# martinruenz/co-fusion

Measured on AMD Instinct MI355X. Metric: frames/sec at 640x480 (N active models) + ICP-reduce achieved HBM GB/s vs peak, higher is better.
Workload: dtype f32

## Files before the change

co_fusion_amd/api.py:

```python
from __future__ import annotations

import ctypes as C

import numpy as np
import torch

from . import lib as _libmod

NUM_PYRS = 3


class Cam(C.Structure):
    _fields_ = [("fx", C.c_float), ("fy", C.c_float), ("cx", C.c_float), ("cy", C.c_float)]

    def level(self, l):
        d = float(1 << l)
        return Cam(self.fx / d, self.fy / d, self.cx / d, self.cy / d)


class Config(C.Structure):
    _fields_ = [("width", C.c_int), ("height", C.c_int), ("fx", C.c_float), ("fy", C.c_float), ("cx", C.c_float),
                ("cy", C.c_float), ("device", C.c_int), ("max_models", C.c_int), ("max_surfels", C.c_int)]


# ... 280 lines not shown
        self._check(self.lib.cf_odom_track_batch_async(self.h, oo, n, pp, C.byref(opts), ee))

    def _batch_args(self, odoms, poses):
        n = len(odoms)
        self._keep_poses = [_f(np.asarray(p, np.float32).reshape(16)) for p in poses]
        pp = (C.POINTER(C.c_float) * max(n, 1))(*[C.cast(k, C.POINTER(C.c_float)) for k in self._keep_poses])
        oo = (C.c_void_p * max(n, 1))(*[o.h for o in odoms])

        def ptrs(ts):
            if ts is None:
                return None
            assert len(ts) == n
            return (C.c_void_p * max(n, 1))(*[None if t is None else t.data_ptr() for t in ts])
        return n, oo, pp, ptrs

    def init_models_batch_select(self, odoms, pred_v4, pred_n4, pred_rgba, poses, frame_rgba, alt_v4=None, alt_n4=None, alt_rgba=None,
                                 fill_counts=None, ratio=0.0):
        n, oo, pp, ptrs = self._batch_args(odoms, poses)
        self._check(self.lib.cf_odom_init_models_batch_select(self.h, oo, n, ptrs(pred_v4), ptrs(pred_n4), ptrs(pred_rgba), ptrs(alt_v4),
                                                              ptrs(alt_n4), ptrs(alt_rgba), ptrs(fill_counts), C.c_float(ratio), pp,
                                                              ptrs(frame_rgba)))

    def init_models_batch_frames(self, odoms, pred_v4, pred_n4, pred_rgba, poses, frame_rgba):
        n, oo, pp, ptrs = self._batch_args(odoms, poses)
        self._check(self.lib.cf_odom_init_models_batch_frames(self.h, oo, n, ptrs(pred_v4), ptrs(pred_n4), ptrs(pred_rgba), pp, ptrs(frame_rgba)))

    def init_models_batch(self, odoms, pred_v4, pred_n4, pred_rgba, poses, frame_rgba):
        n, oo, pp, ptrs = self._batch_args(odoms, poses)
        self._check(self.lib.cf_odom_init_models_batch(self.h, oo, n, ptrs(pred_v4), ptrs(pred_n4), ptrs(pred_rgba), pp, _p(frame_rgba)))

    def set_icp_arith(self, mode):
        self._check(self.lib.cf_set_icp_arith(self.h, {"product": 0, "gram": 1, "reference": 2}.get(mode, mode)))

    def profile_enable(self, on=True):
        self._check(self.lib.cf_profile_enable(self.h, int(on)))

    def profile_read(self, reset=True):
        p = Profile()
        self._check(self.lib.cf_profile_read(self.h, C.byref(p), int(reset)))
        return p


class Odometry:

    _BUF = {0: (np.float32, 3), 1: (np.float32, 3), 2: (np.float32, 3), 3: (np.float32, 3), 4: (np.float32, 1),
            5: (np.float32, 1), 6: (np.uint8, 1), 7: (np.uint8, 1), 8: (np.uint8, 1), 9: (np.int16, 1),
            10: (np.int16, 1)}

    def __init__(self, ctx: Context):
        self.ctx = ctx
        self.h = C.c_void_p()
        ctx._check(ctx.lib.cf_odom_create(ctx.h, C.byref(self.h)))

    def close(self):
        if getattr(self, "h", None) and self.ctx.h:
            self.ctx.lib.cf_odom_destroy(self.h)
        self.h = None

    def __del__(self):
        try:
            self.close()
        except Exception:
            pass

    def init_icp_model(self, pred_v4, pred_n4, pose):
        self.ctx._check(self.ctx.lib.cf_odom_init_icp_model(self.h, _p(pred_v4), _p(pred_n4),
                                                            _f(np.asarray(pose, np.float32).reshape(16))))

    def init_rgb_model(self, rgba):
        self.ctx._check(self.ctx.lib.cf_odom_init_rgb_model(self.h, _p(rgba)))

    def set_band(self, row_begin, row_end, add_counts=1):
        self.ctx._check(self.ctx.lib.cf_odom_set_band(self.h, int(row_begin), int(row_end), int(add_counts)))

    def set_culling(self, on=True):
        self.ctx._check(self.ctx.lib.cf_odom_set_culling(self.h, int(bool(on))))

    def init_rgb(self, rgba):
        self.ctx._check(self.ctx.lib.cf_odom_init_rgb(self.h, _p(rgba)))

    def init_first_rgb(self, rgba):
        self.ctx._check(self.ctx.lib.cf_odom_init_first_rgb(self.h, _p(rgba)))

    def init_icp(self, depth_pyr, cutoff):
        arr = (C.c_void_p * 3)(*[d.data_ptr() for d in depth_pyr])
        self._keep = depth_pyr
        self.ctx._check(self.ctx.lib.cf_odom_init_icp(self.h, arr, C.c_float(cutoff)))

    def init_icp_maps(self, vertex4, normal4):
        self.ctx._check(self.ctx.lib.cf_odom_init_icp_maps(self.h, _p(vertex4), _p(normal4)))

    def track(self, trans, rot, rgb_only=False, icp_weight=10.0, pyramid=True, fast_odom=False, so3=True,
              err_surface=None):
        t = _f(np.asarray(trans, np.float32).reshape(3))
        r = _f(np.asarray(rot, np.float32).reshape(9))
        opts = TrackOpts(int(rgb_only), int(pyramid), int(fast_odom), int(so3), icp_weight)
        st = TrackStats()
        self.ctx._check(self.ctx.lib.cf_odom_get_incremental_transformation(self.h, t, r, C.byref(opts),
                                                                            _p(err_surface), C.byref(st)))
        return np.array(t, np.float32), np.array(r, np.float32).reshape(3, 3), st

    def fetch(self):
        t = (C.c_float * 3)(); r = (C.c_float * 9)()
        st = TrackStats()
        self.ctx._check(self.ctx.lib.cf_odom_fetch_result(self.h, t, r, C.byref(st)))
        return np.array(t, np.float32), np.array(r, np.float32).reshape(3, 3), st

    def level0_visited(self):
        a = C.c_uint64(); b = C.c_uint64()
        self.ctx._check(self.ctx.lib.cf_odom_level0_visited(self.h, C.byref(a), C.byref(b)))
        return a.value, b.value

    def last_launch_shape(self):
        a = (C.c_int * 3)(); b = (C.c_int * 3)(); e = C.c_int()
        self.ctx._check(self.ctx.lib.cf_odom_last_launch_shape(self.h, a, b, C.byref(e)))
        return list(a), list(b), e.value

    def share_frame_maps(self, owner):
        self.ctx._check(self.ctx.lib.cf_odom_share_frame_maps(self.h, owner.h))

    def bench_icp(self, level, iters=200):
        us = C.c_float()
        self.ctx._check(self.ctx.lib.cf_odom_bench_icp(self.h, level, iters, C.byref(us)))
        return us.value

    def buffer_address(self, which, level):
        ptr = C.c_void_p()
        self.ctx._check(self.ctx.lib.cf_odom_buffer(self.h, which, level, C.byref(ptr), None))
        return ptr.value

    def buffer(self, which, level):
        ptr = C.c_void_p(); nbytes = C.c_uint64()
        self.ctx._check(self.ctx.lib.cf_odom_buffer(self.h, which, level, C.byref(ptr), C.byref(nbytes)))
        host = np.empty(nbytes.value, np.uint8)
        self.ctx._check(self.ctx.lib.cf_memcpy_d2h(self.ctx.h, host.ctypes.data_as(C.c_void_p), ptr, nbytes))
        w, h = self.ctx.width >> level, self.ctx.height >> level
        if which == 11:
            return host.view(np.float32).reshape(h, w, 3)
        if which == 12:
            return host.view(DATATERM).reshape(h * w)
        if which == 13:
            return host.reshape(h, w)
        if which == 14:
            return host.view(np.float32).reshape((h * w + 63) // 64, 2)
        if which == 15:
            return host.reshape(self.ctx.height // 4, self.ctx.width // 4)
        if which == 16:
            return host.view(np.uint32)
        dt, planes = self._BUF[which]
        return host.view(dt).reshape(planes * h, w)


class FrameDecoder:

    def __init__(self, ctx: Context, max_w, max_h, slots=4):
        from . import klg as _klg
        self._klg = _klg
        self.ctx, self.lib = ctx, ctx.lib
        self.max_w, self.max_h, self.slots = int(max_w), int(max_h), int(slots)
        self.lib.cf_frame_decoder_create.argtypes = [C.c_void_p, C.c_int, C.c_int, C.c_int, C.POINTER(C.c_void_p)]
        self.lib.cf_frame_decoder_destroy.argtypes = [C.c_void_p]
        self.lib.cf_frame_decoder_destroy.restype = None
        self.lib.cf_frame_decoder_slot.argtypes = [C.c_void_p, C.c_int, C.POINTER(_klg.FrameSlot)]
        self.lib.cf_frame_decoder_submit.argtypes = [C.c_void_p, C.c_int, C.POINTER(_klg.FrameDesc)]
        self.lib.cf_frame_decoder_acquire.argtypes = [C.c_void_p, C.c_int, C.c_int, C.POINTER(C.c_void_p), C.POINTER(C.c_void_p)]
        self.lib.cf_frame_decoder_timing.argtypes = [C.c_void_p, C.c_int, C.POINTER(C.c_double), C.POINTER(C.c_double), C.POINTER(C.c_uint64)]
        from . import images as _im
        self._im = _im
        self.lib.cf_frame_decoder_enable_images.argtypes = [C.c_void_p]
        self.lib.cf_frame_decoder_image_slot.argtypes = [C.c_void_p, C.c_int, C.POINTER(_im.ImageSlot)]
# ... 211 lines not shown
```

co_fusion_amd/csrc/cabi.hip:

```cpp
#include <stdlib.h>
#include <string.h>

#include <string>

#include "cf_host.h"

using namespace cf;

void cf_ctx::set_error(const std::string& m)
{
    std::lock_guard<std::mutex> lk(error_mutex);
    last_error = m;
}

static int lane_ready(cf_ctx* ctx, int lane)
{
    if (!ctx->lanes[lane]) {
        HIPCHK(ctx, hipStreamCreateWithFlags(&ctx->lanes[lane], hipStreamNonBlocking));
        HIPCHK(ctx, hipEventCreateWithFlags(&ctx->lane_done[lane], hipEventDisableTiming));
    }
    return CF_OK;
}
static void leave_lane(cf_ctx* ctx)
{
    if (ctx->forked) { ctx->stream = ctx->forked_from; ctx->forked = false; }
}
static int join_lane(cf_ctx* ctx, int lane)
{
    HIPCHK(ctx, hipEventRecord(ctx->lane_done[lane], ctx->lanes[lane]));
    HIPCHK(ctx, hipStreamWaitEvent(ctx->stream, ctx->lane_done[lane], 0));
    return CF_OK;
}

extern "C" {

int cf_create(const cf_config* cfg, cf_ctx** out)
{
    if (!cfg || !out || cfg->width <= 0 || cfg->height <= 0 || (cfg->width % 16) || (cfg->height % 4)) return CF_EINVAL;
    int ndev = 0;
    if (hipGetDeviceCount(&ndev) != hipSuccess || ndev <= 0) return CF_EHIP;
    cf_ctx* ctx = new cf_ctx();
    ctx->cfg = *cfg;
    if (ctx->cfg.max_models <= 0) ctx->cfg.max_models = 1;
    *out = ctx;
    HIPCHK(ctx, hipSetDevice(cfg->device));
    HIPCHK(ctx, hipStreamCreateWithFlags(&ctx->own_stream, hipStreamNonBlocking));
    ctx->stream = ctx->own_stream;
    ctx->icp_launch = IcpLaunch{256, 0, 0};
    if (int r = dmalloc(ctx, &ctx->d_acc_a, (size_t)kGroups * 32)) return r;
    if (int r = dmalloc(ctx, &ctx->d_acc_b, (size_t)kGroups * 32)) return r;
    if (int r = dmalloc(ctx, &ctx->d_out, 64)) return r;
    if (int r = dmalloc(ctx, &ctx->d_scratch_state, 1)) return r;
    if (int r = dmalloc(ctx, &ctx->d_state_pool, (size_t)cf_ctx::kStateSlots)) return r;
    HIPCHK(ctx, hipHostMalloc(reinterpret_cast<void**>(&ctx->h_state_pool), sizeof(OdomDev) * cf_ctx::kStateSlots, hipHostMallocCoherent));
    memset(ctx->h_state_pool, 0, sizeof(OdomDev) * cf_ctx::kStateSlots);
    if (int r = dmalloc(ctx, &ctx->d_so3_sync, (size_t)ctx->cfg.max_models + 1)) return r;
    if (const char* e = getenv("CF_ICP_ARITH")) {
        if (cf_set_icp_arith(ctx, (!strcmp(e, "gram") || !strcmp(e, "1")) ? CF_ICP_ARITH_GRAM : (!strcmp(e, "reference") || !strcmp(e, "2")) ? CF_ICP_ARITH_REFERENCE
                                  : (!strcmp(e, "product") || !strcmp(e, "0")) ? CF_ICP_ARITH_PRODUCT : -1) != CF_OK) {
            ctx->set_error("CF_ICP_ARITH: product | gram | reference"); return CF_EINVAL;
        }
    }
    if (int r = dmalloc(ctx, &ctx->d_cand_scratch, (size_t)cfg->width * cfg->height)) return r;
    HIPCHK(ctx, hipHostMalloc(reinterpret_cast<void**>(&ctx->h_scratch_state), sizeof(OdomDev)));
    HIPCHK(ctx, hipHostMalloc(reinterpret_cast<void**>(&ctx->h_out), sizeof(unsigned long long) * 64));
    ctx->prof.capacity = 8192;
    ctx->prof.events = new hipEvent_t[ctx->prof.capacity];
    for (int i = 0; i < ctx->prof.capacity; i++) HIPCHK(ctx, hipEventCreate(&ctx->prof.events[i]));
    ctx->prof.used = 0; ctx->prof.enabled = 0; ctx->prof.bytes = 0; ctx->prof.launches = 0;
    HIPCHK(ctx, hipStreamSynchronize(ctx->stream));
    return CF_OK;
}

void cf_destroy(cf_ctx* ctx)
{
    if (ctx && ctx->batch_event) (void)hipEventDestroy(ctx->batch_event);
    if (ctx) for (int i = 0; i < cf_ctx::kSurfEvents; i++) if (ctx->surf_events[i]) (void)hipEventDestroy(ctx->surf_events[i]);
    if (!ctx) return;
    (void)hipStreamSynchronize(ctx->stream);
    (void)cf_rccl_destroy(ctx);
    (void)hipFree(ctx->d_acc_a); (void)hipFree(ctx->d_acc_b); (void)hipFree(ctx->d_out);
    (void)hipFree(ctx->d_scratch_state); (void)hipFree(ctx->d_so3_sync); (void)hipFree(ctx->d_cand_scratch);
    (void)hipFree(ctx->d_state_pool); (void)hipHostFree(ctx->h_state_pool);
    (void)hipHostFree(ctx->h_scratch_state); (void)hipHostFree(ctx->h_out);
    if (ctx->d_ref) (void)hipFree(ctx->d_ref);
    if (ctx->h_ref) (void)hipHostFree(ctx->h_ref);
    if (ctx->d_redetect_bits) (void)hipFree(ctx->d_redetect_bits);
    if (ctx->d_redetect_counts) (void)hipFree(ctx->d_redetect_counts);
    if (ctx->h_redetect_counts) (void)hipHostFree(ctx->h_redetect_counts);
    if (ctx->d_search) (void)hipFree(ctx->d_search);
    if (ctx->h_search) (void)hipHostFree(ctx->h_search);
    for (hipEvent_t e : ctx->redetect_ev) if (e) (void)hipEventDestroy(e);
    if (ctx->prof.events) {
        for (int i = 0; i < ctx->prof.capacity; i++) (void)hipEventDestroy(ctx->prof.events[i]);
        delete[] ctx->prof.events;
    }
    for (int i = 0; i < cf_ctx::kLanes; i++) {
        if (ctx->lanes[i]) (void)hipStreamDestroy(ctx->lanes[i]);
        if (ctx->lane_done[i]) (void)hipEventDestroy(ctx->lane_done[i]);
    }
    if (ctx->fork_point) (void)hipEventDestroy(ctx->fork_point);
    for (int i = 0; i < cf_ctx::kMarks; i++) if (ctx->marks[i]) (void)hipEventDestroy(ctx->marks[i]);
    if (ctx->own_stream) (void)hipStreamDestroy(ctx->own_stream);
    delete ctx;
}

const char* cf_last_error(const cf_ctx* ctx)
{
    if (!ctx) return "null ctx";
    static thread_local std::string copy;
    {
        std::lock_guard<std::mutex> lk(const_cast<cf_ctx*>(ctx)->error_mutex);
        copy = ctx->last_error;
    }
    return copy.c_str();
}
int cf_set_stream(cf_ctx* ctx, void* s)
{
    if (!ctx || ctx->forked) return CF_EINVAL;
    if (ctx->stream != (hipStream_t)s) HIPCHK(ctx, hipStreamSynchronize(ctx->stream));
    ctx->stream = (hipStream_t)s;
    return CF_OK;
}
int cf_use_own_stream(cf_ctx* ctx)
{
    if (!ctx || ctx->forked) return CF_EINVAL;
    if (ctx->stream != ctx->own_stream) HIPCHK(ctx, hipStreamSynchronize(ctx->stream));
    ctx->stream = ctx->own_stream;
    return CF_OK;
}

extern "C++" { thread_local cf_thread_binding cf_tls_binding; }

int cf_fork(cf_ctx* ctx, int lane)
{
    if (!ctx || lane < 0) return CF_EINVAL;
    lane %= cf_ctx::kLanes;
    if (int r = lane_ready(ctx, lane)) return r;
    if (!ctx->fork_point) HIPCHK(ctx, hipEventCreateWithFlags(&ctx->fork_point, hipEventDisableTiming));
    if (!ctx->forked) {
        ctx->forked_from = ctx->stream;
        HIPCHK(ctx, hipEventRecord(ctx->fork_point, ctx->forked_from));
        ctx->forked = true;
    }
    HIPCHK(ctx, hipStreamWaitEvent(ctx->lanes[lane], ctx->fork_point, 0));
    ctx->lanes_used |= 1u << lane;
    ctx->stream = ctx->lanes[lane];
    return CF_OK;
}
int cf_mark(cf_ctx* ctx, int slot)
{
    if (!ctx || slot < 0 || slot >= cf_ctx::kMarks) return CF_EINVAL;
    if (!ctx->marks[slot]) HIPCHK(ctx, hipEventCreateWithFlags(&ctx->marks[slot], hipEventDisableTiming));
    HIPCHK(ctx, hipEventRecord(ctx->marks[slot], ctx->stream));
    ctx->mark_set[slot] = true;
    return CF_OK;
}
int cf_event_wait_host(cf_ctx* ctx, int slot)
{
    if (!ctx || slot < 0 || slot >= cf_ctx::kMarks) return CF_EINVAL;
    if (ctx->mark_set[slot]) HIPCHK(ctx, hipEventSynchronize(ctx->marks[slot]));
    return CF_OK;
}
int cf_fork_after(cf_ctx* ctx, int lane, int slot)
{
    if (!ctx || lane < 0 || slot >= cf_ctx::kMarks || ctx->forked) return CF_EINVAL;
    lane %= cf_ctx::kLanes;
    if (int r = lane_ready(ctx, lane)) return r;
    if (slot >= 0 && ctx->mark_set[slot]) HIPCHK(ctx, hipStreamWaitEvent(ctx->lanes[lane], ctx->marks[slot], 0));
    ctx->forked_from = ctx->stream;
    ctx->forked = true;
    ctx->lanes_used |= 1u << lane;
    ctx->stream = ctx->lanes[lane];
    return CF_OK;
}
int cf_main(cf_ctx* ctx)
{
    if (!ctx) return CF_EINVAL;
    leave_lane(ctx);
    return CF_OK;
}
int cf_join(cf_ctx* ctx)
{
    if (!ctx) return CF_EINVAL;
// ... 132 lines not shown
```

co_fusion_amd/csrc/cabi_odom.hip:

```cpp
#include <math.h>
#include <string.h>

#include <string>
#include <vector>

#include "cf_host.h"

using namespace cf;

template <typename F>
static int each_level_buffer(cf_odom* od, int i, size_t n, F f)
{
    if (int r = f(od->vmap_g_prev[i], n * 3)) return r;
    if (int r = f(od->nmap_g_prev[i], n * 3)) return r;
    if (int r = f(od->vmap_curr[i], n * 3)) return r;
    if (int r = f(od->nmap_curr[i], n * 3)) return r;
    if (int r = f(od->lastDepth[i], n)) return r;
    if (int r = f(od->nextDepth[i], n)) return r;
    if (int r = f(od->lastImage[i], n)) return r;
    if (int r = f(od->nextImage[i], n)) return r;
    if (int r = f(od->lastNextImage[i], n)) return r;
    if (int r = f(od->dIdx[i], n)) return r;
    if (int r = f(od->dIdy[i], n)) return r;
    if (int r = f(od->cloud[i], n * 3)) return r;
// ... 91 lines not shown
static int populate_rgbd(cf_odom* od, const uint8_t* rgba, float* const* depths, uint8_t* const* images)
{
    cf_ctx* ctx = od->ctx; hipStream_t s = ctx->stream;
    RgbdBatch b{};
    b.c[0] = rgbd_chain(od, rgba, depths, images);
    launch_rgbd_pyramids(s, b, 1, ctx->cfg.width, ctx->cfg.height, od->maxDepthRGB);
    LAUNCHCHK(ctx);
    return CF_OK;
}
int cf_odom_init_rgb_model(cf_odom* od, const uint8_t* pred_rgba) { if (!od || !pred_rgba) return CF_EINVAL; return populate_rgbd(od, pred_rgba, od->lastDepth, od->lastImage); }
int cf_odom_init_rgb(cf_odom* od, const uint8_t* rgba) { if (!od || !rgba) return CF_EINVAL; od->next_depth_is_last = false; return populate_rgbd(od, rgba, od->nextDepth, od->nextImage); }

int cf_odom_init_models_batch(cf_ctx* ctx, cf_odom* const* ods, int n, const float* const* pred_v4, const float* const* pred_n4,
                              const uint8_t* const* pred_rgba, const float* const* poses, const uint8_t* frame_rgba)
{
    if (!ctx || n <= 0 || !frame_rgba) return CF_EINVAL;
    std::vector<const uint8_t*> frames((size_t)n, frame_rgba);
    return cf_odom_init_models_batch_frames(ctx, ods, n, pred_v4, pred_n4, pred_rgba, poses, frames.data());
}

int cf_odom_init_models_batch_frames(cf_ctx* ctx, cf_odom* const* ods, int n, const float* const* pred_v4, const float* const* pred_n4,
                                     const uint8_t* const* pred_rgba, const float* const* poses, const uint8_t* const* frame_rgba)
{
    return cf_odom_init_models_batch_select(ctx, ods, n, pred_v4, pred_n4, pred_rgba, nullptr, nullptr, nullptr, nullptr, 0.f, poses, frame_rgba);
}

int cf_odom_init_models_batch_select(cf_ctx* ctx, cf_odom* const* ods, int n, const float* const* pred_v4, const float* const* pred_n4,
                                     const uint8_t* const* pred_rgba, const float* const* alt_v4, const float* const* alt_n4,
                                     const uint8_t* const* alt_rgba, const uint32_t* const* fill_counts, float ratio,
                                     const float* const* poses, const uint8_t* const* frame_rgba)
{
    if (!ctx || !ods || n <= 0 || !pred_v4 || !pred_n4 || !pred_rgba || !poses || !frame_rgba) return CF_EINVAL;
    const bool choose = alt_v4 && alt_n4 && alt_rgba && fill_counts;
    const int W = ctx->cfg.width, H = ctx->cfg.height;
    hipStream_t s = ctx->stream;
    for (int base = 0; base < n; base += kPrepBatch) {
        const int nb = n - base < kPrepBatch ? n - base : kPrepBatch;
        ModelMapsBatch mb{};
        RgbdBatch rb{};
        for (int k = 0; k < nb; k++) {
            cf_odom* od = ods[base + k];
            if (!od || !pred_v4[base + k] || !pred_n4[base + k] || !pred_rgba[base + k] || !poses[base + k] || !frame_rgba[base + k]) return CF_EINVAL;
            mb.m[k] = model_maps_args(od, pred_v4[base + k], pred_n4[base + k], poses[base + k]);
            rb.c[k] = rgbd_chain(od, pred_rgba[base + k], od->lastDepth, od->lastImage);
            rb.c[k].v4 = pred_v4[base + k];
            if (choose && fill_counts[base + k]) {
                if (!alt_v4[base + k] || !alt_n4[base + k] || !alt_rgba[base + k]) return CF_EINVAL;
                mb.m[k].alt_v4 = alt_v4[base + k]; mb.m[k].alt_n4 = alt_n4[base + k]; mb.m[k].sel = fill_counts[base + k]; mb.m[k].sel_ratio = ratio;
                rb.c[k].alt_v4 = alt_v4[base + k]; rb.c[k].alt_rgba = alt_rgba[base + k]; rb.c[k].sel = fill_counts[base + k]; rb.c[k].sel_ratio = ratio;
            }
            od->next_depth_is_last = true;
        }
        int n_chains = nb;
        for (int k = 0; k < nb; k++) {
            cf_odom* od = ods[base + k];
            int owner = -1;
            for (int j = nb; j < n_chains; j++)
                if (rb.c[j].rgba == frame_rgba[base + k]) { owner = j; break; }
            if (owner < 0) {
                owner = n_chains++;
                rb.c[owner] = rgbd_chain(od, frame_rgba[base + k], od->nextDepth, od->nextImage);
                for (int i = 0; i < CF_NUM_PYRS; ++i) rb.c[owner].depth[i] = nullptr;
            }
            rb.fan_owner[k] = (signed char)(owner + 1);
            for (int i = 0; i < CF_NUM_PYRS; ++i) rb.fan_image[i][k] = od->nextImage[i];
        }
        launch_model_maps_and_pyramids(s, mb, nb, rb, n_chains, W, H, ods[base]->maxDepthRGB);
    }
    LAUNCHCHK(ctx);
    return CF_OK;
}

int cf_odom_init_first_rgb(cf_odom* od, const uint8_t* rgba)
{
    if (!od || !rgba) return CF_EINVAL;
    cf_ctx* ctx = od->ctx; hipStream_t s = ctx->stream;
    const int W = ctx->cfg.width, H = ctx->cfg.height;
    launch_intensity(s, rgba, W, H, od->lastNextImage[0]);
    for (int i = 0; i + 1 < CF_NUM_PYRS; i++) launch_pyrdown_u8(s, od->lastNextImage[i], W >> i, H >> i, od->lastNextImage[i + 1]);
    LAUNCHCHK(ctx);
    return CF_OK;
}

int cf_odom_init_icp(cf_odom* od, const float* const depth_pyr[CF_NUM_PYRS], float depth_cutoff)
{
    if (!od || !depth_pyr) return CF_EINVAL;
    cf_ctx* ctx = od->ctx; hipStream_t s = ctx->stream;
    const int W = ctx->cfg.width, H = ctx->cfg.height;
    FrameMapsArgs a{};
    a.cutoff = depth_cutoff;
    for (int i = 0; i < CF_NUM_PYRS; ++i) {
        const cf_cam il = cam_level(ctx_cam(ctx), i);
        a.depth[i] = depth_pyr[i]; a.vmap[i] = od->vmap_curr[i]; a.nmap[i] = od->nmap_curr[i]; a.zrange[i] = od->zrange[i];
        a.fx_inv[i] = 1.f / il.fx; a.fy_inv[i] = 1.f / il.fy; a.cx[i] = il.cx; a.cy[i] = il.cy;
        od->ext_vmap_curr[i] = nullptr; od->ext_nmap_curr[i] = nullptr; od->ext_zrange[i] = nullptr;
    }
    launch_frame_maps(s, a, W, H);
    od->zrange_valid = true;
    LAUNCHCHK(ctx);
    return CF_OK;
}

int cf_odom_init_icp_maps(cf_odom* od, const float* vertex4, const float* normal4)
{
    if (!od || !vertex4 || !normal4) return CF_EINVAL;
    cf_ctx* ctx = od->ctx; hipStream_t s = ctx->stream;
    const int W = ctx->cfg.width, H = ctx->cfg.height;
    HIPCHK(ctx, hipMemcpyAsync(od->vmaps_tmp, vertex4, sizeof(float) * 4 * (size_t)W * H, hipMemcpyDeviceToDevice, s));
    for (int i = 0; i < CF_NUM_PYRS; ++i) { od->ext_vmap_curr[i] = nullptr; od->ext_nmap_curr[i] = nullptr; od->ext_zrange[i] = nullptr; }
    launch_copy_maps(s, vertex4, normal4, W, H, od->vmap_curr[0], od->nmap_curr[0]);
    for (int i = 1; i < CF_NUM_PYRS; ++i) {
        launch_resize_map(s, od->vmap_curr[i - 1], W >> (i - 1), H >> (i - 1), od->vmap_curr[i], false);
        launch_resize_map(s, od->nmap_curr[i - 1], W >> (i - 1), H >> (i - 1), od->nmap_curr[i], true);
    }
    od->zrange_valid = false;
    LAUNCHCHK(ctx);
    return CF_OK;
}

int cf_odom_set_culling(cf_odom* od, int on)
{
    if (!od) return CF_EINVAL;
    od->use_occ = on != 0;
    return CF_OK;
}

int cf_odom_set_band(cf_odom* od, int row_begin, int row_end, int add_counts)
{
    if (!od || row_begin < 0 || row_end < row_begin || row_end > od->ctx->cfg.height || (row_begin & 3) || (row_end & 3)) return CF_EINVAL;
    od->band_begin = row_begin; od->band_end = row_end; od->band_counts = add_counts != 0;
    return CF_OK;
}
int cf_set_collective(cf_ctx* ctx, int (*fn)(void*, int, void*, uint64_t, void*), void* user)
{
    if (!ctx) return CF_EINVAL;
    ctx->collective = fn; ctx->collective_user = user;
    return CF_OK;
}

int cf_odom_bind_frame_maps(cf_odom* od, const float* const vmaps[CF_NUM_PYRS], const float* const nmaps[CF_NUM_PYRS])
{
    if (!od) return CF_EINVAL;
    for (int i = 0; i < CF_NUM_PYRS; i++) { od->ext_vmap_curr[i] = vmaps ? vmaps[i] : nullptr; od->ext_nmap_curr[i] = nmaps ? nmaps[i] : nullptr; od->ext_zrange[i] = nullptr; }
    return CF_OK;
}
int cf_odom_share_frame_maps(cf_odom* od, cf_odom* owner)
{
    if (!od || !owner || od->ctx != owner->ctx) return CF_EINVAL;
    for (int i = 0; i < CF_NUM_PYRS; i++) {
        od->ext_vmap_curr[i] = owner->cur_vmap(i); od->ext_nmap_curr[i] = owner->cur_nmap(i); od->ext_zrange[i] = owner->cur_zrange(i);
    }
    return CF_OK;
}

int cf_odom_level0_visited(cf_odom* od, uint64_t* icp_pixels, uint64_t* residual_pixels)
{
    if (!od || !icp_pixels || !residual_pixels) return CF_EINVAL;
    const cf_ctx* ctx = od->ctx;
    const OdomDev* h = od->h_state;
    const uint64_t N = (uint64_t)ctx->cfg.width * ctx->cfg.height;
    *icp_pixels = N; *residual_pixels = h->rgb ? N : 0;
    if (!h->icp) *icp_pixels = 0;
    if (h->cull && ctx->icp_arith != CF_ICP_ARITH_REFERENCE) {
        if (h->icp) { const CullRuns cr = cull_runs(h->stats.cull_box, 0, ctx->cfg.width, ctx->cfg.height); *icp_pixels = (uint64_t)cr.total * 64 < N ? (uint64_t)cr.total * 64 : N; }
        if (h->rgb && h->res_range && h->res_seen[0] >= 0) { const uint64_t px = (uint64_t)h->res_seen[0] * (uint64_t)(ctx->icp_launch.threads * 4); *residual_pixels = px < N ? px : N; }
    }
    return CF_OK;
}

int cf_odom_last_launch_shape(cf_odom* od, int icp_blocks[3], int residual_blocks[3], int* icp_blocks_err)
{
    if (!od) return CF_EINVAL;
    for (int l = 0; l < CF_NUM_PYRS; l++) {
        if (icp_blocks) icp_blocks[l] = od->launch_shape.icp[l];
        if (residual_blocks) residual_blocks[l] = od->launch_shape.res[l];
    }
    if (icp_blocks_err) *icp_blocks_err = od->launch_shape.icp_err;
    return CF_OK;
}

int cf_odom_buffer(cf_odom* od, int which, int level, void** dptr, uint64_t* bytes)
{
    if (!od || level < 0 || level >= CF_NUM_PYRS || !dptr) return CF_EINVAL;
    const size_t n = (size_t)(od->ctx->cfg.width >> level) * (od->ctx->cfg.height >> level);
    void* p = nullptr; size_t b = 0;
    if (which == 0 && !od->ext_vmap_curr[level]) od->zrange_valid = false;
    switch (which) {
        case 0: p = (void*)od->cur_vmap(level); b = n * 12; break;
        case 1: p = (void*)od->cur_nmap(level); b = n * 12; break;
        case 2: p = od->vmap_g_prev[level]; b = n * 12; break;
        case 3: p = od->nmap_g_prev[level]; b = n * 12; break;
        case 4: p = od->lastDepth[level]; b = n * 4; break;
        case 5: p = od->next_depth(level); b = n * 4; break;
        case 6: p = od->lastImage[level]; b = n; break;
        case 7: p = od->nextImage[level]; b = n; break;
        case 8: p = od->lastNextImage[level]; b = n; break;
        case 9: p = od->dIdx[level]; b = n * 2; break;
        case 10: p = od->dIdy[level]; b = n * 2; break;
        case 11: p = od->cloud[level]; b = n * 12; break;
        case 12: p = od->corres[level]; b = n * 16; break;
        case 13: p = od->cand[level]; b = n; break;
        case 14: p = od->zrange[level]; b = (n + 63) / 64 * sizeof(float2); break;
        case 15: if (level != 0) return CF_EINVAL; p = od->occ; b = (size_t)(od->ctx->cfg.width >> 2) * (od->ctx->cfg.height >> 2); break;
        case 16: if (level != 0) return CF_EINVAL; p = od->aabb; b = 6 * sizeof(unsigned); break;
        default: return CF_EINVAL;
    }
    *dptr = p; if (bytes) *bytes = b;
    return CF_OK;
}

}
```

co_fusion_amd/csrc/cabi_steps.hip:

```cpp
#include <math.h>
#include <string.h>

#include <string>
#include <vector>

#include "cf_host.h"
#include "gn_ref_host.h"

using namespace cf;

template <int N, typename Word>
static void unpack_upper(float* A, float* b, Word word)
{
    int shift = 0;
    for (int i = 0; i < N; ++i)
        for (int j = i; j < N + 1; ++j) {
            const float value = word(shift, i, j);
            shift++;
            if (j == N) { if (b) b[i] = value; }
            else if (A) A[j * N + i] = A[i * N + j] = value;
        }
}
static void se3_unpack_host(const unsigned long long* t, int F, float* A, float* b, float* residual)
{
// ... 312 lines not shown
        OdomDev* s = &h[(size_t)k];
        memset(s, 0, sizeof(*s));
        gn_state_to_dev(y.state, s);
        s->icp_acc = buf.d_acc + acc_words * k; s->rgb_acc = s->icp_acc + kAccWords;
        s->sobelScale = sobel_scale; s->maxDepthDeltaRGB = max_depth_delta;
        s->host_twin = &buf.h_twins[k];
        refresh_hot(s);
        memset(&buf.h_twins[k], 0, sizeof(OdomDev));
        gn_state_to_dev(y.twin, &buf.h_twins[k]);
        if (mode == 2) HIPCHK(ctx, hipMemsetAsync(s->rgb_acc, 0xA5, 8 * rgb_words, ctx->stream));
        unsigned long long* seed = &seeds[(size_t)k * kAccWords];
        for (int g = 0; g < kGroups; g++) { seed[(size_t)g * 32 + 29] = (unsigned long long)y.count_seed[g]; seed[(size_t)g * 32 + 30] = (unsigned long long)y.sigma_seed[g]; }
        HIPCHK(ctx, hipMemcpyAsync(s->icp_acc, seed, 8 * kAccWords, hipMemcpyHostToDevice, ctx->stream));
        OdomDev level = *s;
        level.width = cols; level.height = rows;
        level.cand[0] = y.cand; level.nextDepth[0] = y.next_depth; level.lastDepth[0] = y.last_depth; level.lastImage[0] = y.last_image;
        level.nextImage[0] = y.next_image; level.cloud[0] = y.cloud; level.dIdx[0] = y.dIdx; level.dIdy[0] = y.dIdy;
        level.corres[0] = buf.d_recs + N * k;
        level.res_range = y.ranged ? buf.d_range + 2 * k : nullptr;
        ra.m[k] = rgb_model_args(&level, buf.d_states + k, 0);
        ra.m[k].no_counts = y.no_counts ? 1 : 0;
        ra.m[k].res_blocks = y.ranged ? y.res_blocks : 0;
        ranges[(size_t)2 * k] = y.res_range[0]; ranges[(size_t)2 * k + 1] = y.res_range[1];
        HIPCHK(ctx, hipMemcpyAsync(ra.m[k].recs, y.records, 8 * N, hipMemcpyHostToDevice, ctx->stream));
        HIPCHK(ctx, hipMemcpyAsync(ra.m[k].slot_counts, y.slot_counts, sizeof(unsigned) * n_slots, hipMemcpyHostToDevice, ctx->stream));
    }
    HIPCHK(ctx, hipMemcpyAsync(buf.d_range, ranges.data(), sizeof(unsigned) * 2 * n, hipMemcpyHostToDevice, ctx->stream));
    HIPCHK(ctx, hipMemcpyAsync(buf.d_states, h.data(), sizeof(OdomDev) * n, hipMemcpyHostToDevice, ctx->stream));
    launch_rgb_records_residual(ctx->stream, ctx->icp_launch, ra, n, 0);
    LAUNCHCHK(ctx);
    for (int k = 0; k < n; k++) {
        HIPCHK(ctx, hipMemcpyAsync(systems[k].records, ra.m[k].recs, 8 * N, hipMemcpyDeviceToHost, ctx->stream));
        HIPCHK(ctx, hipMemcpyAsync(systems[k].slot_counts, ra.m[k].slot_counts, sizeof(unsigned) * n_slots, hipMemcpyDeviceToHost, ctx->stream));
        HIPCHK(ctx, hipMemcpyAsync(&acc_a[(size_t)k * kAccWords], ra.m[k].icp_acc, 8 * kAccWords, hipMemcpyDeviceToHost, ctx->stream));
    }
    launch_rgb_slot_step(ctx->stream, ra, buf.d_sync, n, mode, ctx->icp_launch.gram ? -1 : CF_FIX_ICP, next_level, last_of_level ? 1 : 0);
    LAUNCHCHK(ctx);
    if (mode == 2) HIPCHK(ctx, hipMemcpyAsync(h.data(), buf.d_states, sizeof(OdomDev) * n, hipMemcpyDeviceToHost, ctx->stream));
    else for (int k = 0; k < n; k++)
        HIPCHK(ctx, hipMemcpyAsync(&acc_b[(size_t)k * kAccWords], ra.m[k].rgb_acc, 8 * kAccWords, hipMemcpyDeviceToHost, ctx->stream));
    HIPCHK(ctx, hipStreamSynchronize(ctx->stream));
    for (int k = 0; k < n; k++) {
        cf_rgb_system& y = systems[k];
        unsigned long long c = 0, g2 = 0;
        for (int g = 0; g < kGroups; g++) { c += acc_a[(size_t)k * kAccWords + (size_t)g * 32 + 29]; g2 += acc_a[(size_t)k * kAccWords + (size_t)g * 32 + 30]; }
        y.count_total = (int64_t)c; y.sigma_total = (int64_t)g2;
        for (int w = 0; w < 32; w++) {
            unsigned long long t = 0;
            for (int g = 0; g < kGroups && mode != 2; g++) t += acc_b[(size_t)k * kAccWords + (size_t)g * 32 + w];
            y.rgb_sums[w] = (int64_t)t;
        }
        if (mode == 2) {
            gn_state_from_dev(&h[(size_t)k], &y.state);
            gn_state_from_dev(&buf.h_twins[k], &y.twin);
            memcpy(y.hot, &h[(size_t)k].hot, sizeof(GnHot));
        } else memcpy(y.hot, &h[(size_t)k].hot, sizeof(GnHot));
    }
    return CF_OK;
}

int cf_so3_prealign_step(cf_ctx* ctx, int n, cf_so3_system* systems, int do_so3, int first_level)
{
    if (!ctx || !systems || n < 1 || n > kMaxBatch || n > ctx->cfg.max_models || first_level < 0 || first_level > 2) return CF_EINVAL;
    static_assert(sizeof(systems->sync) == sizeof(So3Sync) && sizeof(systems->hot) == sizeof(GnHot), "cf_so3_system mirrors the sync and the hot block");
    for (int k = 0; k < n; k++) {
        const cf_gn_state& g = systems[k].state_in;
        if (g.width <= 0 || g.height <= 0 || (g.width % 16) || (g.height % 4)) return CF_EINVAL;
        if (do_so3 && (!systems[k].last_next_image || !systems[k].next_image)) return CF_EINVAL;
    }
    std::vector<OdomDev> back((size_t)n);
    GnStepBuffers buf;
    buf.stream = ctx->stream;
    HIPCHK(ctx, hipMalloc(reinterpret_cast<void**>(&buf.d_states), sizeof(OdomDev) * n));
    HIPCHK(ctx, hipHostMalloc(reinterpret_cast<void**>(&buf.h_twins), sizeof(OdomDev) * n, hipHostMallocCoherent));
    HIPCHK(ctx, hipMemsetAsync(buf.d_states, 0xA5, sizeof(OdomDev) * n, ctx->stream));
    TrackerStates states{};
    for (int k = 0; k < n; k++) {
        OdomDev* s = &buf.h_twins[k];
        memset(s, 0, sizeof(*s));
        gn_state_to_dev(systems[k].state_in, s);
        s->lastNextImage[2] = systems[k].last_next_image; s->nextImage[2] = systems[k].next_image;
        states.dev[k] = buf.d_states + k; states.host[k] = s;
    }
    launch_so3_prealign(ctx->stream, states, ctx->d_so3_sync, n, do_so3 != 0, first_level, nullptr);
    LAUNCHCHK(ctx);
    HIPCHK(ctx, hipMemcpyAsync(back.data(), buf.d_states, sizeof(OdomDev) * n, hipMemcpyDeviceToHost, ctx->stream));
    for (int k = 0; k < n; k++)
        HIPCHK(ctx, hipMemcpyAsync(systems[k].sync, ctx->d_so3_sync + k, sizeof(So3Sync), hipMemcpyDeviceToHost, ctx->stream));
    HIPCHK(ctx, hipStreamSynchronize(ctx->stream));
    for (int k = 0; k < n; k++) {
        gn_state_from_dev(&back[(size_t)k], &systems[k].state_out);
        memcpy(systems[k].hot, &back[(size_t)k].hot, sizeof(GnHot));
    }
    return CF_OK;
}

}
```

co_fusion_amd/csrc/cabi_track.hip:

```cpp
#include <math.h>
#include <stdio.h>
#include <stdlib.h>
#include <string.h>

#include <string>
#include <utility>

#include "cf_host.h"

using namespace cf;

#ifdef CF_ABLATE
static bool diag_no_box() { static const bool v = getenv("CF_NO_SCREEN_BOX") != nullptr; return v; }
static bool diag_no_zcull() { static const bool v = getenv("CF_NO_ZCULL") != nullptr; return v; }
static bool diag_no_occ() { static const bool v = getenv("CF_NO_OCC") != nullptr; return v; }
static const char* diag_icp_ablate() { return getenv("CF_ICP_ABLATE"); }
static const char* diag_trace_out(const char* name) { const char* e = getenv("CF_ICP_TRACE_OUT"); return e ? e : name; }
struct DiagCall {
    const char* name; int call = -2, seen = 0;
    bool hit() { if (call == -2) call = getenv(name) ? atoi(getenv(name)) : -1; return call >= 0 && seen++ == call; }
};
static int clear_accumulators(cf_ctx* ctx, cf_odom* const* ods, int n)
{
    for (int m = 0; m < n; m++) {
// ... 129 lines not shown
    }
    od->pending_so3_swap = opts->so3 != 0;
    od->launch_shape = LaunchShape{};
    LAUNCHCHK(ctx);
    return CF_OK;
}

static void fill_rgb_args(cf_ctx* ctx, cf_odom* const* ods, int n, RgbArgs out[3])
{
    for (int l = 0; l < 3; l++) {
        RgbArgs& a = out[l];
        memset(&a, 0, sizeof(a));
        a.cols = ctx->cfg.width >> l; a.rows = ctx->cfg.height >> l;
        a.il = cam_level(ctx_cam(ctx), l);
        a.sobelScale = ods[0]->sobelScale; a.maxDepthDelta = ods[0]->maxDepthDeltaRGB;
        for (int m = 0; m < n; m++) {
            a.m[m] = rgb_model_args(ods[m]->h_state, ods[m]->d_state, l);
            a.m[m].no_counts = (ods[m]->band_end > 0 && !ods[m]->band_counts) ? 1 : 0;
            a.m[m].res_blocks = a.m[m].res_range ? residual_blocks_for(ods[m]->res_hint[l]) : 0;
        }
    }
}

static void fill_icp_args(cf_ctx* ctx, cf_odom* const* ods, int n, IcpArgs out[3])
{
    for (int l = 0; l < CF_NUM_PYRS; l++) {
        IcpArgs& a = out[l];
        memset(&a, 0, sizeof(a));
        a.cols = ctx->cfg.width >> l; a.rows = ctx->cfg.height >> l;
        a.intr = cam_level(ctx_cam(ctx), l);
        a.distThres = ods[0]->distThres; a.angleThres = ods[0]->angleThres;
        a.angleSqLt = ods[0]->angleSqLt; a.distSqLe = ods[0]->distSqLe;
        a.occ_w = ctx->cfg.width >> 2; a.occ_shift = 2 - l;
        for (int m = 0; m < n; m++) {
            cf_odom* od = ods[m];
            a.m[m] = IcpModelArgs{od->cur_vmap(l), od->cur_nmap(l), od->vmap_g_prev[l], od->nmap_g_prev[l], od->d_state, od->icp_acc,
                                  od->h_state->err_surface, (od->use_occ && od->occ_valid && !diag_no_occ()) ? od->occ : nullptr,
                                  od->band_end > 0 ? (od->band_begin >> l) : 0, od->band_end > 0 ? (od->band_end >> l) : 0,
                                  od->h_state->cull,
                                  diag_no_zcull() ? nullptr : od->cur_zrange(l),
                                  od->h_state->cull ? box_blocks_for(od->box_hint, l, a.cols, a.rows, ctx->icp_launch.threads) : 0};
        }
    }
}

static int prepare_trackers(cf_ctx* ctx, cf_odom* const* ods, int n, const float* const* poses_in, const cf_track_opts* opts,
                            float* const* err_surfaces, RgbPrepBatch& prep, bool launch_prep, bool reference)
{
    for (int base = 0; base < n; base += kPrepBatch) {
        const int nb = n - base < kPrepBatch ? n - base : kPrepBatch;
        if (base) prep = RgbPrepBatch{};
        for (int m = base; m < base + nb; m++) {
            if (int r = odom_prepare(ods[m], poses_in[m], opts, err_surfaces ? err_surfaces[m] : nullptr, &prep.m[m - base])) return r;
            if (reference) {
                ods[m]->h_state->cull = 0; ods[m]->h_state->res_range = nullptr; prep.m[m - base].res_range = nullptr;
                ods[m]->box_hint[0] = kNoBoxHint;
                HIPCHK(ctx, hipMemsetAsync(ods[m]->aabb, 0, 8 * sizeof(unsigned), ctx->stream));
            }
        }
        if (launch_prep) launch_rgb_prep(ctx->stream, prep, nb, ctx->cfg.width, ctx->cfg.height);
    }
    return CF_OK;
}

extern "C" {

int cf_odom_track_batch_async(cf_ctx* ctx, cf_odom* const* ods, int n, const float* const* poses_in,
                              const cf_track_opts* opts, float* const* err_surfaces)
{
    if (!ctx || !ods || n <= 0 || n > ctx->cfg.max_models || n > kMaxBatch || !poses_in || !opts) return CF_EINVAL;
    const TrackTerms terms = track_terms(opts);
    {
        bool drain = false;
        for (int m = 0; m < n; m++) drain = drain || (ods[m] && ods[m]->result_pending);
        if (drain) {
            HIPCHK(ctx, hipStreamSynchronize(ctx->stream));
            for (int m = 0; m < n; m++) if (ods[m]) ods[m]->result_pending = false;
        }
    }
    RgbPrepBatch prep{};
    if (ctx->icp_arith == CF_ICP_ARITH_REFERENCE) {
        for (int m = 0; m < n; m++)
            if (ods[m]->band_end > 0) { ctx->set_error("the reference-order arithmetic (cf_set_icp_arith 2) does not split a tracker's reductions over GPUs"); return CF_ESTATE; }
        if (int r = prepare_trackers(ctx, ods, n, poses_in, opts, err_surfaces, prep, terms.rgb, true)) return r;
        LAUNCHCHK(ctx);
        for (int m = 0; m < n; m++)
            if (int r = ref_track(ctx, ods[m], poses_in[m], opts, err_surfaces ? err_surfaces[m] : nullptr)) return r;
        for (int m = 0; m < n; m++) ods[m]->result_pending = true;
        return CF_OK;
    }
    for (int m = 0; m < n; m++)
        if (ods[m]->gn_epoch_seen != ctx->gn_mode_epoch) {
            HIPCHK(ctx, hipMemsetAsync(ods[m]->rgb_acc, 0, sizeof(unsigned long long) * ods[m]->rgb_acc_words, ctx->stream));
            ods[m]->gn_epoch_seen = ctx->gn_mode_epoch;
        }
    const bool prep_fused = terms.rgb && opts->so3 != 0 && n <= kPrepBatch;
    if (int r = prepare_trackers(ctx, ods, n, poses_in, opts, err_surfaces, prep, terms.rgb && !prep_fused, false)) return r;
    if (prep_fused) rgb_prep_levels(prep, n, ctx->cfg.width, ctx->cfg.height);
    TrackerStates states{};
    for (int m = 0; m < n; m++) { states.dev[m] = ods[m]->d_state; states.host[m] = ods[m]->h_state; }
    IcpArgs icp_args[3];
    fill_icp_args(ctx, ods, n, icp_args);
    RgbArgs rgb_args[3];
    fill_rgb_args(ctx, ods, n, rgb_args);
    OdomDev* h_states[kMaxBatch];
    for (int m = 0; m < n; m++) h_states[m] = ods[m]->h_state;
    GnHook hook{};
    hook.fn = ctx->collective; hook.user = ctx->collective_user;
    bool any_split = false;
    for (int m = 0; m < n; m++) { hook.split[m] = ods[m]->band_end > 0 ? 1 : 0; any_split = any_split || hook.split[m]; }
    if (any_split && !ctx->collective) { ctx->set_error("a tracker has a row band (cf_odom_set_band) but no collective is registered (cf_set_collective)"); return CF_ESTATE; }
    if (any_split && ctx->gn_mode == 0) { ctx->set_error("split reductions need the record-slot data path (cf_set_gn_mode 1)"); return CF_ESTATE; }
    cf::ProfSink* prof = nullptr;
    if (ctx->prof.enabled > 0 && (ctx->prof_calls++ % (unsigned)ctx->prof.enabled) == 0) prof = &ctx->prof;
    TrackDiag diag;
    if (int r = diag.begin(ctx)) return r;
    LaunchShape* shapes[kMaxBatch];
    for (int m = 0; m < n; m++) shapes[m] = &ods[m]->launch_shape;
    IcpLaunch launch_cfg = ctx->icp_launch; launch_cfg.shape = shapes;
    if (!launch_gn_track(ctx->stream, launch_cfg, states, ctx->d_so3_sync, any_split ? &hook : nullptr, icp_args, rgb_args, n,
                         ctx->cfg.width, ctx->cfg.height, opts->so3 != 0, opts->pyramid != 0, opts->fast_odom != 0, terms.rgb, terms.icp, ctx->gn_mode, prof,
                         h_states, prep_fused ? &prep : nullptr)) {
        ctx->set_error("tracking: the registered collective failed inside the Gauss-Newton loop");
        return CF_ESTATE;
    }
    LAUNCHCHK(ctx);
    if (int r = diag.end(ctx, ods, n, icp_args[0], rgb_args[0])) return r;
    for (int m = 0; m < n; m++) ods[m]->result_pending = true;
    return CF_OK;
}

int cf_wait_stream(cf_ctx* ctx)
{
    HIPCHK(ctx, hipStreamSynchronize(ctx->stream));
    return CF_OK;
}

int cf_odom_fetch_result(cf_odom* od, float trans[3], float rot[9], cf_track_stats* stats)
{
    if (!od) return CF_EINVAL;
    cf_ctx* ctx = od->ctx;
    if (int r = cf_wait_stream(ctx)) return r;
    od->result_pending = false;
    if (trans) memcpy(trans, od->h_state->tcurr, 12);
    if (rot) memcpy(rot, od->h_state->Rcurr, 36);
    if (stats) *stats = od->h_state->stats;
    bool fault = od->h_state->stats.fault != 0;
    if (ctx->icp_arith != CF_ICP_ARITH_REFERENCE && od->expected_solves >= 0 && od->h_state->solves != od->expected_solves) {
        (void)hipMemsetAsync(ctx->d_so3_sync, 0, sizeof(So3Sync) * ((size_t)ctx->cfg.max_models + 1), ctx->stream);
        fault = true;
    }
    od->expected_solves = -1;
    if (od->pending_so3_swap) {
        for (int i = 0; i < CF_NUM_PYRS; i++) std::swap(od->lastNextImage[i], od->nextImage[i]);
        od->pending_so3_swap = false;
    }
    if (fault) {
        ctx->set_error("tracking: a bounded device-side wait expired (workgroups of one launch were not co-resident)");
        return CF_ESTATE;
    }
    return CF_OK;
}

int cf_odom_get_covariance(const cf_track_stats* stats, double cov[36])
{
    if (!stats || !cov) return CF_EINVAL;
    constexpr int N = 6;
    double lu[N * N];
    int perm[N];
    memcpy(lu, stats->lastA, sizeof(lu));
    for (int i = 0; i < N; i++) perm[i] = i;
    for (int k = 0; k < N; k++) {
        int piv = k;
        double big = fabs(lu[k * N + k]);
        for (int r = k + 1; r < N; r++) { const double a = fabs(lu[r * N + k]); if (a > big) { big = a; piv = r; } }
        if (piv != k) {
            for (int c = 0; c < N; c++) std::swap(lu[k * N + c], lu[piv * N + c]);
            std::swap(perm[k], perm[piv]);
        }
        if (big != 0.0)
            for (int r = k + 1; r < N; r++) lu[r * N + k] /= lu[k * N + k];
        for (int r = k + 1; r < N; r++)
            for (int c = k + 1; c < N; c++) lu[r * N + c] -= lu[r * N + k] * lu[k * N + c];
    }
    for (int j = 0; j < N; j++) {
        double x[N];
        for (int i = 0; i < N; i++) x[i] = (perm[i] == j) ? 1.0 : 0.0;
        for (int i = 0; i < N; i++)
            for (int c = 0; c < i; c++) x[i] -= lu[i * N + c] * x[c];
        for (int i = N - 1; i >= 0; i--) {
            for (int c = i + 1; c < N; c++) x[i] -= lu[i * N + c] * x[c];
            x[i] /= lu[i * N + i];
        }
        for (int i = 0; i < N; i++) cov[i * N + j] = x[i];
    }
    return CF_OK;
}

int cf_set_gn_mode(cf_ctx* ctx, int mode)
{
    if (!ctx || mode < 0 || mode > 2) return CF_EINVAL;
    if (mode == 2) {
        if (ctx->xcd_round_robin < 0) { HIPCHK(ctx, hipStreamSynchronize(ctx->stream)); ctx->xcd_round_robin = probe_xcd_round_robin(ctx->stream) ? 1 : 0; }
        if (!ctx->xcd_round_robin) { ctx->set_error("cf_set_gn_mode 2: workgroups of a launch are not dealt round-robin over 8 XCDs on this device; the mode needs that"); return CF_ESTATE; }
    }
// ... 43 lines not shown
```

co_fusion_amd/csrc/cf_host.h:

```cpp
#pragma once

#include <string.h>

#include <mutex>
#include <string>

#include "cf_kernels.h"

struct cf_ctx;
struct cf_thread_binding { const cf_ctx* ctx = nullptr; hipStream_t stream = nullptr; };
extern thread_local cf_thread_binding cf_tls_binding;

struct cf_ctx {
    cf_config cfg{};
    hipStream_t stream = nullptr;
    hipStream_t cur() const { return cf_tls_binding.ctx == this ? cf_tls_binding.stream : stream; }
    hipStream_t own_stream = nullptr;
    std::string last_error;
    std::mutex error_mutex;
    cf::IcpLaunch icp_launch{256, 0};
    int icp_arith = 0;
    float* d_ref = nullptr;
    float* h_ref = nullptr;
    unsigned long long* d_acc_a = nullptr;
    unsigned long long* d_acc_b = nullptr;
    unsigned long long* d_out = nullptr;
    unsigned long long* h_out = nullptr;
    cf::OdomDev* d_scratch_state = nullptr;
    cf::OdomDev* h_scratch_state = nullptr;
    uint8_t* d_cand_scratch = nullptr;
    cf::So3Sync* d_so3_sync = nullptr;
    unsigned gn_mode_epoch = 0;
    int xcd_round_robin = -1;
    int gn_mode = 1;
    static constexpr int kStateSlots = 256;
    cf::OdomDev* d_state_pool = nullptr;
    cf::OdomDev* h_state_pool = nullptr;
    bool slot_used[kStateSlots]{};
    hipEvent_t batch_event = nullptr;
    bool extent_cull = true;
    static constexpr int kLanes = 8;
    hipStream_t lanes[kLanes]{};
    hipEvent_t lane_done[kLanes]{};
    hipEvent_t fork_point = nullptr;
    static constexpr int kMarks = 64;
    hipEvent_t marks[kMarks]{};
    bool mark_set[kMarks]{};
    hipStream_t forked_from = nullptr;
    bool forked = false;
    unsigned lanes_used = 0;
    int (*collective)(void* user, int op, void* dev_buf, uint64_t words, void* stream) = nullptr;
    void* collective_user = nullptr;
    void* rccl = nullptr;
    unsigned prof_calls = 0;
    cf::ProfSink prof{};
    double prof_ms_accum = 0;
    static constexpr int kSurfEvents = 64;
    hipEvent_t surf_events[kSurfEvents]{};
    int surf_used = 0; unsigned surf_calls_seen = 0;
    double surf_ms_accum = 0; uint64_t surf_calls = 0, surf_bytes = 0;
    unsigned* d_redetect_bits = nullptr; unsigned redetect_words = 0;
    unsigned* d_redetect_counts = nullptr; unsigned* h_redetect_counts = nullptr;
    bool redetect_timing = false; hipEvent_t redetect_ev[2]{}; float redetect_last_ms = 0.f;
    static constexpr size_t kSearchWords = (size_t)cf::kRedetectBatch * cf::kMomentWords + 32;
    static constexpr size_t kSearchBytes = kSearchWords * 8 + (size_t)cf::kRedetectBatch * cf::kRedetectBins * 4;
    unsigned long long* d_search = nullptr; unsigned long long* h_search = nullptr;
    void set_error(const std::string& m);
};
inline cf_cam ctx_cam(const cf_ctx* ctx) { return cf_cam{ctx->cfg.fx, ctx->cfg.fy, ctx->cfg.cx, ctx->cfg.cy}; }
extern "C" int cf_wait_stream(cf_ctx* ctx);
#define HIPCHK(ctx, call)                                                                      \
    do {                                                                                       \
        hipError_t e_ = (call);                                                                \
        if (e_ != hipSuccess) {                                                                \
            (ctx)->set_error(std::string(#call) + ": " + hipGetErrorString(e_));               \
            return CF_EHIP;                                                                    \
        }                                                                                      \
    } while (0)
#define LAUNCHCHK(ctx) HIPCHK(ctx, hipGetLastError())
template <typename T>
inline int dmalloc(cf_ctx* ctx, T** p, size_t count)
{
    HIPCHK(ctx, hipMalloc(reinterpret_cast<void**>(p), count * sizeof(T)));
    HIPCHK(ctx, hipMemsetAsync(*p, 0, count * sizeof(T), ctx->cur()));
    return CF_OK;
}
inline int clear_acc(cf_ctx* ctx, unsigned long long* acc)
{
    HIPCHK(ctx, hipMemsetAsync(acc, 0, sizeof(unsigned long long) * cf::kGroups * 32, ctx->stream));
    return CF_OK;
}
struct cf_odom;
namespace cf {
int ref_track(cf_ctx* ctx, cf_odom* od, const float pose[16], const cf_track_opts* opts, float* err_surface);
int ref_icp_step(cf_ctx* ctx, const float Rcurr[9], const float tcurr[3], const float* vc, const float* nc, const float Rprev_inv[9], const float tprev[3],
                 cf_cam intr, const float* vp, const float* np, float dist_thres, float angle_thres, int cols, int rows, float* err, float out29[29]);
int ref_rgb_step(cf_ctx* ctx, const cf_dataterm* corres, float sigma, const float* cloud3, float fx, float fy, const int16_t* dIdx, const int16_t* dIdy,
                 float sobel_scale, int cols, int rows, float out29[29]);
int ref_so3_step(cf_ctx* ctx, const uint8_t* last_image, const uint8_t* next_image, const float basis[9], const float kinv[9], const float krlr[9],
                 int cols, int rows, float out11[11]);
inline void pose_split(const float pose[16], float R[9], float t[3])
{
    for (int i = 0; i < 3; i++) { R[3 * i] = pose[4 * i]; R[3 * i + 1] = pose[4 * i + 1]; R[3 * i + 2] = pose[4 * i + 2]; t[i] = pose[4 * i + 3]; }
}
struct TrackTerms { bool icp, rgb; };
inline TrackTerms track_terms(const cf_track_opts* o) { return TrackTerms{!o->rgb_only && o->icp_weight > 0, o->rgb_only || o->icp_weight < 100}; }
}

struct cf_odom {
    cf_ctx* ctx = nullptr;
    float* vmaps_tmp = nullptr;
    float* nmaps_tmp = nullptr;
    float* vmap_g_prev[3]{};
    float* nmap_g_prev[3]{};
    float* vmap_curr[3]{};
    float* nmap_curr[3]{};
    const float* ext_vmap_curr[3]{};
    const float* ext_nmap_curr[3]{};
    float2* zrange[3]{};
    bool zrange_valid = false;
    const float2* ext_zrange[3]{};
    const float* cur_vmap(int l) const { return ext_vmap_curr[l] ? ext_vmap_curr[l] : vmap_curr[l]; }
    const float* cur_nmap(int l) const { return ext_nmap_curr[l] ? ext_nmap_curr[l] : nmap_curr[l]; }
    const float2* cur_zrange(int l) const { return ext_vmap_curr[l] ? ext_zrange[l] : (zrange_valid ? zrange[l] : nullptr); }
    float* lastDepth[3]{};
    float* nextDepth[3]{};
    bool next_depth_is_last = false;
    float* next_depth(int i) const { return next_depth_is_last ? lastDepth[i] : nextDepth[i]; }
    uint8_t* lastImage[3]{};
    uint8_t* nextImage[3]{};
    uint8_t* lastNextImage[3]{};
    int16_t* dIdx[3]{};
    int16_t* dIdy[3]{};
    float* cloud[3]{};
    cf_dataterm* corres[3]{};
    uint8_t* cand[3]{};
    unsigned char* occ = nullptr;
    bool occ_valid = false;
    bool use_occ = false;
    unsigned* aabb = nullptr;
    float map_pose[12]{};
    int box_hint[4] = {0x7fffffff, 0, 0, 0};
    unsigned* res_range = nullptr;
    int res_hint[3] = {-1, -1, -1};
    bool box_valid = false;
    int band_begin = 0, band_end = 0;
    bool band_counts = true;
    unsigned long long* icp_acc = nullptr;
    unsigned long long* rgb_acc = nullptr;
    cf::OdomDev* d_state = nullptr;
    cf::OdomDev* h_state = nullptr;
    int slot = -1;
    float distThres = 0, angleThres = 0, sobelScale = 0, maxDepthDeltaRGB = 0, maxDepthRGB = 0;
    float angleSqLt = 0, distSqLe = 0;
    float minGrad[3]{};
    bool pending_so3_swap = false;
    size_t rgb_acc_words = 0;
    unsigned gn_epoch_seen = 0;
    bool result_pending = false;
    int expected_solves = -1;
    cf::LaunchShape launch_shape{};
};
```

co_fusion_amd/csrc/cf_kernels.h:

```cpp
#pragma once

#include <hip/hip_runtime.h>
#include <hip/hip_ext.h>
#include <stdint.h>

#include "../../include/cofusion_hip.h"

namespace cf {

__host__ __device__ __forceinline__ cf_cam cam_level(cf_cam c, int level)
{
    const int div = 1 << level;
    return cf_cam{c.fx / div, c.fy / div, c.cx / div, c.cy / div};
}

constexpr int kGroups = 64;

struct alignas(64) GnHot {
    int icp, level_done; float cull_z[2];
    float Rcurr[9], tcurr[3];
    float Rprev_inv[9], tprev[3];
    int cull_box[4];
    int rgb, rgbOnly, level_done2, pad;
    float krkInv[9], kt[3];
// ... 147 lines not shown
    if ((cols & 63) == 0) { const int nrx = (bx1 >> 6) - (bx0 >> 6) + 1; return CullRuns{bx0 >> 6, by0, nrx, nrx * (by1 - by0 + 1)}; }
    const int q0 = (by0 * cols) >> 6, q1 = ((by1 + 1) * cols - 1) >> 6;
    return CullRuns{0, q0, 0, q1 - q0 + 1};
}
inline int box_blocks_for(const int box_hint[4], int L, int cols, int rows, int threads)
{
    if (box_hint[0] == kNoBoxHint) return 0;
    const CullRuns cr = cull_runs(box_hint, L, cols, rows);
    const int wpb = threads / 64;
    const int runs = cr.total + cr.total / 4 + 2 * (cr.nrx > 0 ? cr.nrx : (cols + 63) / 64);
    int want = (((runs + 2 * wpb - 1) / (2 * wpb) + 7) / 8) * 8;
    return want < 8 ? 8 : want;
}
inline int residual_blocks_for(int seen) { return seen < 0 ? 0 : seen + seen / 4 + 2; }
struct GnArgs {
    OdomDev* od[kMaxBatch];
    unsigned long long* icp_acc[kMaxBatch];
    unsigned long long* rgb_acc[kMaxBatch];
    OdomDev* od_host[kMaxBatch];
    int slot_px;
    int icp_gram;
};
struct RgbModelArgs {
    OdomDev* st;
    const uint8_t* cand; const float* nextDepth; const float* lastDepth;
    const uint8_t* lastImage; const uint8_t* nextImage;
    cf_dataterm* corres; const float* cloud; const int16_t* dIdx; const int16_t* dIdy;
    unsigned long long* icp_acc; unsigned long long* rgb_acc;
    int no_counts;
    uint2* recs;
    unsigned* slot_counts;
    const unsigned* res_range;
    int res_blocks;
};
struct RgbArgs {
    RgbModelArgs m[kMaxBatch];
    int cols, rows;
    cf_cam il;
    float sobelScale, maxDepthDelta;
    int compact;
    int slot_px;
    IDiv cdiv;
};
inline RgbModelArgs rgb_model_args(const OdomDev* h , OdomDev* d_state, int level)
{
    return RgbModelArgs{d_state, h->cand[level], h->nextDepth[level], h->lastDepth[level], h->lastImage[level], h->nextImage[level],
                        h->corres[level], h->cloud[level], h->dIdx[level], h->dIdy[level], h->icp_acc, h->rgb_acc, 0,
                        reinterpret_cast<uint2*>(h->corres[level]),
                        reinterpret_cast<unsigned*>(reinterpret_cast<uint2*>(h->corres[level]) + (size_t)(h->width >> level) * (h->height >> level)),
                        h->res_range ? h->res_range + 2 * level : nullptr, 0};
}
constexpr int kMaxSlots = 2 * kMaxBatch;
struct IcpArgs {
    IcpModelArgs m[kMaxBatch];
    int cols, rows;
    cf_cam intr;
    float distThres, angleThres;
    float angleSqLt, distSqLe;
    int occ_w, occ_shift;
    int flags;
    int row_begin, row_end;
    IDiv cdiv;
    int slot_end[kMaxSlots];
    unsigned char slot_desc[kMaxSlots];
    int slots_used;
};
constexpr unsigned char kResidualSlot = 0x80;
void launch_icp_level(hipStream_t s, IcpLaunch cfg, const IcpArgs& args, int n, int level, hipEvent_t ev0 = nullptr, hipEvent_t ev1 = nullptr);
void launch_rgb_residual(hipStream_t s, const RgbArgs& ra, int n);
void launch_rgb_step(hipStream_t s, const RgbArgs& ra, int n);
constexpr uint64_t kRgbResidualBytes = 27;
constexpr uint64_t kRgbResidualBytesCompact = 11;
void launch_acc_total(hipStream_t s, const unsigned long long* acc, unsigned long long* out);
void launch_rgb_cand(hipStream_t s, const int16_t* dIdx, const int16_t* dIdy, const float* next_depth,
                     const uint8_t* next_image, float min_scale, int cols, int rows, uint8_t* cand);
void launch_so3_step(hipStream_t s, const uint8_t* last_image, const uint8_t* next_image, const float basis[9],
                     const float kinv[9], const float krlr[9], int cols, int rows, unsigned long long* out16);
void launch_gn_solve(hipStream_t s, const GnArgs& gn, int n, int next_level, int last_of_level);

struct ProfSink {
    hipEvent_t* events; int capacity; int used; uint64_t bytes; uint64_t launches; int enabled;
};

constexpr int kSo3Blocks = 16;
constexpr int kStepSubs = 16;
struct So3Sync { unsigned long long acc[10][16]; unsigned arrive, depart;
                 unsigned step_top, pad;
                 unsigned step_sub[kStepSubs][32]; };
struct GnHook { int (*fn)(void* user, int op, void* dev_buf, uint64_t words, void* stream); void* user; int split[kMaxBatch]; };
struct TrackerStates { OdomDev* dev[kMaxBatch]; const OdomDev* host[kMaxBatch]; };
bool launch_gn_track(hipStream_t s, IcpLaunch cfg, const TrackerStates& states, So3Sync* so3_syncs ,
                     const GnHook* hook, const IcpArgs icp_args[3], const RgbArgs rgb_args[3], int n, int width, int height, bool so3,
                     bool pyramid, bool fast_odom, bool rgb, bool icp, int mode, ProfSink* prof,
                     OdomDev* const* h_states = nullptr ,
                     const RgbPrepBatch* prep = nullptr );
void launch_rgb_slot_step(hipStream_t s, const RgbArgs& ra, So3Sync* so3_syncs , int n, int mode, int icp_fix, int next_level, int last_of_level);
void launch_rgb_records_residual(hipStream_t s, IcpLaunch cfg, const RgbArgs& ra, int n, int level);
inline size_t rgb_acc_rows(size_t n0)
{
    const size_t slots0 = (n0 + 255) / 256, quads0 = (slots0 + 1) / 2;
    return quads0 > (size_t)kGroups ? quads0 : (size_t)kGroups;
}
void launch_so3_prealign(hipStream_t s, const TrackerStates& states, So3Sync* so3_syncs , int n, bool so3, int first_level,
                         const RgbPrepBatch* prep );
void rgb_prep_levels(RgbPrepBatch& b, int n, int W, int H);
float replay_icp_level0(hipStream_t s, IcpLaunch cfg, const IcpArgs& a0, const RgbArgs& r0, int n, int slots, int ablate, int reps, hipEvent_t e0, hipEvent_t e1);
#ifdef CF_ABLATE
void trace_so3_dump(hipStream_t s);
void trace_solve_begin();
void trace_solve_end(hipStream_t s, const char* path);
void trace_step_solve(hipStream_t s, IcpLaunch cfg, const IcpArgs& a0, const RgbArgs& r0, So3Sync* syncs, int n, const char* path);
void trace_icp_level0(hipStream_t s, IcpLaunch cfg, const IcpArgs& a0, const RgbArgs& r0, int n, int slots, const char* path);
#endif
bool probe_xcd_round_robin(hipStream_t s);
float sqrt_gate_lt(float T);
float sqrt_gate_le(float T);

constexpr int kSurfBatch = 16;
struct IndexPassArgs {
    const float* surfels; const unsigned* count; unsigned id_begin, id_end; float t_inv[16]; float maxDepth; int time, timeDelta;
    unsigned long long* keys; unsigned* index; float* vertConf; float* colorTime; float* normRad;
    const float* t_inv_dev;
    float* clean_rec;
    const float* clean_depth;
    unsigned* ext;
    int ext_slot;
};
__host__ __device__ inline void inv44f(const float a[16], float o[16])
{
    const float c00 = a[5] * a[10] - a[6] * a[9];
    const float c01 = a[6] * a[8] - a[4] * a[10];
    const float c02 = a[4] * a[9] - a[5] * a[8];
    const float det = a[0] * c00 + a[1] * c01 + a[2] * c02;
    const float id = 1.0f / det;
    float Li[9];
    Li[0] = c00 * id; Li[1] = (a[2] * a[9] - a[1] * a[10]) * id; Li[2] = (a[1] * a[6] - a[2] * a[5]) * id;
    Li[3] = c01 * id; Li[4] = (a[0] * a[10] - a[2] * a[8]) * id; Li[5] = (a[2] * a[4] - a[0] * a[6]) * id;
    Li[6] = c02 * id; Li[7] = (a[1] * a[8] - a[0] * a[9]) * id; Li[8] = (a[0] * a[5] - a[1] * a[4]) * id;
    for (int i = 0; i < 3; i++) {
        o[i * 4 + 0] = Li[i * 3 + 0]; o[i * 4 + 1] = Li[i * 3 + 1]; o[i * 4 + 2] = Li[i * 3 + 2];
        o[i * 4 + 3] = -(Li[i * 3 + 0] * a[3] + Li[i * 3 + 1] * a[7] + Li[i * 3 + 2] * a[11]);
    }
    o[12] = 0; o[13] = 0; o[14] = 0; o[15] = 1;
}
struct SplatFillArgs {
    const float* depth_filt; const uint8_t* rgba;
    float inv_fx, inv_fy; int pass_geom, pass_rgb;
    float* fill_vertex; float* fill_normal; uint8_t* fill_image;
    unsigned long long* acc;
    unsigned* out2; unsigned* out2_host;
    int sample_blocks;
};
int fill_ratio_sample_blocks(int cols, int rows);
struct SplatPassArgs {
    const float* surfels; const unsigned* count; unsigned count_bound; float t_inv[16]; float maxDepth, confThreshold; int time, maxTime, timeDelta;
    const float* rays; unsigned long long* keys; uint8_t* image; float* vertexConf; float* normalRad; uint16_t* time16;
    SplatFillArgs fill;
};
struct UpdatePassArgs { const float* in; const unsigned* count; unsigned count_bound; unsigned* owner; const float* records; int time; float* out; };
struct SurfelFuseArgs {
    const unsigned* index; const float* vertConf; const float* normRad;
    const uint8_t* rgba; const float* depth_raw; const float* depth_filt; const uint8_t* mask;
    const float* tcx; const float* tcy;
    float pose[16]; cf_cam cam; float inv_fx, inv_fy;
    int cols, rows, time; float weighting; int maskID; float maxDepth;
    float* records; unsigned* new_flags; unsigned* owner;
    int flags_clean = 0;
};
struct CleanPassArgs {
    const unsigned* index; const float* vertConf; const float* colorTime;
    const float* depth_filt; const uint8_t* mask;
    const float* rec;
    float t_inv[16]; cf_cam cam; int cols, rows, time; float confThreshold, outlierCoeff; int timeDelta, maskID;
    const float* surfels; const unsigned* count; const float* fresh; const unsigned* n_fresh; unsigned total_bound; float* staged; unsigned* flags;
};
struct ScanPassArgs {
    const float* rec; const unsigned* flags; long long n; unsigned* block_sums; unsigned* total; unsigned add_to_total; float* out; unsigned* total_host;
    int zero_flags = 0;
};
void launch_index_keys_batch(hipStream_t s, const IndexPassArgs* items, int n, cf_cam cam, int cols, int rows);
bool launch_update_compaction_index_keys(hipStream_t s, const UpdatePassArgs* up, const ScanPassArgs* sc, const IndexPassArgs* ix, int n, cf_cam cam, int cols,
                                         int rows);
void launch_index_resolve_batch(hipStream_t s, const IndexPassArgs* items, int n, cf_cam cam, int cols, int rows);
enum { kSplatFull = 0, kSplatCount = 1, kSplatDepth = 2 };
void launch_combined_predict_batch(hipStream_t s, const SplatPassArgs* items, int n, cf_cam cam, int cols, int rows, int mode = kSplatFull);
void launch_associate_batch(hipStream_t s, const SurfelFuseArgs* items, int n);
void launch_update_batch(hipStream_t s, const UpdatePassArgs* items, int n);
void launch_clean_batch(hipStream_t s, const CleanPassArgs* items, int n);
// ... 33 lines not shown
```

co_fusion_amd/csrc/track_prep.hip:

```cpp
#include "cf_device.h"
#include "cf_kernels.h"
#include "track_prep_dev.h"

namespace cf {

static constexpr int kBlock = 256;
static inline int grid_for(int n) { return (n + kBlock - 1) / kBlock; }

__global__ void __launch_bounds__(kBlock) vmap_kernel(const float* __restrict__ depth, int cols, int rows, float fx_inv,
                                                      float fy_inv, float cx, float cy, float cutoff,
                                                      float* __restrict__ vmap)
{
    const int i = blockIdx.x * kBlock + threadIdx.x;
    if (i >= cols * rows) return;
    const int v = i / cols, u = i - v * cols;
    const float z = depth[i];
    if (z != 0 && z < cutoff) {
        vmap[i] = z * (u - cx) * fx_inv;
        vmap[i + rows * cols] = z * (v - cy) * fy_inv;
        vmap[i + 2 * rows * cols] = z;
    } else {
        vmap[i] = qnan();
    }
}
// ... 268 lines not shown
    if (fy >= kT2H || gx >= W2 || gy >= H2) return;
    if constexpr (kDepth) store(2, gy * W2 + gx, pyrdown_f32_at(TileTaps<float>{t1, kF1W, oy1, ox1}, W1, H1, gx, gy));
    else store(2, gy * W2 + gx, pyrdown_u8_at(TileTaps<uint8_t>{t1, kF1W, oy1, ox1}, W1, H1, gx, gy));
}
__global__ void __launch_bounds__(kBlock) rgbd_base_kernel(const RgbdBatch b, int N, float cutoff) { rgbd_base_body(b, N, cutoff, (int)blockIdx.x, (int)blockIdx.y); }
__global__ void __launch_bounds__(kBlock) rgbd_pyrdown_kernel(const RgbdBatch b, int level, int scols, int srows)
{
    const RgbdChain& c = b.c[blockIdx.y];
    const int n = (scols / 2) * (srows / 2), nb = (n + kBlock - 1) / kBlock;
    if ((int)blockIdx.x < nb) {
        const int i = blockIdx.x * kBlock + threadIdx.x;
        if (i < n && c.depth[level]) pyrdown_f32_px(c.depth[level], scols, srows, c.depth[level + 1], i);
    } else {
        const int i = (blockIdx.x - nb) * kBlock + threadIdx.x;
        if (i < n) rgbd_store_image(b, (int)blockIdx.y, level + 1, i, pyrdown_u8_val(c.image[level], scols, srows, i));
    }
}

__global__ void __launch_bounds__(kBlock) rgb_expand_kernel(const uint8_t* __restrict__ rgb, int N, uchar4* __restrict__ rgba)
{
    const int i = blockIdx.x * kBlock + threadIdx.x;
    if (i >= N) return;
    rgba[i] = make_uchar4(rgb[3 * i], rgb[3 * i + 1], rgb[3 * i + 2], 255);
}

__global__ void __launch_bounds__(kBlock) intensity_kernel(const uchar4* __restrict__ rgba, int N, uint8_t* __restrict__ dst)
{
    const int i = blockIdx.x * kBlock + threadIdx.x;
    if (i >= N) return;
    const uchar4 s = rgba[i];
    const int value = (int)((float)s.x * 0.114f + (float)s.y * 0.299f + (float)s.z * 0.587f);
    dst[i] = (uint8_t)value;
}

__constant__ float kSobelX[9] = {0.52201f, 0.00000f, -0.52201f, 0.79451f, -0.00000f, -0.79451f, 0.52201f, 0.00000f, -0.52201f};
__constant__ float kSobelY[9] = {0.52201f, 0.79451f, 0.52201f, 0.00000f, 0.00000f, 0.00000f, -0.52201f, -0.79451f, -0.52201f};

__global__ void __launch_bounds__(kBlock) sobel_kernel(const uint8_t* __restrict__ src, int cols, int rows,
                                                       int16_t* __restrict__ dx, int16_t* __restrict__ dy)
{
    const int i = blockIdx.x * kBlock + threadIdx.x;
    if (i >= cols * rows) return;
    const int y = i / cols, x = i - y * cols;
    float dxv = 0, dyv = 0;
    constexpr float sx[9] = {0.52201f, 0.00000f, -0.52201f, 0.79451f, -0.00000f, -0.79451f, 0.52201f, 0.00000f, -0.52201f};
    constexpr float sy[9] = {0.52201f, 0.79451f, 0.52201f, 0.00000f, 0.00000f, 0.00000f, -0.52201f, -0.79451f, -0.52201f};
    if (x >= 1 && y >= 1 && x <= cols - 2 && y <= rows - 2) {
        const uint8_t* __restrict__ p0 = src + (y - 1) * cols + (x - 1);
#pragma unroll
        for (int r = 0; r < 3; r++)
#pragma unroll
            for (int c = 0; c < 3; c++) {
                const float s = (float)p0[r * cols + c];
                dxv += s * sx[8 - (r * 3 + c)];
                dyv += s * sy[8 - (r * 3 + c)];
            }
    } else {
        int k = 8;
        for (int j = max(y - 1, 0); j <= min(y + 1, rows - 1); j++)
            for (int c = max(x - 1, 0); c <= min(x + 1, cols - 1); c++) {
                const float s = (float)src[j * cols + c];
                dxv += s * kSobelX[k];
                dyv += s * kSobelY[k];
                --k;
            }
    }
    dx[i] = (int16_t)(int)dxv;
    dy[i] = (int16_t)(int)dyv;
}

__global__ void __launch_bounds__(kBlock) cloud_kernel(const float* __restrict__ depth, int cols, int rows, float invFx,
                                                       float invFy, float cx, float cy, float* __restrict__ cloud3)
{
    const int i = blockIdx.x * kBlock + threadIdx.x;
    if (i >= cols * rows) return;
    const int y = i / cols, x = i - y * cols;
    const float z = depth[i];
    cloud3[i * 3 + 0] = (x - cx) * z * invFx;
    cloud3[i * 3 + 1] = (y - cy) * z * invFy;
    cloud3[i * 3 + 2] = z;
}


__global__ void __launch_bounds__(kBlock) frame_maps_kernel(const FrameMapsArgs a)
{
    int lb;
    const int lv = level_of(a.L, blockIdx.x, lb);
    const int cols = a.L.cols[lv], rows = a.L.rows[lv], N = cols * rows;
    const int i = lb * kBlock + threadIdx.x;
    const float* __restrict__ depth = a.depth[lv];
    const float cutoff = a.cutoff;
    if (a.zrange[lv]) {
        const float inf = __int_as_float(0x7f800000);
        const float zz = i < N ? depth[i] : 0.f;
        const bool ok = zz != 0 && zz < cutoff;
        float lo = ok ? zz : inf, hi = ok ? zz : -inf;
#pragma unroll
        for (int o = 32; o > 0; o >>= 1) { lo = fminf(lo, __shfl_xor(lo, o, 64)); hi = fmaxf(hi, __shfl_xor(hi, o, 64)); }
        if ((threadIdx.x & 63) == 0 && i < N) a.zrange[lv][i >> 6] = make_float2(lo, hi);
    }
    if (i >= N) return;
    float* __restrict__ vmap = a.vmap[lv];
    float* __restrict__ nmap = a.nmap[lv];
    const float fx_inv = a.fx_inv[lv], fy_inv = a.fy_inv[lv], cx = a.cx[lv], cy = a.cy[lv];
    const int v = i / cols, u = i - v * cols;
    const bool edge = (u == cols - 1 || v == rows - 1);
    const float z = depth[i];
    const float z01 = edge ? 0.f : depth[i + 1], z10 = edge ? 0.f : depth[i + cols];
    float x00 = qnan();
    if (z != 0 && z < cutoff) {
        x00 = z * (u - cx) * fx_inv;
        vmap[i] = x00;
        vmap[i + N] = z * (v - cy) * fy_inv;
        vmap[i + 2 * N] = z;
    } else {
        vmap[i] = qnan();
    }
    if (edge) { nmap[i] = qnan(); return; }
    const float x01 = (z01 != 0 && z01 < cutoff) ? z01 * ((u + 1) - cx) * fx_inv : qnan();
    const float x10 = (z10 != 0 && z10 < cutoff) ? z10 * (u - cx) * fx_inv : qnan();
    if (!is_nan(x00) && !is_nan(x01) && !is_nan(x10)) {
        const f3 v00 = {x00, z * (v - cy) * fy_inv, z};
        const f3 v01 = {x01, z01 * (v - cy) * fy_inv, z01};
        const f3 v10 = {x10, z10 * ((v + 1) - cy) * fy_inv, z10};
        const f3 r = normalized(cross(v01 - v00, v10 - v00));
        nmap[i] = r.x; nmap[i + N] = r.y; nmap[i + 2 * N] = r.z;
    } else {
        nmap[i] = qnan();
    }
}

__global__ void __launch_bounds__(kBlock) rgb_prep_kernel(const RgbPrepBatch b) { rgb_prep_body(b.m[blockIdx.y], (int)blockIdx.x); }

struct MapVal { f3 p; bool have; };

__device__ __forceinline__ void emit_map(float* __restrict__ map, int idx, int N, const MapVal& m, const m33& R, const f3& t, bool add_t)
{
    if (!m.have) { map[idx] = qnan(); return; }
    if (!is_nan(m.p.x)) {
        f3 d = mul(R, m.p);
        if (add_t) d = d + t;
        map[idx] = d.x; map[idx + N] = d.y; map[idx + 2 * N] = d.z;
    } else {
        map[idx] = qnan(); map[idx + N] = m.p.y; map[idx + 2 * N] = m.p.z;
    }
}

__device__ __forceinline__ MapVal resize4(const MapVal& a00, const MapVal& a01, const MapVal& a10, const MapVal& a11, bool normalize)
{
    MapVal o; o.have = false; o.p = f3{qnan(), qnan(), qnan()};
    const float x00 = a00.have ? a00.p.x : qnan(), x01 = a01.have ? a01.p.x : qnan();
    const float x10 = a10.have ? a10.p.x : qnan(), x11 = a11.have ? a11.p.x : qnan();
    if (is_nan(x00) || is_nan(x01) || is_nan(x10) || is_nan(x11)) return o;
    f3 n;
    n.x = (a00.p.x + a01.p.x + a10.p.x + a11.p.x) / 4;
    n.y = (a00.p.y + a01.p.y + a10.p.y + a11.p.y) / 4;
    n.z = (a00.p.z + a01.p.z + a10.p.z + a11.p.z) / 4;
    if (normalize) n = normalized(n);
    o.have = true; o.p = n;
    return o;
}

__device__ __forceinline__ MapVal lane_mapval(const MapVal& m, int src_lane)
{
    MapVal o;
    o.p.x = __shfl(m.p.x, src_lane, 64); o.p.y = __shfl(m.p.y, src_lane, 64); o.p.z = __shfl(m.p.z, src_lane, 64);
    o.have = __shfl((int)m.have, src_lane, 64) != 0;
    return o;
}
__device__ __forceinline__ void model_maps_tiled_body(const ModelMapsBatch& b, int bx, int by)
{
    const ModelMapsArgs& a = b.m[by];
    const int cols = a.cols, rows = a.rows, N0 = cols * rows, c1 = cols >> 1, c2 = cols >> 2, N1 = N0 >> 2, N2 = N0 >> 4;
    const int lane = threadIdx.x & 63, lx = lane & 15, ly = lane >> 4;
    const int tiles_x = cols >> 4;
    const int tile = bx * 4 + (threadIdx.x >> 6);
    if (tile >= tiles_x * (rows >> 2)) return;
    const int ty = tile / tiles_x, tx = tile - ty * tiles_x;
    const int x = tx * 16 + lx, y = ty * 4 + ly, i0 = y * cols + x;
    const bool alt = a.sel && (float)a.sel[0] / (float)a.sel[1] < a.sel_ratio;
    const float4* __restrict__ v4 = reinterpret_cast<const float4*>(alt ? a.alt_v4 : a.pred_v4);
    const float4* __restrict__ n4 = reinterpret_cast<const float4*>(alt ? a.alt_n4 : a.pred_n4);
    float4* __restrict__ snap = reinterpret_cast<float4*>(a.snapshot);
    m33 R; for (int k = 0; k < 9; k++) R.m[k] = a.R[k];
    const f3 tr = {a.t[0], a.t[1], a.t[2]};
    const float4 vs = v4[i0], ns = n4[i0];
    snap[i0] = vs;
    MapVal v0, n0;
    v0.have = true; n0.have = true;
    const bool valid = !(vs.z == 0);
    if (valid) { v0.p = f3{vs.x, vs.y, vs.z}; n0.p = f3{ns.x, ns.y, ns.z}; }
    else { v0.p = f3{qnan(), qnan(), qnan()}; n0.p = v0.p; }
    emit_map(a.vmap[0], i0, N0, v0, R, tr, true);
    emit_map(a.nmap[0], i0, N0, n0, R, tr, false);
    const MapVal v01 = lane_mapval(v0, lane + 1), v10 = lane_mapval(v0, lane + 16), v11 = lane_mapval(v0, lane + 17);
    const MapVal n01 = lane_mapval(n0, lane + 1), n10 = lane_mapval(n0, lane + 16), n11 = lane_mapval(n0, lane + 17);
    MapVal v1, n1;
    v1.have = false; n1.have = false; v1.p = f3{qnan(), qnan(), qnan()}; n1.p = v1.p;
    if (((lx | ly) & 1) == 0) {
        v1 = resize4(v0, v01, v10, v11, false);
        n1 = resize4(n0, n01, n10, n11, true);
        const int i1 = (y >> 1) * c1 + (x >> 1);
        emit_map(a.vmap[1], i1, N1, v1, R, tr, true);
        emit_map(a.nmap[1], i1, N1, n1, R, tr, false);
    }
    const MapVal w01 = lane_mapval(v1, lane + 2), w10 = lane_mapval(v1, lane + 32), w11 = lane_mapval(v1, lane + 34);
    const MapVal m01 = lane_mapval(n1, lane + 2), m10 = lane_mapval(n1, lane + 32), m11 = lane_mapval(n1, lane + 34);
    const unsigned long long valid_bits = __ballot(valid);
    if ((lx & 3) == 0 && ly == 0) {
        const MapVal v2 = resize4(v1, w01, w10, w11, false);
        const MapVal n2 = resize4(n1, m01, m10, m11, true);
        const int i2 = (y >> 2) * c2 + (x >> 2);
        emit_map(a.vmap[2], i2, N2, v2, R, tr, true);
        emit_map(a.nmap[2], i2, N2, n2, R, tr, false);
        if (a.occ) a.occ[i2] = ((valid_bits >> lx) & 0x000F000F000F000Full) != 0 ? 1 : 0;
    }
    if (a.aabb && valid_bits != 0) {
        const float inf = __int_as_float(0x7f800000);
        float lo[3] = {inf, inf, inf}, hi[3] = {-inf, -inf, -inf};
        if (valid && !is_nan(v0.p.x) && !is_nan(vs.z)) { lo[0] = hi[0] = (float)x; lo[1] = hi[1] = (float)y; lo[2] = hi[2] = vs.z; }
#pragma unroll
        for (int o = 32; o > 0; o >>= 1)
#pragma unroll
            for (int k = 0; k < 3; k++) { lo[k] = fminf(lo[k], __shfl_xor(lo[k], o, 64)); hi[k] = fmaxf(hi[k], __shfl_xor(hi[k], o, 64)); }
        if (lane < 6 && lo[0] <= hi[0] && lo[1] <= hi[1] && lo[2] <= hi[2]) {
            const float val = lane == 0 ? lo[0] : lane == 1 ? lo[1] : lane == 2 ? lo[2] : lane == 3 ? hi[0] : lane == 4 ? hi[1] : hi[2];
            const unsigned key = lane < 3 ? ~fkey(val) : fkey(val);
            if (key > __hip_atomic_load(&a.aabb[lane], __ATOMIC_RELAXED, __HIP_MEMORY_SCOPE_AGENT)) atomicMax(&a.aabb[lane], key);
        }
    }
}
__global__ void __launch_bounds__(256) model_maps_tiled_kernel(const ModelMapsBatch b) { model_maps_tiled_body(b, (int)blockIdx.x, (int)blockIdx.y); }
__global__ void __launch_bounds__(256) prep_fused_kernel(const ModelMapsBatch mb, int mm_bx, int mm_total, const RgbdBatch rb, int W, int H, float cutoff, int tiles)
{
    __shared__ float tile_lds[kTileLds];
    const int n_pyr = (int)gridDim.x - mm_total, b = blockIdx.x;
    if (b >= n_pyr) { const int m = b - n_pyr, by = m / mm_bx; model_maps_tiled_body(mb, m - by * mm_bx, by); }
    else {
        const int by = b / (2 * tiles), t = b - by * 2 * tiles;
        if (t < tiles) rgbd_tile_body<true>(rb, W, H, cutoff, t, by, tile_lds);
        else rgbd_tile_body<false>(rb, W, H, cutoff, t - tiles, by, tile_lds);
    }
}

static Level3 levels3(int W, int H)
{
    Level3 L; int acc = 0;
    for (int i = 0; i < 3; i++) { L.cols[i] = W >> i; L.rows[i] = H >> i; acc += grid_for(L.cols[i] * L.rows[i]); L.blk_end[i] = acc; }
    return L;
}
void launch_frame_maps(hipStream_t s, FrameMapsArgs a, int W, int H)
{
    a.L = levels3(W, H);
    frame_maps_kernel<<<a.L.blk_end[2], kBlock, 0, s>>>(a);
}
void rgb_prep_levels(RgbPrepBatch& b, int n, int W, int H)
{
    const Level3 L = levels3(W, H);
    for (int m = 0; m < n; m++) b.m[m].L = L;
}
void launch_rgb_prep(hipStream_t s, RgbPrepBatch b, int n, int W, int H)
{
    const Level3 L = levels3(W, H);
    for (int m = 0; m < n; m++) b.m[m].L = L;
    rgb_prep_kernel<<<dim3(L.blk_end[2], n), kBlock, 0, s>>>(b);
}
void launch_model_maps(hipStream_t s, const ModelMapsBatch& b, int n)
{
    const int tiles = (b.m[0].cols >> 4) * (b.m[0].rows >> 2);
    model_maps_tiled_kernel<<<dim3((tiles + 3) / 4, n), 256, 0, s>>>(b);
}
void launch_model_maps_and_pyramids(hipStream_t s, const ModelMapsBatch& mb, int n, const RgbdBatch& rb, int n_chains, int W, int H, float cutoff)
{
    static_assert(kBlock == 256, "the fused launch runs both bodies with 256 threads");
    const int mm_bx = ((mb.m[0].cols >> 4) * (mb.m[0].rows >> 2) + 3) / 4, tiles = rgbd_tiles(W, H);
    prep_fused_kernel<<<2 * tiles * n_chains + mm_bx * n, 256, 0, s>>>(mb, mm_bx, mm_bx * n, rb, W, H, cutoff, tiles);
}
void launch_rgbd_pyramids(hipStream_t s, const RgbdBatch& b, int n_chains, int W, int H, float cutoff)
{
    rgbd_base_kernel<<<dim3(2 * grid_for(W * H), n_chains), kBlock, 0, s>>>(b, W * H, cutoff);
    for (int i = 0; i + 1 < 3; i++)
        rgbd_pyrdown_kernel<<<dim3(2 * grid_for(((W >> i) / 2) * ((H >> i) / 2)), n_chains), kBlock, 0, s>>>(b, i, W >> i, H >> i);
}
void launch_vmap(hipStream_t s, const float* depth, int cols, int rows, cf_cam intr, float cutoff, float* vmap)
{
    vmap_kernel<<<grid_for(cols * rows), kBlock, 0, s>>>(depth, cols, rows, 1.f / intr.fx, 1.f / intr.fy, intr.cx, intr.cy,
                                                         cutoff, vmap);
}
void launch_nmap(hipStream_t s, const float* vmap, int cols, int rows, float* nmap)
{
    nmap_kernel<<<grid_for(cols * rows), kBlock, 0, s>>>(vmap, cols, rows, nmap);
}
void launch_copy_maps(hipStream_t s, const float* v4, const float* n4, int cols, int rows, float* vmap, float* nmap)
{
    copy_maps_kernel<<<grid_for(cols * rows), kBlock, 0, s>>>(reinterpret_cast<const float4*>(v4),
                                                              reinterpret_cast<const float4*>(n4), cols * rows, vmap, nmap);
}
void launch_resize_map(hipStream_t s, const float* in, int in_cols, int in_rows, float* out, bool normalize)
{
    const int n = (in_cols / 2) * (in_rows / 2);
    if (normalize) resize_map_kernel<true><<<grid_for(n), kBlock, 0, s>>>(in, in_cols, in_rows, out);
    else resize_map_kernel<false><<<grid_for(n), kBlock, 0, s>>>(in, in_cols, in_rows, out);
}
void launch_transform_maps(hipStream_t s, float* vmap, float* nmap, int cols, int rows, const float R[9], const float t[3])
{
    m33 Rm; for (int i = 0; i < 9; i++) Rm.m[i] = R[i];
    transform_maps_kernel<<<grid_for(cols * rows), kBlock, 0, s>>>(vmap, nmap, cols * rows, Rm, f3{t[0], t[1], t[2]});
}
void launch_vertices_to_depth(hipStream_t s, const float* v4, int cols, int rows, float cutoff, float* depth)
{
    vertices_to_depth_kernel<<<grid_for(cols * rows), kBlock, 0, s>>>(reinterpret_cast<const float4*>(v4), cols * rows,
                                                                      cutoff, depth);
}
void launch_pyrdown_f32(hipStream_t s, const float* src, int scols, int srows, float* dst)
{
    pyrdown_f32_kernel<<<grid_for((scols / 2) * (srows / 2)), kBlock, 0, s>>>(src, scols, srows, dst);
}
void launch_pyrdown_u8(hipStream_t s, const uint8_t* src, int scols, int srows, uint8_t* dst)
{
    pyrdown_u8_kernel<<<grid_for((scols / 2) * (srows / 2)), kBlock, 0, s>>>(src, scols, srows, dst);
}
void launch_intensity(hipStream_t s, const uint8_t* rgba, int cols, int rows, uint8_t* dst)
{
    intensity_kernel<<<grid_for(cols * rows), kBlock, 0, s>>>(reinterpret_cast<const uchar4*>(rgba), cols * rows, dst);
}
void launch_rgb_expand(hipStream_t s, const uint8_t* rgb, int n, uint8_t* rgba)
{
    rgb_expand_kernel<<<grid_for(n), kBlock, 0, s>>>(rgb, n, reinterpret_cast<uchar4*>(rgba));
}
void launch_sobel(hipStream_t s, const uint8_t* src, int cols, int rows, int16_t* dx, int16_t* dy)
{
    sobel_kernel<<<grid_for(cols * rows), kBlock, 0, s>>>(src, cols, rows, dx, dy);
}
void launch_cloud(hipStream_t s, const float* depth, int cols, int rows, cf_cam il, float* cloud3)
{
    cloud_kernel<<<grid_for(cols * rows), kBlock, 0, s>>>(depth, cols, rows, 1.0f / il.fx, 1.0f / il.fy, il.cx, il.cy, cloud3);
}

}
```

co_fusion_amd/csrc/track_prep_dev.h:

```cpp
#pragma once
#include "cf_device.h"
#include "cf_kernels.h"

namespace cf {
__device__ __forceinline__ int level_of(const Level3& L, int b, int& lb)
{
    const int lv = b < L.blk_end[0] ? 0 : (b < L.blk_end[1] ? 1 : 2);
    lb = b - (lv ? L.blk_end[lv - 1] : 0);
    return lv;
}

__device__ __forceinline__ void rgb_prep_body(const RgbPrepArgs& a, int bx)
{
    int lb;
    const int lv = level_of(a.L, bx, lb);
    const int cols = a.L.cols[lv], rows = a.L.rows[lv];
    const int k = lb * 256 + (int)threadIdx.x;
    uint8_t ok = 0;
    if (k < cols * rows) {
    const int y = k / cols, x = k - y * cols;
    const uint8_t* __restrict__ src = a.nextImage[lv];
    {
        const float z = a.lastDepth[lv][k];
        float* __restrict__ cloud3 = a.cloud[lv];
        cloud3[k * 3 + 0] = (x - a.cx[lv]) * z * a.fx_inv[lv];
        cloud3[k * 3 + 1] = (y - a.cy[lv]) * z * a.fy_inv[lv];
        cloud3[k * 3 + 2] = z;
    }
    float dxv = 0, dyv = 0;
    constexpr float sx[9] = {0.52201f, 0.00000f, -0.52201f, 0.79451f, -0.00000f, -0.79451f, 0.52201f, 0.00000f, -0.52201f};
    constexpr float sy[9] = {0.52201f, 0.79451f, 0.52201f, 0.00000f, 0.00000f, 0.00000f, -0.52201f, -0.79451f, -0.52201f};
    if (x >= 1 && y >= 1 && x <= cols - 2 && y <= rows - 2) {
        const uint8_t* __restrict__ p0 = src + (y - 1) * cols + (x - 1);
#pragma unroll
        for (int r = 0; r < 3; r++)
#pragma unroll
            for (int c = 0; c < 3; c++) {
                const float s = (float)p0[r * cols + c];
                dxv += s * sx[8 - (r * 3 + c)];
                dyv += s * sy[8 - (r * 3 + c)];
            }
    } else {
        int kk = 8;
        for (int j = max(y - 1, 0); j <= min(y + 1, rows - 1); j++)
            for (int c = max(x - 1, 0); c <= min(x + 1, cols - 1); c++) {
                const float s = (float)src[j * cols + c];
                dxv += s * sx[kk];
                dyv += s * sy[kk];
                --kk;
            }
    }
    const int16_t dx16 = (int16_t)(int)dxv, dy16 = (int16_t)(int)dyv;
    a.dIdx[lv][k] = dx16; a.dIdy[lv][k] = dy16;
    if (x < cols - 5 && y < rows - 1) {
        bool valid = true;
        for (int u = max(y - 2, 0); u < min(y + 2, rows); u++)
            for (int v = max(x - 2, 0); v < min(x + 2, cols); v++) valid = valid && (src[u * cols + v] > 0);
        if (valid) {
            const int valx = dx16, valy = dy16;
            const float mTwo = (float)((valx * valx) + (valy * valy));
            if (mTwo >= a.minScale[lv] && !is_nan(a.nextDepth[lv][k])) ok = 1;
        }
    }
    a.cand[lv][k] = ok;
    }
    if (a.res_range) {
        if (__syncthreads_or(ok)) {
            if (threadIdx.x == 0) { atomicMax(&a.res_range[2 * lv], ~(unsigned)lb); atomicMax(&a.res_range[2 * lv + 1], (unsigned)lb + 1u); }
        }
    }
}
}
```

co_fusion_amd/csrc/track_reduce.hip:

```cpp
#include "cf_device.h"
#include "cf_kernels.h"
#include "track_prep_dev.h"
#include "track_sums_dev.h"

namespace cf {

__device__ __forceinline__ int idiv(int n, IDiv d) { return (int)(__umulhi((unsigned)n, d.M) >> d.s); }

struct IcpProj { f3 vcurr_g; int g; int inb; int ux, uy; };

__device__ __forceinline__ IcpProj icp_project(const m33& Rcurr, const f3& tcurr, const m33& Rprev_inv, const f3& tprev, const cf_cam& intr,
                                               int cols, int rows, f3 vcurr)
{
    IcpProj o;
    o.vcurr_g = mul(Rcurr, vcurr) + tcurr;
    const f3 vcurr_cp = mul(Rprev_inv, o.vcurr_g - tprev);
    const int ux = f2i_rn(vcurr_cp.x * intr.fx / vcurr_cp.z + intr.cx);
    const int uy = f2i_rn(vcurr_cp.y * intr.fy / vcurr_cp.z + intr.cy);
    o.inb = !(ux < 0 || uy < 0 || ux >= cols || uy >= rows || vcurr_cp.z < 0);
    o.g = o.inb ? uy * cols + ux : 0;
    o.ux = o.inb ? ux : 0; o.uy = o.inb ? uy : 0;
    return o;
}

// ... 590 lines not shown

#include "track_so3_dev.h"
#include "track_solve_dev.h"
#include "track_rgb_step_dev.h"

namespace cf {

#ifdef CF_ABLATE
static IcpArgs g_last_icp_args; static int g_last_n_icp_blocks = 0, g_last_grid = 0;
#endif
static IcpArgs with_cdiv(IcpArgs a) { a.cdiv = make_idiv(a.cols); return a; }
typedef void (*IcpKernel)(const IcpArgs, const RgbArgs, int);
#define ICP_TAG(T) {{icp_reduce_kernel<1, T, false>, icp_reduce_kernel<1, T, true>}, {icp_reduce_kernel<2, T, false>, icp_reduce_kernel<2, T, true>}, \
                    {icp_reduce_kernel<4, T, false>, icp_reduce_kernel<4, T, true>}}
static constexpr IcpKernel kIcpKernels[7][3][2] = {ICP_TAG(0), ICP_TAG(1), ICP_TAG(2), {}, ICP_TAG(4), ICP_TAG(5), ICP_TAG(6)};
#undef ICP_TAG
static void launch_plain_or_timed(IcpKernel kernel, dim3 grid, dim3 block, unsigned lds, hipStream_t s, hipEvent_t ev0, hipEvent_t ev1, const IcpArgs& args,
                              const RgbArgs& ra, int n_icp_blocks)
{
    if (!ev0 && !ev1) kernel<<<grid, block, lds, s>>>(args, ra, n_icp_blocks);
    else hipExtLaunchKernelGGL(kernel, grid, block, lds, s, ev0, ev1, 0, args, ra, n_icp_blocks);
}

static void launch_icp_rgbres(hipStream_t s, IcpLaunch cfg, const IcpArgs& args_in, const RgbArgs& ra_in, bool icp, bool rgb, int n, int level,
                              hipEvent_t ev0, hipEvent_t ev1)
{
    if (cfg.ppt == 0) cfg.ppt = (level == 0 && !cfg.gram) ? 2 : 1;
    const int res_per_block = cfg.threads * (ra_in.compact ? 4 : 1);
    const int n_res_blocks = rgb ? ((icp ? args_in.cols * args_in.rows : ra_in.cols * ra_in.rows) + res_per_block - 1) / res_per_block : 0;
    IcpArgs args = with_cdiv(args_in);
    RgbArgs ra = ra_in; ra.cdiv = make_idiv(ra.cols);
    const int N = ((args.row_end > 0 ? args.row_end : args.rows) - args.row_begin) * args.cols;
    const int per_block = cfg.threads * cfg.ppt;
    const int nlog = (N + per_block - 1) / per_block;
    const int full = icp ? ((nlog + 7) / 8) * 8 : 0;
    int blocks[kMaxBatch];
    for (int m = 0; m < n; m++) {
        IcpModelArgs& ma = args.m[m];
        const bool ok = icp && ma.cull && ma.box_blocks > 0 && !cfg.gram && (!(args.flags & 1) || (args.flags & 2)) && args.row_end == 0 && ma.row_end == 0;
        ma.box_blocks = ok ? (ma.box_blocks < full ? ((ma.box_blocks + 7) / 8) * 8 : full) : 0;
        blocks[m] = ok ? ma.box_blocks : full;
    }
    int res_compact[kMaxBatch] = {};
    for (int m = 0; m < n && n_res_blocks > 0; m++) {
        RgbModelArgs& rm = ra.m[m];
        if (!ra.compact || !rm.res_range || rm.res_blocks <= 0 || rm.res_blocks > n_res_blocks) rm.res_blocks = n_res_blocks;
        else res_compact[m] = rm.res_blocks;
        if (!ra.compact) rm.res_range = nullptr;
    }
    if (cfg.shape) {
        const int L = 2 - args.occ_shift;
        for (int m = 0; m < n; m++) {
            LaunchShape* sh = cfg.shape[m];
            if (!sh || L < 0 || L > 2) continue;
            if (args.flags & 1) sh->icp_err = args.m[m].box_blocks; else sh->icp[L] = args.m[m].box_blocks;
            sh->res[L] = res_compact[m];
        }
    }
    int total = 0, slot = 0, n_icp_blocks = 0;
    auto add = [&](int m, bool residual, int count) {
        total += ((count + 7) / 8) * 8;
        args.slot_end[slot] = total; args.slot_desc[slot] = (unsigned char)(m | (residual ? kResidualSlot : 0)); slot++;
        if (!residual) n_icp_blocks += count;
    };
    for (int pass = 0; pass < 2 && icp; pass++) for (int m = 0; m < n; m++) if ((args.m[m].box_blocks > 0) == (pass == 0)) add(m, false, blocks[m]);
    for (int m = 0; m < n && n_res_blocks > 0; m++) add(m, true, ra.m[m].res_blocks);
    args.slots_used = slot;
    for (; slot < kMaxSlots; slot++) { args.slot_end[slot] = 0x7fffffff; args.slot_desc[slot] = 0; }
    const dim3 grid(total);
#ifdef CF_ABLATE
    g_last_icp_args = args; g_last_n_icp_blocks = n_icp_blocks; g_last_grid = (int)grid.x;
#endif
    const unsigned lds = cfg.gram ? (unsigned)(cfg.threads / 64) * kGramWaveDwords * sizeof(int) : 0u;
    const int tag = (level == 0 ? 0 : level == 1 ? 1 : 2) + (n > 1 ? 4 : 0), ppt_index = cfg.ppt == 4 ? 2 : cfg.ppt == 2 ? 1 : 0;
    static_assert(kIcpKernels[3][0][0] == nullptr && kIcpKernels[2][2][1] && kIcpKernels[4][0][0], "tags are level (0..2) or level + 4: row 3 is never looked up");
    launch_plain_or_timed(kIcpKernels[tag][ppt_index][cfg.gram ? 1 : 0], grid, dim3(cfg.threads), lds, s, ev0, ev1, args, ra, n_icp_blocks);
}

void launch_icp_level(hipStream_t s, IcpLaunch cfg, const IcpArgs& args, int n, int level, hipEvent_t ev0, hipEvent_t ev1)
{
    launch_icp_rgbres(s, cfg, args, RgbArgs{}, true, false, n, level, ev0, ev1);
}

void launch_so3_prealign(hipStream_t s, const TrackerStates& states, So3Sync* so3_syncs, int n, bool so3, int first_level, const RgbPrepBatch* prep)
{
    const int gx = so3 ? 8 * kSo3Blocks : 1;
    static const RgbPrepBatch none{};
    const int prep_bx = prep ? prep->m[0].L.blk_end[2] : 0;
    so3_prealign_kernel<<<gx * n + prep_bx * n, 256, 0, s>>>(states, so3_syncs, so3 ? 1 : 0, first_level, gx, gx * n, prep ? *prep : none, prep_bx);
}

void launch_rgb_slot_step(hipStream_t s, const RgbArgs& ra, So3Sync* so3_syncs, int n, int mode, int icp_fix, int next_level, int last_of_level)
{
    const int N = ra.cols * ra.rows, n_slots = (N + ra.slot_px - 1) / ra.slot_px;
    if (mode == 2) {
        const int n_quads = (n_slots + 1) / 2;
        rgb_step_solve_kernel<<<8 * n_quads * ((n + 7) / 8), 256, 0, s>>>(ra, so3_syncs, n_slots, n_quads, make_idiv(n_quads > 1 ? n_quads : 2), n,
                                                                         icp_fix, next_level, last_of_level);
    } else rgb_slot_step_kernel<<<dim3(n_slots, n), 256, 0, s>>>(ra, n_slots);
}
void launch_rgb_records_residual(hipStream_t s, IcpLaunch cfg, const RgbArgs& ra_in, int n, int level)
{
    RgbArgs ra = ra_in; ra.compact = 1; ra.slot_px = cfg.threads * 4;
    IcpArgs a{}; a.cols = ra.cols; a.rows = ra.rows;
    launch_icp_rgbres(s, cfg, a, ra, false, true, n, level, nullptr, nullptr);
}

bool launch_gn_track(hipStream_t s, IcpLaunch cfg, const TrackerStates& states, So3Sync* so3_syncs, const GnHook* hook, const IcpArgs icp_args[3],
                     const RgbArgs rgb_args[3], int n, int width, int height, bool so3, bool pyramid, bool fast_odom, bool rgb, bool icp, int mode,
                     ProfSink* prof, OdomDev* const* h_states, const RgbPrepBatch* prep)
{
    int iterations[3];
    iterations[0] = fast_odom ? 3 : 10;
    iterations[1] = pyramid ? 5 : 0;
    iterations[2] = pyramid ? 4 : 0;
    int first_level = 2;
    while (first_level > 0 && iterations[first_level] == 0) first_level--;
    launch_so3_prealign(s, states, so3_syncs, n, so3, first_level, prep);
    GnArgs gn{};
    gn.icp_gram = cfg.gram;
    gn.slot_px = cfg.threads * 4;
    for (int m = 0; m < n; m++) {
        gn.od[m] = const_cast<OdomDev*>(icp_args[0].m[m].st);
        gn.icp_acc[m] = icp_args[0].m[m].acc;
        gn.rgb_acc[m] = rgb_args[0].m[m].rgb_acc;
        gn.od_host[m] = h_states ? h_states[m] : nullptr;
    }
    const bool slots = mode != 0;
    bool any_culled = false;
    for (int m = 0; m < n; m++) any_culled = any_culled || (icp_args[0].m[m].cull && icp_args[0].m[m].err);
    const bool err_aside = icp && any_culled;
    bool hook_failed = false;
    for (int i = 2; i >= 0; i--) {
        const int N = (width >> i) * (height >> i);
        for (int j = 0; j < iterations[i]; j++) {
            const bool last_of_level = (j == iterations[i] - 1);
            int next_level = i;
            if (last_of_level) {
                next_level = i - 1;
                while (next_level >= 0 && iterations[next_level] == 0) next_level--;
            }
            RgbArgs ra = rgb_args[i];
            ra.compact = slots ? 1 : 0;
            ra.slot_px = cfg.threads * 4;
            {
                const bool timed = prof && prof->enabled && i == 0 && prof->used + 4 <= prof->capacity;
                IcpArgs a = icp_args[i];
                a.flags = (i == 0 && last_of_level) ? (err_aside ? 3 : 1) : 0;
                launch_icp_rgbres(s, cfg, a, ra, icp, rgb, n, i, timed ? prof->events[prof->used] : nullptr,
                                  timed ? prof->events[prof->used + 1] : nullptr);
                if (timed) {
                    prof->used += 2;
                    prof->bytes += (uint64_t)N * ((icp ? 24 + 24 * (uint64_t)n : 0) + (rgb ? (slots ? kRgbResidualBytesCompact : kRgbResidualBytes) * (uint64_t)n : 0));
                    prof->launches += 1;
                }
            }
            const bool err_here = err_aside && i == 0 && last_of_level;
            const bool err_with_step = err_here && rgb && slots && mode != 2;
            if (err_here && !err_with_step) {
                icp_error_surface_kernel<<<dim3((N + 255) / 256, n), 256, 0, s>>>(with_cdiv(icp_args[i]));
            }
            if (hook && hook->fn) {
                FoldArgs fa{}; int nf = 0;
                for (int m = 0; m < n; m++) if (hook->split[m]) fa.acc[nf++] = gn.icp_acc[m];
                if (nf) acc_fold_kernel<<<nf, 64, 0, s>>>(fa);
                for (int m = 0; m < n; m++)
                    if (hook->split[m] && hook->fn(hook->user, 0, gn.icp_acc[m], 32, (void*)s) != 0) hook_failed = true;
            }
            if (rgb && mode == 2) {
                launch_rgb_slot_step(s, ra, so3_syncs, n, 2, cfg.gram ? -1 : kFixICP, next_level, last_of_level ? 1 : 0);
                continue;
            }
            if (rgb) {
                if (slots) {
                    const int n_slots = (N + ra.slot_px - 1) / ra.slot_px;
                    if (err_with_step) rgb_slot_step_err_kernel<<<dim3(n_slots + (N + 255) / 256, n), 256, 0, s>>>(ra, n_slots, with_cdiv(icp_args[i]));
                    else launch_rgb_slot_step(s, ra, so3_syncs, n, 1, 0, next_level, last_of_level ? 1 : 0);
                }
                else rgb_step_kernel<<<dim3((N + 255) / 256, n), 256, 0, s>>>(ra);
            }
            gn_solve_kernel<<<n, 256, 0, s>>>(gn, next_level, last_of_level ? 1 : 0);
        }
    }
    return !hook_failed;
}

float replay_icp_level0(hipStream_t s, IcpLaunch cfg, const IcpArgs& a0, const RgbArgs& r0, int n, int slots, int ablate, int reps, hipEvent_t e0, hipEvent_t e1)
{
    IcpArgs a = a0; a.flags = ablate << 8;
    RgbArgs ra = r0; ra.compact = slots ? 1 : 0; ra.slot_px = cfg.threads * 4;
    for (int i = 0; i < 3; i++) launch_icp_rgbres(s, cfg, a, ra, true, true, n, 0, nullptr, nullptr);
    (void)hipEventRecord(e0, s);
    for (int i = 0; i < reps; i++) launch_icp_rgbres(s, cfg, a, ra, true, true, n, 0, nullptr, nullptr);
    (void)hipEventRecord(e1, s);
    (void)hipStreamSynchronize(s);
    float ms = 0; (void)hipEventElapsedTime(&ms, e0, e1);
    return ms * 1000.f / reps;
}

#ifdef CF_ABLATE
void trace_so3_dump(hipStream_t s)
// ... 140 lines not shown
```

co_fusion_amd/csrc/track_so3_dev.h:

```cpp
#pragma once
#include "track_prep_dev.h"
#include "track_sums_dev.h"

namespace cf {

__device__ __forceinline__ void screen_box(const float* lo, const float* hi, const float* Rb, const float* tb, const float* Rcurr, const float* tcurr,
                                           cf_cam intr, float distThres, int W, int H, int lane, int (&out)[4], float (&zout)[2])
{
    const float finf = __int_as_float(0x7f800000);
    zout[0] = -finf; zout[1] = finf;
    if (!(lo[0] <= hi[0])) { out[0] = 1; out[1] = 1; out[2] = 0; out[3] = 0; return; }
    const float m = distThres * 1.01f + 1e-3f;
    const float px = (lane & 1) ? hi[0] + 3.f : lo[0] - 3.f, py = (lane & 2) ? hi[1] + 3.f : lo[1] - 3.f;
    const float znear = lo[2] - m, pz = (lane & 4) ? hi[2] + m : znear;
    const float cx_ = (px - intr.cx) / intr.fx * pz, cy_ = (py - intr.cy) / intr.fy * pz;
    const float dx = (Rb[0] * cx_ + Rb[1] * cy_ + Rb[2] * pz + tb[0]) - tcurr[0];
    const float dy = (Rb[3] * cx_ + Rb[4] * cy_ + Rb[5] * pz + tb[1]) - tcurr[1];
    const float dz = (Rb[6] * cx_ + Rb[7] * cy_ + Rb[8] * pz + tb[2]) - tcurr[2];
    const float xc = Rcurr[0] * dx + Rcurr[3] * dy + Rcurr[6] * dz;
    const float yc = Rcurr[1] * dx + Rcurr[4] * dy + Rcurr[7] * dz;
    const float zc = Rcurr[2] * dx + Rcurr[5] * dy + Rcurr[8] * dz;
    const float u = intr.fx * xc / zc + intr.cx, v = intr.fy * yc / zc + intr.cy;
    const bool bad = !(znear > 0.05f) || !(zc > 0.05f) || !is_finite(u) || !is_finite(v);
    float u0 = u, u1 = u, v0 = v, v1 = v, z0 = zc, z1 = zc;
#pragma unroll
    for (int o = 1; o < 8; o <<= 1) {
        u0 = fminf(u0, __shfl_xor(u0, o, 64)); u1 = fmaxf(u1, __shfl_xor(u1, o, 64));
        v0 = fminf(v0, __shfl_xor(v0, o, 64)); v1 = fmaxf(v1, __shfl_xor(v1, o, 64));
        z0 = fminf(z0, __shfl_xor(z0, o, 64)); z1 = fmaxf(z1, __shfl_xor(z1, o, 64));
    }
    if (__any(bad)) { out[0] = 0; out[1] = 0; out[2] = W - 1; out[3] = H - 1; return; }
    zout[0] = z0 - (1e-3f + 1e-3f * fabsf(z0)); zout[1] = z1 + (1e-3f + 1e-3f * fabsf(z1));
    const float fw = (float)(W + 16), fh = (float)(H + 16);
    out[0] = (int)floorf(fminf(fmaxf(u0, -16.f), fw)) - 3; out[1] = (int)floorf(fminf(fmaxf(v0, -16.f), fh)) - 3;
    out[2] = (int)ceilf(fminf(fmaxf(u1, -16.f), fw)) + 3; out[3] = (int)ceilf(fminf(fmaxf(v1, -16.f), fh)) + 3;
}

__device__ __forceinline__ void so3_gradient(const uint8_t* __restrict__ img, int cols, int x, int y, float& gx, float& gy)
{
    const float actu = (float)img[y * cols + x];
    float back = (float)img[y * cols + x - 1], fore = (float)img[y * cols + x + 1];
    gx = ((back + actu) / 2.0f) - ((fore + actu) / 2.0f);
    back = (float)img[(y - 1) * cols + x]; fore = (float)img[(y + 1) * cols + x];
    gy = ((back + actu) / 2.0f) - ((fore + actu) / 2.0f);
}

__device__ __forceinline__ void so3_pass(const uint8_t* __restrict__ lastImage, const uint8_t* __restrict__ nextImage,
                                         const m33& B, const m33& Ki, const float* __restrict__ krlr, int cols, int rows,
                                         unsigned long long (*lds)[16], unsigned long long* totals, int block, int blocks)
{
    constexpr float lim = (float)(1 << ((50 - kFixSO3) / 2));
    constexpr float scale = (float)(1 << kFixSO3);
    const int N = cols * rows, T = blockDim.x;
    unsigned long long acc[16];
#pragma unroll
    for (int k = 0; k < 16; k++) acc[k] = 0;
    const float a = krlr[0], b = krlr[1], c = krlr[2], d = krlr[3], e = krlr[4], f = krlr[5], g = krlr[6], h = krlr[7],
                ii = krlr[8];
    for (int k = block * T + threadIdx.x; k < N; k += blocks * T) {
        const int y = k / cols, x = k - y * cols;
        const f3 unwarped = {(float)x, (float)y, 1.0f};
        const f3 warped = mul(B, unwarped);
        const int wx = f2i_rn(warped.x / warped.z), wy = f2i_rn(warped.y / warped.z);
        if (!(wx >= 1 && wx < cols - 1 && wy >= 1 && wy < rows - 1 && x >= 1 && x < cols - 1 && y >= 1 && y < rows - 1))
            continue;
        float gnx, gny, glx, gly;
        so3_gradient(nextImage, cols, wx, wy, gnx, gny);
        so3_gradient(lastImage, cols, x, y, glx, gly);
        const float gx = (gnx + glx) / 2.0f, gy = (gny + gly) / 2.0f;
        const f3 point = mul(Ki, unwarped);
        const float z2 = point.z * point.z;
        const f3 left = {((point.z * (d * gy + a * gx)) - (gy * g * y) - (gx * g * x)) / z2,
                         ((point.z * (e * gy + b * gx)) - (gy * h * y) - (gx * h * x)) / z2,
                         ((point.z * (f * gy + c * gx)) - (gy * ii * y) - (gx * ii * x)) / z2};
        const f3 jac = cross(left, point);
        const float row[4] = {jac.x, jac.y, jac.z, -((float)nextImage[wy * cols + wx] - (float)lastImage[y * cols + x])};
        double r[4], rs[4];
#pragma unroll
        for (int q = 0; q < 4; q++) { r[q] = (double)clamp_row(row[q], lim); rs[q] = (double)(clamp_row(row[q], lim) * scale); }
#pragma unroll
        for (int p = 0; p < 3; p++)
#pragma unroll
            for (int q = 0; q < 4; q++)
                if (q >= p)
                    acc[4 * p - (p * (p - 1)) / 2 + (q - p)] += (unsigned long long)__double_as_longlong(fma(rs[p], r[q], kMagic)) - kMagicBits;
        acc[9] += (unsigned long long)__double_as_longlong(fma(rs[3], r[3], kMagic)) - kMagicBits;
        acc[10] += 1;
    }
    const int lane = threadIdx.x & 63, wave = threadIdx.x >> 6;
    const unsigned long long v = wave_reduce16_u64(acc, lane);
    if ((lane & 3) == 0) lds[wave][lane >> 2] = v;
    __syncthreads();
    if (threadIdx.x < 16) {
        unsigned long long t = 0;
        for (int w = 0; w < (T >> 6); w++) t += lds[w][threadIdx.x];
        totals[threadIdx.x] = t;
    }
    __syncthreads();
}

__device__ inline void so3_unpack(const unsigned long long* t, float A[9], float b[3], float residual[2])
{
    int shift = 0;
    for (int i = 0; i < 3; ++i)
        for (int j = i; j < 4; ++j) {
            const float value = fix_to_f32((long long)t[shift++], kFixSO3);
            if (j == 3) b[i] = value;
            else A[j * 3 + i] = A[i * 3 + j] = value;
        }
    residual[0] = fix_to_f32((long long)t[9], kFixSO3);
    residual[1] = (float)(long long)t[10];
}

__device__ inline void k_matrix(cf_cam c, double K[9])
{
    for (int i = 0; i < 9; i++) K[i] = 0;
    K[0] = c.fx; K[4] = c.fy; K[2] = c.cx; K[5] = c.cy; K[8] = 1;
}

__device__ inline void prepare_iteration(OdomDev* od, int level)
{
    double K[9], Kinv[9], Rt[16];
    k_matrix(cam_level(od->intr, level), K);
    inv33<double>(K, Kinv);
    inv44_affine(od->resultRt, Rt);
    const double R[9] = {Rt[0], Rt[1], Rt[2], Rt[4], Rt[5], Rt[6], Rt[8], Rt[9], Rt[10]};
    double tmp[9], KRK[9];
    mul33<double>(K, R, tmp);
    mul33<double>(tmp, Kinv, KRK);
    for (int k = 0; k < 9; k++) od->krkInv[k] = (float)KRK[k];
    const double tv[3] = {Rt[3], Rt[7], Rt[11]};
    for (int r = 0; r < 3; r++) od->kt[r] = (float)(K[r * 3 + 0] * tv[0] + K[r * 3 + 1] * tv[1] + K[r * 3 + 2] * tv[2]);
}

__global__ void __launch_bounds__(1024) so3_step_kernel(const uint8_t* __restrict__ lastImage,
                                                        const uint8_t* __restrict__ nextImage, m33 B, m33 Ki, m33 krlr,
                                                        int cols, int rows, unsigned long long* __restrict__ out16)
{
    __shared__ unsigned long long lds[16][16];
    __shared__ unsigned long long totals[16];
    so3_pass(lastImage, nextImage, B, Ki, krlr.m, cols, rows, lds, totals, blockIdx.x, gridDim.x);
    if (threadIdx.x < 16) out16[threadIdx.x] = totals[threadIdx.x];
}

#ifdef CF_ABLATE
__device__ unsigned long long g_so3_trace[12][8];
#define OSTAMP(it, k) do { if (lead && by == 0 && threadIdx.x == 0) g_so3_trace[it][k] = wall_clock64(); } while (0)
#else
#define OSTAMP(it, k) do {} while (0)
#endif
__global__ void __launch_bounds__(256) so3_prealign_kernel(const TrackerStates ts, So3Sync* __restrict__ syncs, int do_so3,
                                                           int first_level, int gx, int so3_blocks, const RgbPrepBatch prep, int prep_bx)
{
    if ((int)blockIdx.x >= so3_blocks) {
        const int r = (int)blockIdx.x - so3_blocks, m = r / prep_bx;
        rgb_prep_body(prep.m[m], r - m * prep_bx);
        return;
    }
    const int by = (int)blockIdx.x / gx, bxx = (int)blockIdx.x - by * gx;
    OdomDev* const god = ts.dev[by];
    So3Sync* sync = syncs + by;
    __shared__ OdomDev s_od;
    __shared__ unsigned long long lds[16][16];
    __shared__ unsigned long long totals[16];
    __shared__ float s_basis[9], s_kinv[9], s_krlr[9];
    __shared__ int s_done;
    __shared__ double s_resultR[9];
    __shared__ double s_K[9], s_Kinv[9];
    __shared__ float s_Rlr[9];
    __shared__ float s_lastError, s_lastCount;
    __shared__ double s_lastResultR[9];
    __shared__ float s_jtj[9], s_jtr[3], s_delta[3], s_fws[15];
    __shared__ int s_iws[3];
    const bool one_xcd = do_so3 && gx > 1;
    if (one_xcd && (bxx & 7) != (by & 7)) return;
    const int bx = one_xcd ? (bxx >> 3) : bxx;
    const bool lead = bx == 0;
    const unsigned G = one_xcd ? (unsigned)gx >> 3 : (unsigned)gx;
    {
        static_assert(sizeof(OdomDev) % 4 == 0, "OdomDev is staged as 32-bit words");
        constexpr int kWords = (int)(sizeof(OdomDev) / 4);
        const unsigned* __restrict__ src = reinterpret_cast<const unsigned*>(ts.host[by]);
        constexpr int kPer = (kWords + 255) / 256;
        unsigned w[kPer];
#pragma unroll
        for (int q = 0; q < kPer; q++) w[q] = ((int)threadIdx.x + 256 * q < kWords) ? src[threadIdx.x + 256 * q] : 0u;
#pragma unroll
        for (int q = 0; q < kPer; q++) if ((int)threadIdx.x + 256 * q < kWords) reinterpret_cast<unsigned*>(&s_od)[threadIdx.x + 256 * q] = w[q];
        __syncthreads();
        if (lead) for (int k = threadIdx.x; k < kWords; k += 256) reinterpret_cast<unsigned*>(god)[k] = reinterpret_cast<const unsigned*>(&s_od)[k];
        __syncthreads();
    }
    const OdomDev* const od = &s_od;
    const int L = 2, cols = od->width >> L, rows = od->height >> L;
    if (threadIdx.x == 0) {
        for (int k = 0; k < 9; k++) { s_resultR[k] = (k % 4 == 0) ? 1.0 : 0.0; s_lastResultR[k] = s_resultR[k]; s_Rlr[k] = (k % 4 == 0) ? 1.f : 0.f; }
        k_matrix(cam_level(od->intr, L), s_K);
        inv33<double>(s_K, s_Kinv);
        s_lastError = 3.402823466e+38F / 2; s_lastCount = 3.402823466e+38F / 2;
        s_done = 0;
        if (lead) { god->stats.so3_iterations = 0; god->stats.last_so3_error = 0; god->stats.last_so3_count = 0; }
    }
    __syncthreads();
    if (do_so3) {
        const uint8_t* __restrict__ lastNext = od->lastNextImage[L];
        const uint8_t* __restrict__ next = od->nextImage[L];
        OSTAMP(11, 0);
        for (int it = 0; it < 10; it++) {
            OSTAMP(it, 0);
            if (threadIdx.x == 0) {
                double tmp[9], H[9];
                mul33<double>(s_K, s_resultR, tmp);
                mul33<double>(tmp, s_Kinv, H);
                for (int k = 0; k < 9; k++) { s_basis[k] = (float)H[k]; s_kinv[k] = (float)s_Kinv[k]; s_krlr[k] = (float)tmp[k]; }
            }
            __syncthreads();
            m33 B, Ki;
            for (int k = 0; k < 9; k++) { B.m[k] = s_basis[k]; Ki.m[k] = s_kinv[k]; }
            OSTAMP(it, 1);
            so3_pass(lastNext, next, B, Ki, s_krlr, cols, rows, lds, totals, bx, (int)G);
            OSTAMP(it, 2);
            if (G > 1) {
                if (threadIdx.x < 64) {
                    unsigned long long* slot = sync->acc[it];
                    if (threadIdx.x < 11 && totals[threadIdx.x] != 0)
                        __hip_atomic_fetch_add(&slot[threadIdx.x], totals[threadIdx.x], __ATOMIC_RELAXED, __HIP_MEMORY_SCOPE_WORKGROUP);
                    asm volatile("s_waitcnt vmcnt(0)" ::: "memory");
                    if (threadIdx.x == 0) {
                        __hip_atomic_fetch_add(&sync->arrive, 1u, __ATOMIC_RELAXED, __HIP_MEMORY_SCOPE_WORKGROUP);
                        const unsigned target = (unsigned)(it + 1) * G;
                        unsigned spins = 0;
                        while (l2_read_u32(&sync->arrive) < target) {
                            if (++spins > (1u << 22)) { god->stats.fault = 1; break; }
                            __builtin_amdgcn_s_sleep(1);
                        }
                    }
                    __builtin_amdgcn_wave_barrier();
                    if (threadIdx.x < 16) totals[threadIdx.x] = l2_read_u64(&slot[threadIdx.x]);
                }
                __syncthreads();
            }
            OSTAMP(it, 3);
            if (threadIdx.x == 0) {
                float jtj[9], jtr[3], residual[2];
                so3_unpack(totals, jtj, jtr, residual);
                if (lead) god->stats.so3_iterations = it + 1;
                float err = sqrtf(residual[0]) / residual[1];
                float cnt = residual[1];
                if (err < s_lastError && (double)fabsf(s_lastError - cnt) < 0.001) {
                    s_done = 1;
                } else if ((double)err > (double)s_lastError + 0.001) {
                    err = s_lastError; cnt = s_lastCount;
                    for (int k = 0; k < 9; k++) s_resultR[k] = s_lastResultR[k];
                    s_done = 1;
                } else {
                    s_lastError = err; s_lastCount = cnt;
                    for (int k = 0; k < 9; k++) s_lastResultR[k] = s_resultR[k];
                    for (int k = 0; k < 9; k++) s_jtj[k] = jtj[k];
                    for (int k = 0; k < 3; k++) s_jtr[k] = jtr[k];
                    ldlt_solve<float, 3>(s_jtj, s_jtr, s_delta, 1.17549435e-38f, s_fws, s_iws);
                    const float delta[3] = {s_delta[0], s_delta[1], s_delta[2]};
                    const double dd[3] = {delta[0], delta[1], delta[2]};
                    double rotUpdate[9];
                    rodrigues(dd, rotUpdate);
                    float ru[9], nr[9];
                    for (int k = 0; k < 9; k++) ru[k] = (float)rotUpdate[k];
                    mul33<float>(ru, s_Rlr, nr);
                    for (int k = 0; k < 9; k++) { s_Rlr[k] = nr[k]; s_resultR[k] = nr[k]; }
                }
                if (lead) { god->stats.last_so3_error = err; god->stats.last_so3_count = cnt; }
            }
            __syncthreads();
            OSTAMP(it, 4);
            if (s_done) break;
        }
        OSTAMP(11, 1);
        if (G > 1 && threadIdx.x == 0) {
            if (__hip_atomic_fetch_add(&sync->depart, 1u, __ATOMIC_RELAXED, __HIP_MEMORY_SCOPE_WORKGROUP) == G - 1) {
                for (int it = 0; it < 10; it++)
                    for (int w = 0; w < 16; w++) sync->acc[it][w] = 0;
                sync->arrive = 0; sync->depart = 0;
            }
        }
    }
    if (lead && threadIdx.x < 64) {
        const int lane = threadIdx.x;
        unsigned key = 0;
        if (od->cull && lane < 6) { key = od->aabb_acc[lane]; od->aabb_acc[lane] = 0; }
        const float val = lane < 3 ? fkey_inv(~key) : fkey_inv(key);
        float lo[3], hi[3];
#pragma unroll
        for (int k = 0; k < 3; k++) { lo[k] = __shfl(val, k, 64); hi[k] = __shfl(val, 3 + k, 64); }
        if (__shfl((int)key, 3, 64) == 0) { lo[0] = 1.f; hi[0] = 0.f; }
        int ib[4] = {0, 0, od->width - 1, od->height - 1};
        float zb[2] = {-__int_as_float(0x7f800000), __int_as_float(0x7f800000)};
        if (od->cull) screen_box(lo, hi, od->box_R, od->box_t, od->Rcurr, od->tcurr, od->intr, od->distThres, od->width, od->height, lane, ib, zb);
        if (lane == 0) {
            for (int k = 0; k < 3; k++) { god->box_lo[k] = lo[k]; god->box_hi[k] = hi[k]; }
            for (int k = 0; k < 4; k++) god->stats.cull_box[k] = ib[k];
            god->cull_z[0] = zb[0]; god->cull_z[1] = zb[1];
        }
    }
    if (lead && threadIdx.x == 0) {
// ... 14 lines not shown
```

co_fusion_amd/host/CoFusion.cpp:

```cpp
#include "CoFusion.h"
#include "ExportWriter.h"

#include <algorithm>
#include <chrono>

#include <cmath>
#include <cstdio>
#include <cstdlib>
#include <cstring>
#include <condition_variable>
#include <exception>
#include <functional>
#include <mutex>
#include <stdexcept>
#include <thread>

namespace cofusion {

PhaseTimes& phaseTimes() { static thread_local PhaseTimes t; return t; }
namespace {
struct PhaseTimer {
    int id; std::chrono::steady_clock::time_point t0 = std::chrono::steady_clock::now();
    explicit PhaseTimer(int i) : id(i) {}
    ~PhaseTimer() { phaseTimes().ms[id] += std::chrono::duration<double, std::milli>(std::chrono::steady_clock::now() - t0).count(); }
// ... 75 lines not shown
}
}

int CoFusion::rcclSumHost(int64_t* buf, uint64_t n)
{
    if (n > rcclStageWords) {
        if (rcclStage) cf_free(ctx, rcclStage);
        rcclStage = nullptr; rcclStageWords = 0;
        void* p = nullptr;
        const uint64_t words = n < 4096 ? 4096 : n;
        if (cf_malloc(ctx, words * 8, &p) != CF_OK) return -1;
        rcclStage = static_cast<int64_t*>(p); rcclStageWords = words;
    }
    if (cf_memcpy_h2d(ctx, rcclStage, buf, n * 8) != CF_OK) return -1;
    if (cf_rccl_allreduce(ctx, rcclStage, n, 0, cf_get_stream(ctx)) != CF_OK) return -1;
    return cf_memcpy_d2h(ctx, buf, rcclStage, n * 8) == CF_OK ? 0 : -1;
}

void CoFusion::initRccl(const void* id128)
{
    check(ctx, cf_rccl_init(ctx, id128, dist.rank, dist.world), "cf_rccl_init");
    dist.allreduce_dev = rccl_sum_device; dist.user_dev = ctx;
    dist.allreduce_i64 = rccl_sum_host; dist.user = this;
}

void CoFusion::broadcast(void* dev_buf, uint64_t bytes, int root)
{
    check(ctx, cf_rccl_broadcast(ctx, dev_buf, bytes, root, cf_get_stream(ctx)), "cf_rccl_broadcast");
}

Model::Model(cf_ctx* c, unsigned char id_, float confidenceThresh, bool enableFillIn, int maxSurfels, float maxDepth_, bool owned_)
    : ctx(c), pose(Mat4f::identity()), lastPose(Mat4f::identity()), confidenceThreshold(confidenceThresh), maxDepth(maxDepth_), id(id_),
      fillIn(enableFillIn), owned(owned_)
{
    if (!owned) return;
    check(ctx, cf_model_create(ctx, maxSurfels, &model), "cf_model_create");
    check(ctx, cf_odom_create(ctx, &odom), "cf_odom_create");
    if (!enableFillIn) check(ctx, cf_odom_set_culling(odom, 1), "cf_odom_set_culling");
    void* p = nullptr;
    uint64_t bytes = 0;
    void* indexMap = nullptr;
    check(ctx, cf_model_buffer(model, 0, &indexMap, &bytes), "cf_model_buffer");
    check(ctx, cf_malloc(ctx, bytes, &p), "cf_malloc");
    icpError = static_cast<float*>(p);
}
Model::~Model()
{
    if (icpError) cf_free(ctx, icpError);
    if (odom) cf_odom_destroy(odom);
    if (model) cf_model_destroy(model);
}
unsigned Model::lastCount() const
{
    uint32_t c = 0;
    if (owned) cf_model_count(model, &c);
    return c;
}
void Model::initialise(const uint8_t* rgba, const float* depthRaw, const float* depthFiltered, int time, float maxD)
{
    if (!owned) return;
    check(ctx, cf_model_initialise(model, rgba, depthRaw, depthFiltered, time, maxD), "cf_model_initialise");
}
static const void* mbuf(cf_ctx* ctx, cf_model* m, int which)
{
    void* p = nullptr;
    check(ctx, cf_model_buffer(m, which, &p, nullptr), "cf_model_buffer");
    return p;
}
const float* Model::vertexConfProjection() const { return owned ? static_cast<const float*>(mbuf(ctx, model, 5)) : nullptr; }

void Model::trackingInputs(bool doFillIn, bool frameToFrameRGB, const float*& v, const float*& n, const uint8_t*& img) const
{
    if (doFillIn) {
        v = static_cast<const float*>(mbuf(ctx, model, 8)); n = static_cast<const float*>(mbuf(ctx, model, 9));
        img = static_cast<const uint8_t*>(mbuf(ctx, model, 10));
    } else {
        v = static_cast<const float*>(mbuf(ctx, model, 5)); n = static_cast<const float*>(mbuf(ctx, model, 6));
        img = static_cast<const uint8_t*>(mbuf(ctx, model, (frameToFrameRGB && allowsFillIn()) ? 10 : 4));
    }
}
void Model::bindFrameMaps(const float* const depthPyr[3], float depthCutoff, Model* frameOwner)
{
    if (frameOwner == this) {
        check(ctx, cf_odom_init_icp(odom, depthPyr, depthCutoff), "initICP");
    } else {
        check(ctx, cf_odom_share_frame_maps(odom, frameOwner->odom), "share_frame_maps");
    }
}
void Model::initICP(bool doFillIn, bool frameToFrameRGB, const float* const depthPyr[3], float depthCutoff, const uint8_t* rgba,
                    Model* frameOwner)
{
    if (!owned) return;
    const float* v; const float* n; const uint8_t* img;
    trackingInputs(doFillIn, frameToFrameRGB, v, n, img);
    check(ctx, cf_odom_init_icp_model(odom, v, n, pose.m), "initICPModel");
    check(ctx, cf_odom_init_rgb_model(odom, img), "initRGBModel");
    bindFrameMaps(depthPyr, depthCutoff, frameOwner);
    check(ctx, cf_odom_init_rgb(odom, rgba), "initRGB");
}
float Model::computeFusionWeight(float weightMultiplier) const { return cf_fusion_weight(pose.m, lastPose.m, weightMultiplier); }

void Model::fuse(int time, const uint8_t* rgba, const uint8_t* mask, const float* depthRaw, const float* depthFiltered, float depthCutoff,
                 float weightMultiplier)
{
    if (!owned) return;
    const float md = depthCutoff < maxDepth ? depthCutoff : maxDepth;
    check(ctx, cf_model_fuse(model, pose.m, time, rgba, mask, depthRaw, depthFiltered, md, computeFusionWeight(weightMultiplier), (int)id),
          "cf_model_fuse");
}
void Model::clean(int time, int timeDelta, float , const float* depthFiltered, const uint8_t* mask, float outlierCoeff)
{
    if (!owned) return;
    check(ctx, cf_model_clean(model, pose.m, time, confidenceThreshold, outlierCoeff, timeDelta, depthFiltered, mask, (int)id, nullptr), "cf_model_clean");
}
void Model::predictIndices(int time, float depthCutoff, int timeDelta)
{
    if (!owned) return;
    if (shards > 1) check(ctx, cf_model_predict_indices_sharded(model, pose.m, time, depthCutoff, timeDelta, shard, shards), "predictIndices (sharded)");
    else check(ctx, cf_model_predict_indices(model, pose.m, time, depthCutoff, timeDelta), "predictIndices");
}
void Model::combinedPredict(float depthCutoff, int time, int maxTime, int timeDelta)
{
    if (!owned) return;
    check(ctx, cf_model_combined_predict(model, pose.m, depthCutoff, confidenceThreshold, time, maxTime, timeDelta), "combinedPredict");
}
void Model::performFillIn(const uint8_t* rgba, const float* depthFiltered, bool frameToFrameRGB, bool lost)
{
    if (fillIn && owned) check(ctx, cf_model_perform_fill_in(model, rgba, depthFiltered, lost ? 1 : 0, (lost || frameToFrameRGB) ? 1 : 0), "performFillIn");
}
void Model::prefetchFillRatio()
{
    if (owned && allowsFillIn()) check(ctx, cf_model_prefetch_fill_ratio(model), "prefetch_fill_ratio");
}
bool Model::requiresFillIn(float ratio)
{
    if (!allowsFillIn() || !owned) return false;
    int out = 0;
    check(ctx, cf_model_requires_fill_in(model, ratio, &out), "requiresFillIn");
    return out != 0;
}
const uint32_t* Model::fillRatioDevice() const
{
    if (!allowsFillIn() || !owned) return nullptr;
    const uint32_t* counts = nullptr;
    check(ctx, cf_model_fill_ratio_device(model, &counts), "fill_ratio_device");
    return counts;
}
std::vector<float> Model::downloadMap() const
{
    if (!owned) return {};
    const unsigned n = lastCount();
    std::vector<float> out((size_t)n * 12);
    uint32_t c = 0;
    check(ctx, cf_model_download_map(model, out.data(), n, &c), "downloadMap");
    return out;
}

static const int SPIX = 16;

Segmentation::Segmentation(cf_ctx* c, int w, int h, const Distributed* d) : ctx(c), width(w), height(h), dist(d)
{
    check(ctx, cf_seg_create(ctx, &seg), "cf_seg_create");
    memset(gtMapping, 0, sizeof(gtMapping));
    if (dist && dist->active()) {
        void* p = nullptr;
        check(ctx, cf_malloc(ctx, (uint64_t)w * h * 16, &p), "cf_malloc");
        zeroImage = static_cast<float*>(p);
// ... 1420 lines not shown
```

co_fusion_amd/lib.py:

```python
from __future__ import annotations

import ctypes as C
import os
import subprocess

_HERE = os.path.dirname(os.path.abspath(__file__))
_LIB_DIR = os.environ.get("CF_LIB_DIR") or os.path.join(_HERE, "lib")
LIB_PATH = os.environ.get("CF_HIP_LIB") or os.path.join(_LIB_DIR, "libcofusion_hip.so")

SYMBOLS = [
    "cf_create", "cf_destroy", "cf_last_error", "cf_set_stream", "cf_use_own_stream", "cf_get_stream", "cf_synchronize", "cf_fork", "cf_main", "cf_join", "cf_join_lane", "cf_thread_lane", "cf_mark", "cf_event_wait_host", "cf_fork_after", "cf_malloc",
    "cf_free", "cf_memcpy_h2d", "cf_memcpy_d2h", "cf_malloc_host", "cf_free_host", "cf_memcpy_h2d_async", "cf_memcpy_d2h_async", "cf_memcpy_d2d_async", "cf_rgb_to_rgba", "cf_create_vmap", "cf_create_nmap", "cf_copy_maps", "cf_resize_map",
    "cf_transform_maps", "cf_vertices_to_depth", "cf_pyrdown_gauss_f32", "cf_pyrdown_gauss_u8",
    "cf_rgba_to_intensity", "cf_sobel", "cf_project_cloud", "cf_icp_step", "cf_icp_step_band", "cf_rgb_residual", "cf_rgb_step",
    "cf_so3_step", "cf_gn_solve_step", "cf_so3_prealign_step", "cf_rgb_records_step","cf_odom_create", "cf_odom_destroy", "cf_odom_init_icp_model", "cf_odom_init_rgb_model",
    "cf_odom_init_rgb", "cf_odom_init_models_batch", "cf_odom_init_models_batch_frames", "cf_odom_init_models_batch_select", "cf_model_fill_ratio_device", "cf_odom_init_first_rgb", "cf_odom_init_icp", "cf_odom_init_icp_maps", "cf_odom_get_incremental_transformation",
    "cf_odom_track_batch_async", "cf_odom_fetch_result", "cf_odom_get_covariance", "cf_odom_bind_frame_maps", "cf_odom_share_frame_maps", "cf_odom_set_culling", "cf_odom_set_band", "cf_set_collective", "cf_model_predict_indices_sharded", "cf_odom_buffer",
    "cf_bilateral", "cf_model_create", "cf_model_destroy", "cf_model_initialise", "cf_model_count",
    "cf_model_predict_indices", "cf_model_index_keys", "cf_model_index_resolve", "cf_model_combined_predict", "cf_model_predict_inactive", "cf_model_synthesize_depth", "cf_model_prefetch_fill_ratio", "cf_model_perform_fill_in", "cf_model_requires_fill_in",
    "cf_model_fuse", "cf_model_clean", "cf_models_frame_passes", "cf_models_preindex", "cf_model_download_map", "cf_model_upload_map", "cf_model_buffer",
    "cf_set_extent_culling", "cf_model_extents_unknown",
    "cf_redetect_score", "cf_redetect_timing", "cf_relabel",
    "cf_redetect_frame_moments", "cf_redetect_model_moments", "cf_redetect_register_step", "cf_redetect_register",
    "cf_fusion_weight", "cf_seg_create", "cf_seg_destroy", "cf_seg_slic", "cf_seg_crf", "cf_seg_sums", "cf_seg_infer", "cf_seg_early", "cf_seg_run_batch", "cf_seg_fetch", "cf_seg_publish_poses", "cf_seg_fetch_poses",
    "cf_seg_labels", "cf_seg_buffer", "cf_seg_create_masks", "cf_seg_masks", "cf_seg_masks_batch", "cf_seg_new_mask_value",
    "cf_depth_pyramid", "cf_set_icp_launch", "cf_set_icp_arith", "cf_get_icp_arith", "cf_set_gn_mode", "cf_profile_enable", "cf_profile_read", "cf_odom_bench_icp", "cf_odom_level0_visited", "cf_odom_last_launch_shape",
    "cf_rccl_unique_id", "cf_rccl_init", "cf_rccl_allreduce", "cf_rccl_broadcast", "cf_rccl_info", "cf_rccl_destroy",
    "cf_render_create", "cf_render_destroy", "cf_render", "cf_render_palette",
    "cf_ferns_table", "cf_ferns_create", "cf_ferns_destroy", "cf_ferns_get_table", "cf_ferns_encode", "cf_ferns_search", "cf_ferns_append", "cf_ferns_add_async",
    "cf_ferns_relocalise", "cf_ferns_count", "cf_ferns_download", "cf_ferns_last_search",
    "cf_frame_decoder_create", "cf_frame_decoder_destroy", "cf_frame_decoder_slot", "cf_frame_decoder_submit", "cf_frame_decoder_acquire", "cf_frame_decoder_timing",
    "cf_frame_decoder_enable_images", "cf_frame_decoder_image_slot", "cf_frame_decoder_submit_images", "cf_frame_decoder_acquire_mask", "cf_frame_decoder_image_timing",
    "cf_png_encoder_create", "cf_png_encoder_destroy", "cf_png_encoder_submit", "cf_png_encoder_acquire", "cf_png_encoder_timing",
    "cf_deform_create", "cf_deform_destroy", "cf_deform_default_thresholds", "cf_deform_sample", "cf_deform_set_nodes", "cf_deform_weights", "cf_deform_assemble",
    "cf_deform_iterate", "cf_deform_optimise", "cf_deform_apply", "cf_deform_apply_poses", "cf_deform_download", "cf_deform_weights_device",
    "cf_deform_create_sized", "cf_deform_assemble_local", "cf_deform_iterate_local", "cf_deform_optimise_local",
    "cf_deform_enable_relative", "cf_deform_set_relative", "cf_deform_set_relative_device", "cf_deform_pick_relative", "cf_deform_download_relative",
    "cf_deform_download_out", "cf_deform_bench_relative_y",
    "cf_ferns_gate_async", "cf_ferns_gate_wait", "cf_ferns_constraints", "cf_ferns_find_frame", "cf_ferns_constraint_buffers", "cf_ferns_keyframe_buffers",
    "cf_local_loop_create", "cf_local_loop_destroy", "cf_local_loop_constraints_async", "cf_local_loop_wait", "cf_local_loop_constraint_buffers",
    "cf_local_loop_target_times",
    "cf_mesh_create", "cf_mesh_destroy", "cf_mesh_default_grid", "cf_mesh_accumulate", "cf_mesh_extract", "cf_mesh_download", "cf_mesh_grid_download",
    "cf_mesh_extract_grid", "cf_mesh_timing",
]


def build(verbose: bool = False) -> str:
    cmd = ["make", "-C", os.path.join(_HERE, "csrc"), "-j8"]
    if not verbose:
        cmd.insert(1, "-s")
    subprocess.check_call(cmd)
    cmd = ["make", "-C", os.path.join(_HERE, "host")]
    if not verbose:
        cmd.insert(1, "-s")
    subprocess.check_call(cmd)
    return LIB_PATH


HOST_LIB_PATH = os.path.join(_LIB_DIR, "libcofusion.so")
HOST_SYMBOLS = [
    "cofusion_default_config", "cofusion_create", "cofusion_destroy", "cofusion_last_error", "cofusion_set_stream",
    "cofusion_process_frame", "cofusion_process_frame_device", "cofusion_process_frame_device_masked", "cofusion_group_process_frames_device_masked", "cofusion_num_models", "cofusion_tick", "cofusion_model_info",
    "cofusion_model_download", "cofusion_model_icp_stats", "cofusion_model_cull_box", "cofusion_model_level0_visited", "cofusion_model_tracking_inputs", "cofusion_mask_device", "cofusion_context", "cofusion_set_crf", "cofusion_set_seg_early",
    "cofusion_save_ply", "cofusion_export_poses", "cofusion_set_export_segmentation", "cofusion_klg_open", "cofusion_klg_next", "cofusion_klg_set_reference_compatible", "cofusion_klg_close",
    "cofusion_klg_create", "cofusion_klg_write", "cofusion_klg_finish", "cofusion_debug_phase_ms", "cofusion_set_allreduce", "cofusion_set_allreduce_device", "cofusion_group_create", "cofusion_group_destroy", "cofusion_group_size", "cofusion_group_sequence", "cofusion_group_set_stream", "cofusion_group_process_frames", "cofusion_group_process_frames_device", "cofusion_rccl_unique_id", "cofusion_init_rccl", "cofusion_broadcast", "cofusion_model_owned", "cofusion_is_lost",
    "cofusion_render", "cofusion_render_device", "cofusion_set_export_views", "cofusion_set_export_async", "cofusion_export_flush", "cofusion_export_stats", "cofusion_set_relocalisation", "cofusion_reloc_stats", "cofusion_deform_background", "cofusion_set_loop_closure", "cofusion_loop_stats", "cofusion_set_local_loop_closure", "cofusion_local_loop_stats",
    "cofusion_set_relative_constraints", "cofusion_add_relative_constraints", "cofusion_relative_constraints", "cofusion_relative_stats", "cofusion_local_closure_download",
    "cofusion_set_redetection", "cofusion_redetect_stats", "cofusion_redetect_last", "cofusion_num_inactive_models",
    "cofusion_set_redetection_search", "cofusion_redetect_search_last",
    "cofusion_klg_player_open", "cofusion_klg_player_next", "cofusion_klg_player_process", "cofusion_klg_player_rewind", "cofusion_klg_player_set_limits", "cofusion_klg_player_close",
    "cofusion_jpeg_front", "cofusion_jpeg_finish_host", "cofusion_klg_prefetch_open", "cofusion_klg_prefetch_next", "cofusion_klg_prefetch_rewind", "cofusion_klg_prefetch_close",
    "cofusion_image_reader_open", "cofusion_image_reader_next", "cofusion_image_reader_rewind", "cofusion_image_reader_close",
    "cofusion_image_player_open", "cofusion_image_player_next", "cofusion_image_player_process", "cofusion_image_player_rewind", "cofusion_image_player_set_limits",
    "cofusion_image_player_times", "cofusion_image_player_close",
    "cofusion_image_prefetch_open", "cofusion_image_prefetch_next", "cofusion_image_prefetch_rewind", "cofusion_image_prefetch_close",
    "cofusion_save_mesh", "cofusion_model_mesh", "cofusion_set_mesh_max_voxels", "cofusion_write_mesh_ply",
    "cofusion_png_decode", "cofusion_png_finish_host", "cofusion_exr_decode", "cofusion_exr_finish_host", "cofusion_ppm_decode",
]
_host = None


def load_host() -> C.CDLL:
    global _host
    if _host is None:
        load()
        if not os.path.exists(HOST_LIB_PATH):
            raise RuntimeError(f"{HOST_LIB_PATH} is missing: run __graft_entry__.build()")
        _host = C.CDLL(HOST_LIB_PATH)
        _host.cofusion_last_error.restype = C.c_char_p
        _host.cofusion_mask_device.restype = C.c_void_p
        _host.cofusion_context.restype = C.c_void_p
        _host.cofusion_group_sequence.restype = C.c_void_p
    return _host


_lib = None


def load() -> C.CDLL:
    global _lib
# ... 19 lines not shown
```

include/cofusion_hip.h:

```cpp
#ifndef COFUSION_HIP_H_
#define COFUSION_HIP_H_

#include <stdint.h>

#ifdef __cplusplus
extern "C" {
#endif

#define CF_OK 0
#define CF_EINVAL (-1)
#define CF_EHIP (-2)
#define CF_ENOMEM (-3)
#define CF_ESTATE (-4)

#define CF_NUM_PYRS 3
#define CF_SE3_WORDS 32
#define CF_SO3_WORDS 16
#define CF_FIX_ICP 32
#define CF_FIX_RGB_MAX 32
static inline int CF_FIX_RGB_BITS(float sigma)
{
    union { float f; uint32_t u; } v;
    int F;
    if (sigma == -1.0f || !(sigma >= 2.0f)) return 8;
// ... 44 lines not shown
int cf_synchronize(cf_ctx *ctx);
int cf_fork(cf_ctx *ctx, int lane);
int cf_main(cf_ctx *ctx);
int cf_join(cf_ctx *ctx);
int cf_join_lane(cf_ctx *ctx, int lane);
int cf_thread_lane(cf_ctx *ctx, int lane);
int cf_mark(cf_ctx *ctx, int slot);
int cf_event_wait_host(cf_ctx *ctx, int slot);
int cf_fork_after(cf_ctx *ctx, int lane, int slot);
int cf_malloc(cf_ctx *ctx, uint64_t bytes, void **dptr);
int cf_free(cf_ctx *ctx, void *dptr);
int cf_memcpy_h2d(cf_ctx *ctx, void *dst, const void *src, uint64_t bytes);
int cf_memcpy_d2h(cf_ctx *ctx, void *dst, const void *src, uint64_t bytes);
int cf_malloc_host(cf_ctx *ctx, uint64_t bytes, void **hptr);
int cf_free_host(cf_ctx *ctx, void *hptr);
int cf_memcpy_h2d_async(cf_ctx *ctx, void *dst, const void *src_pinned, uint64_t bytes);
int cf_memcpy_d2h_async(cf_ctx *ctx, void *dst_pinned, const void *src, uint64_t bytes);
int cf_memcpy_d2d_async(cf_ctx *ctx, void *dst, const void *src, uint64_t bytes);
int cf_rgb_to_rgba(cf_ctx *ctx, const uint8_t *rgb_dev, int cols, int rows, uint8_t *rgba_dev);

int cf_create_vmap(cf_ctx *ctx, const float *depth, int cols, int rows, cf_cam intr, float depth_cutoff, float *vmap);
int cf_create_nmap(cf_ctx *ctx, const float *vmap, int cols, int rows, float *nmap);
int cf_copy_maps(cf_ctx *ctx, const float *vertex4, const float *normal4, int cols, int rows, float *vmap, float *nmap);
int cf_resize_map(cf_ctx *ctx, const float *in, int in_cols, int in_rows, float *out, int normalize);
int cf_transform_maps(cf_ctx *ctx, float *vmap, float *nmap, int cols, int rows, const float R[9], const float t[3]);
int cf_vertices_to_depth(cf_ctx *ctx, const float *vertex4, int cols, int rows, float cutoff, float *depth);
int cf_pyrdown_gauss_f32(cf_ctx *ctx, const float *src, int src_cols, int src_rows, float *dst);
int cf_pyrdown_gauss_u8(cf_ctx *ctx, const uint8_t *src, int src_cols, int src_rows, uint8_t *dst);
int cf_rgba_to_intensity(cf_ctx *ctx, const uint8_t *rgba, int cols, int rows, uint8_t *dst);
int cf_sobel(cf_ctx *ctx, const uint8_t *src, int cols, int rows, int16_t *dx, int16_t *dy);
int cf_project_cloud(cf_ctx *ctx, const float *depth, int cols, int rows, cf_cam intr_level, float *cloud3);

int cf_icp_step(cf_ctx *ctx, const float Rcurr[9], const float tcurr[3], const float *vmap_curr,
                const float *nmap_curr, const float Rprev_inv[9], const float tprev[3], cf_cam intr,
                const float *vmap_g_prev, const float *nmap_g_prev, float dist_thres, float angle_thres,
                int cols, int rows, float *A_host, float *b_host, float *residual_host, int64_t *sums_host,
                float *err_surface);
int cf_icp_step_band(cf_ctx *ctx, const float Rcurr[9], const float tcurr[3], const float *vmap_curr,
                     const float *nmap_curr, const float Rprev_inv[9], const float tprev[3], cf_cam intr,
                     const float *vmap_g_prev, const float *nmap_g_prev, float dist_thres, float angle_thres,
                     int cols, int rows, int row_begin, int row_end, float *A_host, float *b_host,
                     float *residual_host, int64_t *sums_host, float *err_surface);
int cf_rgb_residual(cf_ctx *ctx, float min_scale, const int16_t *dIdx, const int16_t *dIdy, const float *last_depth,
                    const float *next_depth, const uint8_t *last_image, const uint8_t *next_image,
                    cf_dataterm *corres, float max_depth_delta, const float kt[3], const float krkinv[9],
                    int cols, int rows, int *sigma_sum_host, int *count_host);
int cf_rgb_step(cf_ctx *ctx, const cf_dataterm *corres, float sigma, const float *cloud3, float fx, float fy,
                const int16_t *dIdx, const int16_t *dIdy, float sobel_scale, int cols, int rows, float *A_host,
                float *b_host, int64_t *sums_host);
int cf_so3_step(cf_ctx *ctx, const uint8_t *last_image, const uint8_t *next_image, const float image_basis[9],
                const float kinv[9], const float krlr[9], int cols, int rows, float *A_host, float *b_host,
                float *residual_host, int64_t *sums_host);

typedef struct {
    int rgb_only, pyramid, fast_odom, so3;
    float icp_weight;
} cf_track_opts;
typedef struct {
    float last_icp_error, last_icp_count, last_rgb_error, last_rgb_count, last_so3_error, last_so3_count;
    double lastA[36], lastb[6];
    int so3_iterations;
    int fault;
    int cull_box[4];
} cf_track_stats;

int cf_odom_create(cf_ctx *ctx, cf_odom **out);
void cf_odom_destroy(cf_odom *od);
int cf_odom_init_icp_model(cf_odom *od, const float *pred_vertex4, const float *pred_normal4, const float pose[16]);
int cf_odom_init_rgb_model(cf_odom *od, const uint8_t *pred_rgba);
int cf_odom_init_rgb(cf_odom *od, const uint8_t *rgba);
int cf_odom_init_first_rgb(cf_odom *od, const uint8_t *rgba);
int cf_odom_init_models_batch(cf_ctx *ctx, cf_odom *const *ods, int n, const float *const *pred_vertex4,
                              const float *const *pred_normal4, const uint8_t *const *pred_rgba, const float *const *poses ,
                              const uint8_t *frame_rgba);
int cf_odom_init_models_batch_frames(cf_ctx *ctx, cf_odom *const *ods, int n, const float *const *pred_vertex4,
                                     const float *const *pred_normal4, const uint8_t *const *pred_rgba, const float *const *poses ,
                                     const uint8_t *const *frame_rgba );
int cf_odom_init_models_batch_select(cf_ctx *ctx, cf_odom *const *ods, int n, const float *const *pred_vertex4,
                                     const float *const *pred_normal4, const uint8_t *const *pred_rgba,
                                     const float *const *alt_vertex4, const float *const *alt_normal4, const uint8_t *const *alt_rgba,
                                     const uint32_t *const *fill_counts, float ratio, const float *const *poses ,
                                     const uint8_t *const *frame_rgba );
int cf_odom_init_icp(cf_odom *od, const float *const depth_pyr[CF_NUM_PYRS], float depth_cutoff);
int cf_odom_get_incremental_transformation(cf_odom *od, float trans[3], float rot[9], const cf_track_opts *opts,
                                           float *icp_err_surface, cf_track_stats *stats);
int cf_odom_track_batch_async(cf_ctx *ctx, cf_odom *const *ods, int n, const float *const *poses_in ,
                              const cf_track_opts *opts, float *const *icp_err_surfaces );
int cf_odom_fetch_result(cf_odom *od, float trans[3], float rot[9], cf_track_stats *stats);
int cf_odom_get_covariance(const cf_track_stats *stats, double cov[36]);

typedef struct {
    cf_cam intr;
    int32_t width, height;
    int32_t icp, rgb, rgbOnly;
    float icpWeight;
    float Rprev[9], tprev[3], Rprev_inv[9], Rcurr[9], tcurr[3];
    double resultRt[16];
    float krkInv[9], kt[3];
    float lastRGBError;
    int32_t level_done, solves;
    float residual[2];
    float cull_z[2];
    float pose_inv[16];
    cf_track_stats stats;
} cf_gn_state;
typedef struct {
    int64_t icp_acc[64 * 32];
    int64_t rgb_acc[64 * 32];
    cf_gn_state state;
    cf_gn_state twin;
    uint32_t hot[48];
} cf_gn_system;
int cf_gn_solve_step(cf_ctx *ctx, int n, cf_gn_system *systems, int next_level, int last_of_level, int icp_fix);
typedef struct {
    const uint8_t *last_next_image;
    const uint8_t *next_image;
    cf_gn_state state_in;
    cf_gn_state state_out;
    uint32_t hot[48];
    uint64_t sync[418];
} cf_so3_system;
int cf_so3_prealign_step(cf_ctx *ctx, int n, cf_so3_system *systems, int do_so3, int first_level);
typedef struct {
    const uint8_t *cand;
    const float *next_depth, *last_depth;
    const uint8_t *last_image, *next_image;
    const float *cloud;
    const int16_t *dIdx, *dIdy;
    int32_t no_counts;
    int32_t ranged;
    uint32_t res_range[2];
    int32_t res_blocks;
    uint64_t *records;
    uint32_t *slot_counts;
    int64_t count_seed[64], sigma_seed[64];
    int64_t count_total, sigma_total;
    int64_t rgb_sums[32];
    cf_gn_state state;
    cf_gn_state twin;
    uint32_t hot[48];
} cf_rgb_system;
int cf_rgb_records_step(cf_ctx *ctx, int n, cf_rgb_system *systems, int cols, int rows, float max_depth_delta, float sobel_scale,
                        float fx, float fy, int next_level, int last_of_level);
int cf_odom_level0_visited(cf_odom *od, uint64_t *icp_pixels, uint64_t *residual_pixels);
int cf_odom_last_launch_shape(cf_odom *od, int icp_blocks[3], int residual_blocks[3], int *icp_blocks_err);
int cf_odom_set_culling(cf_odom *od, int on);
typedef int (*cf_collective_fn)(void *user, int op, void *dev_buf, uint64_t words, void *hip_stream);
int cf_set_collective(cf_ctx *ctx, cf_collective_fn fn, void *user);
int cf_odom_set_band(cf_odom *od, int row_begin, int row_end, int add_counts);
#define CF_RCCL_ID_BYTES 128
int cf_rccl_unique_id(void *id128);
int cf_rccl_init(cf_ctx *ctx, const void *id128, int rank, int world);
int cf_rccl_allreduce(cf_ctx *ctx, void *dev_buf, uint64_t words, int op, void *hip_stream);
int cf_rccl_broadcast(cf_ctx *ctx, void *dev_buf, uint64_t bytes, int root, void *hip_stream);
int cf_rccl_info(const cf_ctx *ctx, int *rank, int *world, int *rccl_version);
int cf_rccl_destroy(cf_ctx *ctx);
int cf_odom_bind_frame_maps(cf_odom *od, const float *const vmaps[CF_NUM_PYRS], const float *const nmaps[CF_NUM_PYRS]);
int cf_odom_share_frame_maps(cf_odom *od, cf_odom *owner);
int cf_odom_buffer(cf_odom *od, int which, int level, void **dptr, uint64_t *bytes);
int cf_odom_init_icp_maps(cf_odom *od, const float *vertex4, const float *normal4);
int cf_depth_pyramid(cf_ctx *ctx, const float *depth_filtered, int cols, int rows, float *l1, float *l2);

int cf_bilateral(cf_ctx *ctx, const float *depth, int cols, int rows, float maxD, float *out);

int cf_model_create(cf_ctx *ctx, int max_surfels, cf_model **out);
void cf_model_destroy(cf_model *m);
// ... 415 lines not shown
```

Before: 963.2.

## Defer frame-map build into fused track-head kernel on side lane, stage SO3 image in LDS

```diff
diff --git a/co_fusion_amd/api.py b/co_fusion_amd/api.py
--- a/co_fusion_amd/api.py
+++ b/co_fusion_amd/api.py
@@ -386,10 +386,11 @@
     def init_first_rgb(self, rgba):
         self.ctx._check(self.ctx.lib.cf_odom_init_first_rgb(self.h, _p(rgba)))
 
-    def init_icp(self, depth_pyr, cutoff):
+    def init_icp(self, depth_pyr, cutoff, deferred=False):
         arr = (C.c_void_p * 3)(*[d.data_ptr() for d in depth_pyr])
         self._keep = depth_pyr
-        self.ctx._check(self.ctx.lib.cf_odom_init_icp(self.h, arr, C.c_float(cutoff)))
+        fn = self.ctx.lib.cf_odom_init_icp_deferred if deferred else self.ctx.lib.cf_odom_init_icp
+        self.ctx._check(fn(self.h, arr, C.c_float(cutoff)))
 
     def init_icp_maps(self, vertex4, normal4):
         self.ctx._check(self.ctx.lib.cf_odom_init_icp_maps(self.h, _p(vertex4), _p(normal4)))
diff --git a/co_fusion_amd/csrc/cabi.hip b/co_fusion_amd/csrc/cabi.hip
--- a/co_fusion_amd/csrc/cabi.hip
+++ b/co_fusion_amd/csrc/cabi.hip
@@ -19,6 +19,13 @@
         HIPCHK(ctx, hipStreamCreateWithFlags(&ctx->lanes[lane], hipStreamNonBlocking));
         HIPCHK(ctx, hipEventCreateWithFlags(&ctx->lane_done[lane], hipEventDisableTiming));
     }
+    return CF_OK;
+}
+int track_side_lane(cf_ctx* ctx, SideLane* out)
+{
+    if (int r = lane_ready(ctx, cf_ctx::kTrackLane)) return r;
+    if (!ctx->track_fork) HIPCHK(ctx, hipEventCreateWithFlags(&ctx->track_fork, hipEventDisableTiming));
+    *out = SideLane{ctx->lanes[cf_ctx::kTrackLane], ctx->track_fork, ctx->lane_done[cf_ctx::kTrackLane]};
     return CF_OK;
 }
 static void leave_lane(cf_ctx* ctx)
@@ -100,6 +107,7 @@
         if (ctx->lane_done[i]) (void)hipEventDestroy(ctx->lane_done[i]);
     }
     if (ctx->fork_point) (void)hipEventDestroy(ctx->fork_point);
+    if (ctx->track_fork) (void)hipEventDestroy(ctx->track_fork);
     for (int i = 0; i < cf_ctx::kMarks; i++) if (ctx->marks[i]) (void)hipEventDestroy(ctx->marks[i]);
     if (ctx->own_stream) (void)hipStreamDestroy(ctx->own_stream);
     delete ctx;
diff --git a/co_fusion_amd/csrc/cabi_odom.hip b/co_fusion_amd/csrc/cabi_odom.hip
--- a/co_fusion_amd/csrc/cabi_odom.hip
+++ b/co_fusion_amd/csrc/cabi_odom.hip
@@ -197,11 +197,9 @@
     return CF_OK;
 }
 
-int cf_odom_init_icp(cf_odom* od, const float* const depth_pyr[CF_NUM_PYRS], float depth_cutoff)
-{
-    if (!od || !depth_pyr) return CF_EINVAL;
-    cf_ctx* ctx = od->ctx; hipStream_t s = ctx->stream;
-    const int W = ctx->cfg.width, H = ctx->cfg.height;
+static FrameMapsArgs frame_maps_args(cf_odom* od, const float* const depth_pyr[CF_NUM_PYRS], float depth_cutoff)
+{
+    cf_ctx* ctx = od->ctx;
     FrameMapsArgs a{};
     a.cutoff = depth_cutoff;
     for (int i = 0; i < CF_NUM_PYRS; ++i) {
@@ -210,9 +208,27 @@
         a.fx_inv[i] = 1.f / il.fx; a.fy_inv[i] = 1.f / il.fy; a.cx[i] = il.cx; a.cy[i] = il.cy;
         od->ext_vmap_curr[i] = nullptr; od->ext_nmap_curr[i] = nullptr; od->ext_zrange[i] = nullptr;
     }
-    launch_frame_maps(s, a, W, H);
+    od->maps_owner = nullptr;
+    return a;
+}
+
+int cf_odom_init_icp(cf_odom* od, const float* const depth_pyr[CF_NUM_PYRS], float depth_cutoff)
+{
+    if (!od || !depth_pyr) return CF_EINVAL;
+    cf_ctx* ctx = od->ctx;
+    od->maps_pending = false;
+    launch_frame_maps(ctx->stream, frame_maps_args(od, depth_pyr, depth_cutoff), ctx->cfg.width, ctx->cfg.height);
     od->zrange_valid = true;
     LAUNCHCHK(ctx);
+    return CF_OK;
+}
+
+int cf_odom_init_icp_deferred(cf_odom* od, const float* const depth_pyr[CF_NUM_PYRS], float depth_cutoff)
+{
+    if (!od || !depth_pyr) return CF_EINVAL;
+    od->pending_maps = frame_maps_args(od, depth_pyr, depth_cutoff);
+    od->maps_pending = true;
+    od->zrange_valid = true;
     return CF_OK;
 }
 
@@ -221,6 +237,7 @@
     if (!od || !vertex4 || !normal4) return CF_EINVAL;
     cf_ctx* ctx = od->ctx; hipStream_t s = ctx->stream;
     const int W = ctx->cfg.width, H = ctx->cfg.height;
+    od->maps_pending = false; od->maps_owner = nullptr;
     HIPCHK(ctx, hipMemcpyAsync(od->vmaps_tmp, vertex4, sizeof(float) * 4 * (size_t)W * H, hipMemcpyDeviceToDevice, s));
     for (int i = 0; i < CF_NUM_PYRS; ++i) { od->ext_vmap_curr[i] = nullptr; od->ext_nmap_curr[i] = nullptr; od->ext_zrange[i] = nullptr; }
     launch_copy_maps(s, vertex4, normal4, W, H, od->vmap_curr[0], od->nmap_curr[0]);
@@ -233,6 +250,18 @@
     return CF_OK;
 }
 
+}
+int flush_frame_maps(cf_odom* od)
+{
+    if (!od || !od->maps_pending) return CF_OK;
+    cf_ctx* ctx = od->ctx;
+    od->maps_pending = false;
+    launch_frame_maps(ctx->stream, od->pending_maps, ctx->cfg.width, ctx->cfg.height);
+    LAUNCHCHK(ctx);
+    return CF_OK;
+}
+extern "C" {
+
 int cf_odom_set_culling(cf_odom* od, int on)
 {
     if (!od) return CF_EINVAL;
@@ -257,6 +286,7 @@
 {
     if (!od) return CF_EINVAL;
     for (int i = 0; i < CF_NUM_PYRS; i++) { od->ext_vmap_curr[i] = vmaps ? vmaps[i] : nullptr; od->ext_nmap_curr[i] = nmaps ? nmaps[i] : nullptr; od->ext_zrange[i] = nullptr; }
+    od->maps_owner = nullptr;
     return CF_OK;
 }
 int cf_odom_share_frame_maps(cf_odom* od, cf_odom* owner)
@@ -265,6 +295,7 @@
     for (int i = 0; i < CF_NUM_PYRS; i++) {
         od->ext_vmap_curr[i] = owner->cur_vmap(i); od->ext_nmap_curr[i] = owner->cur_nmap(i); od->ext_zrange[i] = owner->cur_zrange(i);
     }
+    od->maps_owner = owner->maps_source();
     return CF_OK;
 }
 
@@ -299,6 +330,9 @@
     if (!od || level < 0 || level >= CF_NUM_PYRS || !dptr) return CF_EINVAL;
     const size_t n = (size_t)(od->ctx->cfg.width >> level) * (od->ctx->cfg.height >> level);
     void* p = nullptr; size_t b = 0;
+    if (which == 0 || which == 1 || which == 14) {
+        if (int r = flush_frame_maps(which == 14 ? od : od->maps_source())) return r;
+    }
     if (which == 0 && !od->ext_vmap_curr[level]) od->zrange_valid = false;
     switch (which) {
         case 0: p = (void*)od->cur_vmap(level); b = n * 12; break;
diff --git a/co_fusion_amd/csrc/cabi_steps.hip b/co_fusion_amd/csrc/cabi_steps.hip
--- a/co_fusion_amd/csrc/cabi_steps.hip
+++ b/co_fusion_amd/csrc/cabi_steps.hip
@@ -418,7 +418,7 @@
         s->lastNextImage[2] = systems[k].last_next_image; s->nextImage[2] = systems[k].next_image;
         states.dev[k] = buf.d_states + k; states.host[k] = s;
     }
-    launch_so3_prealign(ctx->stream, states, ctx->d_so3_sync, n, do_so3 != 0, first_level, nullptr);
+    launch_so3_prealign(ctx->stream, states, ctx->d_so3_sync, n, do_so3 != 0, first_level);
     LAUNCHCHK(ctx);
     HIPCHK(ctx, hipMemcpyAsync(back.data(), buf.d_states, sizeof(OdomDev) * n, hipMemcpyDeviceToHost, ctx->stream));
     for (int k = 0; k < n; k++)
diff --git a/co_fusion_amd/csrc/cabi_track.hip b/co_fusion_amd/csrc/cabi_track.hip
--- a/co_fusion_amd/csrc/cabi_track.hip
+++ b/co_fusion_amd/csrc/cabi_track.hip
@@ -235,6 +235,7 @@
     if (ctx->icp_arith == CF_ICP_ARITH_REFERENCE) {
         for (int m = 0; m < n; m++)
             if (ods[m]->band_end > 0) { ctx->set_error("the reference-order arithmetic (cf_set_icp_arith 2) does not split a tracker's reductions over GPUs"); return CF_ESTATE; }
+        for (int m = 0; m < n; m++) if (int r = flush_frame_maps(ods[m]->maps_source())) return r;
         if (int r = prepare_trackers(ctx, ods, n, poses_in, opts, err_surfaces, prep, terms.rgb, true)) return r;
         LAUNCHCHK(ctx);
         for (int m = 0; m < n; m++)
@@ -271,9 +272,23 @@
     LaunchShape* shapes[kMaxBatch];
     for (int m = 0; m < n; m++) shapes[m] = &ods[m]->launch_shape;
     IcpLaunch launch_cfg = ctx->icp_launch; launch_cfg.shape = shapes;
+    SideLane side{};
+    bool aside = prep_fused && !ctx->forked && !any_split;
+#ifdef CF_HEAD_ON_STREAM
+    aside = false;
+#endif
+    if (aside) if (int r = track_side_lane(ctx, &side)) return r;
+    FrameMapsArgs head_maps{};
+    bool take_maps = false;
+    for (int m = 0; m < n; m++) {
+        cf_odom* src = ods[m]->maps_source();
+        if (!src || !src->maps_pending) continue;
+        if (prep_fused && !take_maps) { head_maps = src->pending_maps; src->maps_pending = false; take_maps = true; }
+        else if (int r = flush_frame_maps(src)) return r;
+    }
     if (!launch_gn_track(ctx->stream, launch_cfg, states, ctx->d_so3_sync, any_split ? &hook : nullptr, icp_args, rgb_args, n,
                          ctx->cfg.width, ctx->cfg.height, opts->so3 != 0, opts->pyramid != 0, opts->fast_odom != 0, terms.rgb, terms.icp, ctx->gn_mode, prof,
-                         h_states, prep_fused ? &prep : nullptr)) {
+                         h_states, prep_fused ? &prep : nullptr, aside ? &side : nullptr, take_maps ? &head_maps : nullptr)) {
         ctx->set_error("tracking: the registered collective failed inside the Gauss-Newton loop");
         return CF_ESTATE;
     }
diff --git a/co_fusion_amd/csrc/cf_host.h b/co_fusion_amd/csrc/cf_host.h
--- a/co_fusion_amd/csrc/cf_host.h
+++ b/co_fusion_amd/csrc/cf_host.h
@@ -43,6 +43,8 @@
     hipStream_t lanes[kLanes]{};
     hipEvent_t lane_done[kLanes]{};
     hipEvent_t fork_point = nullptr;
+    hipEvent_t track_fork = nullptr;
+    static constexpr int kTrackLane = 6;
     static constexpr int kMarks = 64;
     hipEvent_t marks[kMarks]{};
     bool mark_set[kMarks]{};
@@ -69,6 +71,8 @@
 };
 inline cf_cam ctx_cam(const cf_ctx* ctx) { return cf_cam{ctx->cfg.fx, ctx->cfg.fy, ctx->cfg.cx, ctx->cfg.cy}; }
 extern "C" int cf_wait_stream(cf_ctx* ctx);
+int track_side_lane(cf_ctx* ctx, cf::SideLane* out);
+int flush_frame_maps(cf_odom* od);
 #define HIPCHK(ctx, call)                                                                      \
     do {                                                                                       \
         hipError_t e_ = (call);                                                                \
@@ -123,6 +127,10 @@
     const float* cur_vmap(int l) const { return ext_vmap_curr[l] ? ext_vmap_curr[l] : vmap_curr[l]; }
     const float* cur_nmap(int l) const { return ext_nmap_curr[l] ? ext_nmap_curr[l] : nmap_curr[l]; }
     const float2* cur_zrange(int l) const { return ext_vmap_curr[l] ? ext_zrange[l] : (zrange_valid ? zrange[l] : nullptr); }
+    bool maps_pending = false;
+    cf::FrameMapsArgs pending_maps{};
+    cf_odom* maps_owner = nullptr;
+    cf_odom* maps_source() { return ext_vmap_curr[0] ? maps_owner : this; }
     float* lastDepth[3]{};
     float* nextDepth[3]{};
     bool next_depth_is_last = false;
diff --git a/co_fusion_amd/csrc/cf_kernels.h b/co_fusion_amd/csrc/cf_kernels.h
--- a/co_fusion_amd/csrc/cf_kernels.h
+++ b/co_fusion_amd/csrc/cf_kernels.h
@@ -253,18 +253,24 @@
     hipEvent_t* events; int capacity; int used; uint64_t bytes; uint64_t launches; int enabled;
 };
 
-constexpr int kSo3Blocks = 16;
+#ifndef CF_SO3_BLOCKS
+#define CF_SO3_BLOCKS 16
+#endif
+constexpr int kSo3Blocks = CF_SO3_BLOCKS;
 constexpr int kStepSubs = 16;
 struct So3Sync { unsigned long long acc[10][16]; unsigned arrive, depart;
                  unsigned step_top, pad;
                  unsigned step_sub[kStepSubs][32]; };
 struct GnHook { int (*fn)(void* user, int op, void* dev_buf, uint64_t words, void* stream); void* user; int split[kMaxBatch]; };
 struct TrackerStates { OdomDev* dev[kMaxBatch]; const OdomDev* host[kMaxBatch]; };
+struct So3Images { const uint8_t* next[kMaxBatch]; const uint8_t* last[kMaxBatch]; int cols[kMaxBatch], rows[kMaxBatch]; };
+struct SideLane { hipStream_t stream; hipEvent_t fork, done; };
 bool launch_gn_track(hipStream_t s, IcpLaunch cfg, const TrackerStates& states, So3Sync* so3_syncs ,
                      const GnHook* hook, const IcpArgs icp_args[3], const RgbArgs rgb_args[3], int n, int width, int height, bool so3,
                      bool pyramid, bool fast_odom, bool rgb, bool icp, int mode, ProfSink* prof,
                      OdomDev* const* h_states = nullptr ,
-                     const RgbPrepBatch* prep = nullptr );
+                     const RgbPrepBatch* prep = nullptr ,
+                     const SideLane* side = nullptr, const FrameMapsArgs* maps = nullptr );
 void launch_rgb_slot_step(hipStream_t s, const RgbArgs& ra, So3Sync* so3_syncs , int n, int mode, int icp_fix, int next_level, int last_of_level);
 void launch_rgb_records_residual(hipStream_t s, IcpLaunch cfg, const RgbArgs& ra, int n, int level);
 inline size_t rgb_acc_rows(size_t n0)
@@ -272,9 +278,9 @@
     const size_t slots0 = (n0 + 255) / 256, quads0 = (slots0 + 1) / 2;
     return quads0 > (size_t)kGroups ? quads0 : (size_t)kGroups;
 }
-void launch_so3_prealign(hipStream_t s, const TrackerStates& states, So3Sync* so3_syncs , int n, bool so3, int first_level,
-                         const RgbPrepBatch* prep );
+void launch_so3_prealign(hipStream_t s, const TrackerStates& states, So3Sync* so3_syncs , int n, bool so3, int first_level);
 void rgb_prep_levels(RgbPrepBatch& b, int n, int W, int H);
+void launch_track_head(hipStream_t s, const RgbPrepBatch& b, int n, const FrameMapsArgs* maps );
 float replay_icp_level0(hipStream_t s, IcpLaunch cfg, const IcpArgs& a0, const RgbArgs& r0, int n, int slots, int ablate, int reps, hipEvent_t e0, hipEvent_t e1);
 #ifdef CF_ABLATE
 void trace_so3_dump(hipStream_t s);
diff --git a/co_fusion_amd/csrc/track_prep.hip b/co_fusion_amd/csrc/track_prep.hip
--- a/co_fusion_amd/csrc/track_prep.hip
+++ b/co_fusion_amd/csrc/track_prep.hip
@@ -374,55 +374,17 @@
 }
 
 
-__global__ void __launch_bounds__(kBlock) frame_maps_kernel(const FrameMapsArgs a)
-{
-    int lb;
-    const int lv = level_of(a.L, blockIdx.x, lb);
-    const int cols = a.L.cols[lv], rows = a.L.rows[lv], N = cols * rows;
-    const int i = lb * kBlock + threadIdx.x;
-    const float* __restrict__ depth = a.depth[lv];
-    const float cutoff = a.cutoff;
-    if (a.zrange[lv]) {
-        const float inf = __int_as_float(0x7f800000);
-        const float zz = i < N ? depth[i] : 0.f;
-        const bool ok = zz != 0 && zz < cutoff;
-        float lo = ok ? zz : inf, hi = ok ? zz : -inf;
-#pragma unroll
-        for (int o = 32; o > 0; o >>= 1) { lo = fminf(lo, __shfl_xor(lo, o, 64)); hi = fmaxf(hi, __shfl_xor(hi, o, 64)); }
-        if ((threadIdx.x & 63) == 0 && i < N) a.zrange[lv][i >> 6] = make_float2(lo, hi);
-    }
-    if (i >= N) return;
-    float* __restrict__ vmap = a.vmap[lv];
-    float* __restrict__ nmap = a.nmap[lv];
-    const float fx_inv = a.fx_inv[lv], fy_inv = a.fy_inv[lv], cx = a.cx[lv], cy = a.cy[lv];
-    const int v = i / cols, u = i - v * cols;
-    const bool edge = (u == cols - 1 || v == rows - 1);
-    const float z = depth[i];
-    const float z01 = edge ? 0.f : depth[i + 1], z10 = edge ? 0.f : depth[i + cols];
-    float x00 = qnan();
-    if (z != 0 && z < cutoff) {
-        x00 = z * (u - cx) * fx_inv;
-        vmap[i] = x00;
-        vmap[i + N] = z * (v - cy) * fy_inv;
-        vmap[i + 2 * N] = z;
-    } else {
-        vmap[i] = qnan();
-    }
-    if (edge) { nmap[i] = qnan(); return; }
-    const float x01 = (z01 != 0 && z01 < cutoff) ? z01 * ((u + 1) - cx) * fx_inv : qnan();
-    const float x10 = (z10 != 0 && z10 < cutoff) ? z10 * (u - cx) * fx_inv : qnan();
-    if (!is_nan(x00) && !is_nan(x01) && !is_nan(x10)) {
-        const f3 v00 = {x00, z * (v - cy) * fy_inv, z};
-        const f3 v01 = {x01, z01 * (v - cy) * fy_inv, z01};
-        const f3 v10 = {x10, z10 * ((v + 1) - cy) * fy_inv, z10};
-        const f3 r = normalized(cross(v01 - v00, v10 - v00));
-        nmap[i] = r.x; nmap[i + N] = r.y; nmap[i + 2 * N] = r.z;
-    } else {
-        nmap[i] = qnan();
-    }
-}
+__global__ void __launch_bounds__(kBlock) frame_maps_kernel(const FrameMapsArgs a) { frame_maps_body(a, (int)blockIdx.x); }
 
 __global__ void __launch_bounds__(kBlock) rgb_prep_kernel(const RgbPrepBatch b) { rgb_prep_body(b.m[blockIdx.y], (int)blockIdx.x); }
+
+__global__ void __launch_bounds__(kBlock) track_head_kernel(const RgbPrepBatch b, int prep_bx, const FrameMapsArgs maps, int maps_bx)
+{
+    const int vb = (int)blockIdx.x;
+    if (vb < maps_bx) { frame_maps_body(maps, vb); return; }
+    const int r = vb - maps_bx, m = r / prep_bx;
+    rgb_prep_body(b.m[m], r - m * prep_bx);
+}
 
 struct MapVal { f3 p; bool have; };
 
@@ -551,6 +513,13 @@
     const Level3 L = levels3(W, H);
     for (int m = 0; m < n; m++) b.m[m].L = L;
 }
+void launch_track_head(hipStream_t s, const RgbPrepBatch& b, int n, const FrameMapsArgs* maps)
+{
+    const int prep_bx = b.m[0].L.blk_end[2];
+    FrameMapsArgs fm{};
+    if (maps) { fm = *maps; fm.L = b.m[0].L; }
+    track_head_kernel<<<(maps ? prep_bx : 0) + prep_bx * n, kBlock, 0, s>>>(b, prep_bx, fm, maps ? prep_bx : 0);
+}
 void launch_rgb_prep(hipStream_t s, RgbPrepBatch b, int n, int W, int H)
 {
     const Level3 L = levels3(W, H);
diff --git a/co_fusion_amd/csrc/track_prep_dev.h b/co_fusion_amd/csrc/track_prep_dev.h
--- a/co_fusion_amd/csrc/track_prep_dev.h
+++ b/co_fusion_amd/csrc/track_prep_dev.h
@@ -70,4 +70,52 @@
         }
     }
 }
+
+__device__ __forceinline__ void frame_maps_body(const FrameMapsArgs& a, int vb)
+{
+    int lb;
+    const int lv = level_of(a.L, vb, lb);
+    const int cols = a.L.cols[lv], rows = a.L.rows[lv], N = cols * rows;
+    const int i = lb * 256 + (int)threadIdx.x;
+    const float* __restrict__ depth = a.depth[lv];
+    const float cutoff = a.cutoff;
+    if (a.zrange[lv]) {
+        const float inf = __int_as_float(0x7f800000);
+        const float zz = i < N ? depth[i] : 0.f;
+        const bool ok = zz != 0 && zz < cutoff;
+        float lo = ok ? zz : inf, hi = ok ? zz : -inf;
+#pragma unroll
+        for (int o = 32; o > 0; o >>= 1) { lo = fminf(lo, __shfl_xor(lo, o, 64)); hi = fmaxf(hi, __shfl_xor(hi, o, 64)); }
+        if ((threadIdx.x & 63) == 0 && i < N) a.zrange[lv][i >> 6] = make_float2(lo, hi);
+    }
+    if (i >= N) return;
+    float* __restrict__ vmap = a.vmap[lv];
+    float* __restrict__ nmap = a.nmap[lv];
+    const float fx_inv = a.fx_inv[lv], fy_inv = a.fy_inv[lv], cx = a.cx[lv], cy = a.cy[lv];
+    const int v = i / cols, u = i - v * cols;
+    const bool edge = (u == cols - 1 || v == rows - 1);
+    const float z = depth[i];
+    const float z01 = edge ? 0.f : depth[i + 1], z10 = edge ? 0.f : depth[i + cols];
+    float x00 = qnan();
+    if (z != 0 && z < cutoff) {
+        x00 = z * (u - cx) * fx_inv;
+        vmap[i] = x00;
+        vmap[i + N] = z * (v - cy) * fy_inv;
+        vmap[i + 2 * N] = z;
+    } else {
+        vmap[i] = qnan();
+    }
+    if (edge) { nmap[i] = qnan(); return; }
+    const float x01 = (z01 != 0 && z01 < cutoff) ? z01 * ((u + 1) - cx) * fx_inv : qnan();
+    const float x10 = (z10 != 0 && z10 < cutoff) ? z10 * (u - cx) * fx_inv : qnan();
+    if (!is_nan(x00) && !is_nan(x01) && !is_nan(x10)) {
+        const f3 v00 = {x00, z * (v - cy) * fy_inv, z};
+        const f3 v01 = {x01, z01 * (v - cy) * fy_inv, z01};
+        const f3 v10 = {x10, z10 * ((v + 1) - cy) * fy_inv, z10};
+        const f3 r = normalized(cross(v01 - v00, v10 - v00));
+        nmap[i] = r.x; nmap[i + N] = r.y; nmap[i + 2 * N] = r.z;
+    } else {
+        nmap[i] = qnan();
+    }
 }
+}
diff --git a/co_fusion_amd/csrc/track_reduce.hip b/co_fusion_amd/csrc/track_reduce.hip
--- a/co_fusion_amd/csrc/track_reduce.hip
+++ b/co_fusion_amd/csrc/track_reduce.hip
@@ -696,12 +696,15 @@
     launch_icp_rgbres(s, cfg, args, RgbArgs{}, true, false, n, level, ev0, ev1);
 }
 
-void launch_so3_prealign(hipStream_t s, const TrackerStates& states, So3Sync* so3_syncs, int n, bool so3, int first_level, const RgbPrepBatch* prep)
+void launch_so3_prealign(hipStream_t s, const TrackerStates& states, So3Sync* so3_syncs, int n, bool so3, int first_level)
 {
     const int gx = so3 ? 8 * kSo3Blocks : 1;
-    static const RgbPrepBatch none{};
-    const int prep_bx = prep ? prep->m[0].L.blk_end[2] : 0;
-    so3_prealign_kernel<<<gx * n + prep_bx * n, 256, 0, s>>>(states, so3_syncs, so3 ? 1 : 0, first_level, gx, gx * n, prep ? *prep : none, prep_bx);
+    So3Images im{};
+    for (int m = 0; m < n; m++) {
+        const OdomDev* h = states.host[m];
+        im.next[m] = h->nextImage[2]; im.last[m] = h->lastNextImage[2]; im.cols[m] = h->width >> 2; im.rows[m] = h->height >> 2;
+    }
+    so3_prealign_kernel<<<gx * n, 256, 0, s>>>(states, im, so3_syncs, so3 ? 1 : 0, first_level, gx);
 }
 
 void launch_rgb_slot_step(hipStream_t s, const RgbArgs& ra, So3Sync* so3_syncs, int n, int mode, int icp_fix, int next_level, int last_of_level)
@@ -722,7 +725,7 @@
 
 bool launch_gn_track(hipStream_t s, IcpLaunch cfg, const TrackerStates& states, So3Sync* so3_syncs, const GnHook* hook, const IcpArgs icp_args[3],
                      const RgbArgs rgb_args[3], int n, int width, int height, bool so3, bool pyramid, bool fast_odom, bool rgb, bool icp, int mode,
-                     ProfSink* prof, OdomDev* const* h_states, const RgbPrepBatch* prep)
+                     ProfSink* prof, OdomDev* const* h_states, const RgbPrepBatch* prep, const SideLane* side, const FrameMapsArgs* maps)
 {
     int iterations[3];
     iterations[0] = fast_odom ? 3 : 10;
@@ -730,7 +733,14 @@
     iterations[2] = pyramid ? 4 : 0;
     int first_level = 2;
     while (first_level > 0 && iterations[first_level] == 0) first_level--;
-    launch_so3_prealign(s, states, so3_syncs, n, so3, first_level, prep);
+    if (prep && side) {
+        (void)hipEventRecord(side->fork, s);
+        (void)hipStreamWaitEvent(side->stream, side->fork, 0);
+        launch_track_head(side->stream, *prep, n, maps);
+        (void)hipEventRecord(side->done, side->stream);
+    } else if (prep) launch_track_head(s, *prep, n, maps);
+    launch_so3_prealign(s, states, so3_syncs, n, so3, first_level);
+    if (prep && side) (void)hipStreamWaitEvent(s, side->done, 0);
     GnArgs gn{};
     gn.icp_gram = cfg.gram;
     gn.slot_px = cfg.threads * 4;
diff --git a/co_fusion_amd/csrc/track_so3_dev.h b/co_fusion_amd/csrc/track_so3_dev.h
--- a/co_fusion_amd/csrc/track_so3_dev.h
+++ b/co_fusion_amd/csrc/track_so3_dev.h
@@ -45,18 +45,57 @@
     gy = ((back + actu) / 2.0f) - ((fore + actu) / 2.0f);
 }
 
+__device__ __forceinline__ void so3_add_pixel(unsigned long long (&acc)[16], int x, int y, float gnx, float gny, float glx, float gly,
+                                              float nextc, float lastc, const m33& Ki, const float* __restrict__ krlr)
+{
+    constexpr float lim = (float)(1 << ((50 - kFixSO3) / 2));
+    constexpr float scale = (float)(1 << kFixSO3);
+    const float a = krlr[0], b = krlr[1], c = krlr[2], d = krlr[3], e = krlr[4], f = krlr[5], g = krlr[6], h = krlr[7],
+                ii = krlr[8];
+    const f3 unwarped = {(float)x, (float)y, 1.0f};
+    const float gx = (gnx + glx) / 2.0f, gy = (gny + gly) / 2.0f;
+    const f3 point = mul(Ki, unwarped);
+    const float z2 = point.z * point.z;
+    const f3 left = {((point.z * (d * gy + a * gx)) - (gy * g * y) - (gx * g * x)) / z2,
+                     ((point.z * (e * gy + b * gx)) - (gy * h * y) - (gx * h * x)) / z2,
+                     ((point.z * (f * gy + c * gx)) - (gy * ii * y) - (gx * ii * x)) / z2};
+    const f3 jac = cross(left, point);
+    const float row[4] = {jac.x, jac.y, jac.z, -(nextc - lastc)};
+    double r[4], rs[4];
+#pragma unroll
+    for (int q = 0; q < 4; q++) { r[q] = (double)clamp_row(row[q], lim); rs[q] = (double)(clamp_row(row[q], lim) * scale); }
+#pragma unroll
+    for (int p = 0; p < 3; p++)
+#pragma unroll
+        for (int q = 0; q < 4; q++)
+            if (q >= p)
+                acc[4 * p - (p * (p - 1)) / 2 + (q - p)] += (unsigned long long)__double_as_longlong(fma(rs[p], r[q], kMagic)) - kMagicBits;
+    acc[9] += (unsigned long long)__double_as_longlong(fma(rs[3], r[3], kMagic)) - kMagicBits;
+    acc[10] += 1;
+}
+
+__device__ __forceinline__ void so3_fold(const unsigned long long (&acc)[16], unsigned long long (*lds)[16], unsigned long long* totals)
+{
+    const int lane = threadIdx.x & 63, wave = threadIdx.x >> 6, T = blockDim.x;
+    const unsigned long long v = wave_reduce16_u64(acc, lane);
+    if ((lane & 3) == 0) lds[wave][lane >> 2] = v;
+    __syncthreads();
+    if (threadIdx.x < 16) {
+        unsigned long long t = 0;
+        for (int w = 0; w < (T >> 6); w++) t += lds[w][threadIdx.x];
+        totals[threadIdx.x] = t;
+    }
+    __syncthreads();
+}
+
 __device__ __forceinline__ void so3_pass(const uint8_t* __restrict__ lastImage, const uint8_t* __restrict__ nextImage,
                                          const m33& B, const m33& Ki, const float* __restrict__ krlr, int cols, int rows,
                                          unsigned long long (*lds)[16], unsigned long long* totals, int block, int blocks)
 {
-    constexpr float lim = (float)(1 << ((50 - kFixSO3) / 2));
-    constexpr float scale = (float)(1 << kFixSO3);
     const int N = cols * rows, T = blockDim.x;
     unsigned long long acc[16];
 #pragma unroll
     for (int k = 0; k < 16; k++) acc[k] = 0;
-    const float a = krlr[0], b = krlr[1], c = krlr[2], d = krlr[3], e = krlr[4], f = krlr[5], g = krlr[6], h = krlr[7],
-                ii = krlr[8];
     for (int k = block * T + threadIdx.x; k < N; k += blocks * T) {
         const int y = k / cols, x = k - y * cols;
         const f3 unwarped = {(float)x, (float)y, 1.0f};
@@ -67,36 +106,75 @@
         float gnx, gny, glx, gly;
         so3_gradient(nextImage, cols, wx, wy, gnx, gny);
         so3_gradient(lastImage, cols, x, y, glx, gly);
-        const float gx = (gnx + glx) / 2.0f, gy = (gny + gly) / 2.0f;
-        const f3 point = mul(Ki, unwarped);
-        const float z2 = point.z * point.z;
-        const f3 left = {((point.z * (d * gy + a * gx)) - (gy * g * y) - (gx * g * x)) / z2,
-                         ((point.z * (e * gy + b * gx)) - (gy * h * y) - (gx * h * x)) / z2,
-                         ((point.z * (f * gy + c * gx)) - (gy * ii * y) - (gx * ii * x)) / z2};
-        const f3 jac = cross(left, point);
-        const float row[4] = {jac.x, jac.y, jac.z, -((float)nextImage[wy * cols + wx] - (float)lastImage[y * cols + x])};
-        double r[4], rs[4];
-#pragma unroll
-        for (int q = 0; q < 4; q++) { r[q] = (double)clamp_row(row[q], lim); rs[q] = (double)(clamp_row(row[q], lim) * scale); }
-#pragma unroll
-        for (int p = 0; p < 3; p++)
-#pragma unroll
-            for (int q = 0; q < 4; q++)
-                if (q >= p)
-                    acc[4 * p - (p * (p - 1)) / 2 + (q - p)] += (unsigned long long)__double_as_longlong(fma(rs[p], r[q], kMagic)) - kMagicBits;
-        acc[9] += (unsigned long long)__double_as_longlong(fma(rs[3], r[3], kMagic)) - kMagicBits;
-        acc[10] += 1;
-    }
-    const int lane = threadIdx.x & 63, wave = threadIdx.x >> 6;
-    const unsigned long long v = wave_reduce16_u64(acc, lane);
-    if ((lane & 3) == 0) lds[wave][lane >> 2] = v;
-    __syncthreads();
-    if (threadIdx.x < 16) {
-        unsigned long long t = 0;
-        for (int w = 0; w < (T >> 6); w++) t += lds[w][threadIdx.x];
-        totals[threadIdx.x] = t;
-    }
-    __syncthreads();
+        so3_add_pixel(acc, x, y, gnx, gny, glx, gly, (float)nextImage[wy * cols + wx], (float)lastImage[y * cols + x], Ki, krlr);
+    }
+    so3_fold(acc, lds, totals);
+}
+
+constexpr int kSo3Px = 96 / kSo3Blocks;
+constexpr int kSo3StageMax = kSo3Px * kSo3Blocks * 256;
+struct So3Held { float glx[kSo3Px], gly[kSo3Px], lastc[kSo3Px]; int xy[kSo3Px]; unsigned ok; };
+
+__device__ __forceinline__ void so3_hold(const uint8_t* __restrict__ lastImage, int cols, int rows, int block, int blocks, So3Held& h)
+{
+    const int N = cols * rows;
+    h.ok = 0;
+    int at[kSo3Px];
+#pragma unroll
+    for (int j = 0; j < kSo3Px; j++) {
+        const int k = (j * blocks + block) * 256 + (int)threadIdx.x;
+        const int y = k / cols, x = k - y * cols;
+        const bool in = k < N && x >= 1 && x < cols - 1 && y >= 1 && y < rows - 1;
+        if (in) h.ok |= 1u << j;
+        h.xy[j] = in ? (x | (y << 16)) : (1 | (1 << 16));
+        at[j] = in ? k : cols + 1;
+    }
+    float c[kSo3Px], l[kSo3Px], r[kSo3Px], u[kSo3Px], d[kSo3Px];
+#pragma unroll
+    for (int j = 0; j < kSo3Px; j++) {
+        c[j] = (float)lastImage[at[j]]; l[j] = (float)lastImage[at[j] - 1]; r[j] = (float)lastImage[at[j] + 1];
+        u[j] = (float)lastImage[at[j] - cols]; d[j] = (float)lastImage[at[j] + cols];
+    }
+#pragma unroll
+    for (int j = 0; j < kSo3Px; j++) {
+        h.glx[j] = ((l[j] + c[j]) / 2.0f) - ((r[j] + c[j]) / 2.0f);
+        h.gly[j] = ((u[j] + c[j]) / 2.0f) - ((d[j] + c[j]) / 2.0f);
+        h.lastc[j] = c[j];
+    }
+}
+
+__device__ __forceinline__ void so3_pass_staged(const So3Held& h, const uint8_t* s_next , const m33& B, const m33& Ki,
+                                                const float* __restrict__ krlr, int cols, int rows, unsigned long long (*lds)[16],
+                                                unsigned long long* totals)
+{
+    unsigned long long acc[16];
+#pragma unroll
+    for (int k = 0; k < 16; k++) acc[k] = 0;
+    unsigned ok = 0;
+    int at[kSo3Px];
+#pragma unroll
+    for (int j = 0; j < kSo3Px; j++) {
+        const int x = h.xy[j] & 0xffff, y = h.xy[j] >> 16;
+        const f3 unwarped = {(float)x, (float)y, 1.0f};
+        const f3 warped = mul(B, unwarped);
+        const int wx = f2i_rn(warped.x / warped.z), wy = f2i_rn(warped.y / warped.z);
+        const bool in = ((h.ok >> j) & 1u) && wx >= 1 && wx < cols - 1 && wy >= 1 && wy < rows - 1;
+        if (in) ok |= 1u << j;
+        at[j] = in ? wy * cols + wx : cols + 1;
+    }
+    float c[kSo3Px], l[kSo3Px], r[kSo3Px], u[kSo3Px], d[kSo3Px];
+#pragma unroll
+    for (int j = 0; j < kSo3Px; j++) {
+        c[j] = (float)s_next[at[j]]; l[j] = (float)s_next[at[j] - 1]; r[j] = (float)s_next[at[j] + 1];
+        u[j] = (float)s_next[at[j] - cols]; d[j] = (float)s_next[at[j] + cols];
+    }
+#pragma unroll
+    for (int j = 0; j < kSo3Px; j++)
+        if ((ok >> j) & 1u) {
+            const float gnx = ((l[j] + c[j]) / 2.0f) - ((r[j] + c[j]) / 2.0f), gny = ((u[j] + c[j]) / 2.0f) - ((d[j] + c[j]) / 2.0f);
+            so3_add_pixel(acc, h.xy[j] & 0xffff, h.xy[j] >> 16, gnx, gny, h.glx[j], h.gly[j], c[j], h.lastc[j], Ki, krlr);
+        }
+    so3_fold(acc, lds, totals);
 }
 
 __device__ inline void so3_unpack(const unsigned long long* t, float A[9], float b[3], float residual[2])
@@ -149,14 +227,9 @@
 #else
 #define OSTAMP(it, k) do {} while (0)
 #endif
-__global__ void __launch_bounds__(256) so3_prealign_kernel(const TrackerStates ts, So3Sync* __restrict__ syncs, int do_so3,
-                                                           int first_level, int gx, int so3_blocks, const RgbPrepBatch prep, int prep_bx)
-{
-    if ((int)blockIdx.x >= so3_blocks) {
-        const int r = (int)blockIdx.x - so3_blocks, m = r / prep_bx;
-        rgb_prep_body(prep.m[m], r - m * prep_bx);
-        return;
-    }
+__global__ void __launch_bounds__(256) so3_prealign_kernel(const TrackerStates ts, const So3Images im, So3Sync* __restrict__ syncs, int do_so3,
+                                                           int first_level, int gx)
+{
     const int by = (int)blockIdx.x / gx, bxx = (int)blockIdx.x - by * gx;
     OdomDev* const god = ts.dev[by];
     So3Sync* sync = syncs + by;
@@ -177,6 +250,21 @@
     const int bx = one_xcd ? (bxx >> 3) : bxx;
     const bool lead = bx == 0;
     const unsigned G = one_xcd ? (unsigned)gx >> 3 : (unsigned)gx;
+    __shared__ __attribute__((aligned(16))) uint8_t s_next[kSo3StageMax];
+    const int icols = im.cols[by], irows = im.rows[by], iN = icols * irows;
+    const bool staged = do_so3 && iN <= kSo3StageMax && iN <= kSo3Px * 256 * (int)G && icols >= 3 && irows >= 3;
+    const uint8_t* __restrict__ gnext = im.next[by];
+    const bool by_words = staged && (reinterpret_cast<uintptr_t>(gnext) & 3) == 0 && iN >= 4;
+    constexpr int kImgPer = kSo3StageMax / 4 / 256;
+    unsigned iw[kImgPer];
+    if (by_words) {
+        const int n_words = iN >> 2;
+#pragma unroll
+        for (int q = 0; q < kImgPer; q++) iw[q] = reinterpret_cast<const unsigned*>(gnext)[min((int)threadIdx.x + 256 * q, n_words - 1)];
+    }
+    So3Held held;
+    held.ok = 0;
+    if (staged) so3_hold(im.last[by], icols, irows, bx, (int)G, held);
     {
         static_assert(sizeof(OdomDev) % 4 == 0, "OdomDev is staged as 32-bit words");
         constexpr int kWords = (int)(sizeof(OdomDev) / 4);
@@ -187,6 +275,13 @@
         for (int q = 0; q < kPer; q++) w[q] = ((int)threadIdx.x + 256 * q < kWords) ? src[threadIdx.x + 256 * q] : 0u;
 #pragma unroll
         for (int q = 0; q < kPer; q++) if ((int)threadIdx.x + 256 * q < kWords) reinterpret_cast<unsigned*>(&s_od)[threadIdx.x + 256 * q] = w[q];
+        if (by_words) {
+#pragma unroll
+            for (int q = 0; q < kImgPer; q++) if ((int)threadIdx.x + 256 * q < (iN >> 2)) reinterpret_cast<unsigned*>(s_next)[threadIdx.x + 256 * q] = iw[q];
+            for (int k = (iN & ~3) + (int)threadIdx.x; k < iN; k += 256) s_next[k] = gnext[k];
+        } else if (staged) {
+            for (int k = threadIdx.x; k < iN; k += 256) s_next[k] = gnext[k];
+        }
         __syncthreads();
         if (lead) for (int k = threadIdx.x; k < kWords; k += 256) reinterpret_cast<unsigned*>(god)[k] = reinterpret_cast<const unsigned*>(&s_od)[k];
         __syncthreads();
@@ -218,7 +313,8 @@
             m33 B, Ki;
             for (int k = 0; k < 9; k++) { B.m[k] = s_basis[k]; Ki.m[k] = s_kinv[k]; }
             OSTAMP(it, 1);
-            so3_pass(lastNext, next, B, Ki, s_krlr, cols, rows, lds, totals, bx, (int)G);
+            if (staged) so3_pass_staged(held, s_next, B, Ki, s_krlr, cols, rows, lds, totals);
+            else so3_pass(lastNext, next, B, Ki, s_krlr, cols, rows, lds, totals, bx, (int)G);
             OSTAMP(it, 2);
             if (G > 1) {
                 if (threadIdx.x < 64) {
diff --git a/co_fusion_amd/host/CoFusion.cpp b/co_fusion_amd/host/CoFusion.cpp
--- a/co_fusion_amd/host/CoFusion.cpp
+++ b/co_fusion_amd/host/CoFusion.cpp
@@ -181,7 +181,7 @@
 void Model::bindFrameMaps(const float* const depthPyr[3], float depthCutoff, Model* frameOwner)
 {
     if (frameOwner == this) {
-        check(ctx, cf_odom_init_icp(odom, depthPyr, depthCutoff), "initICP");
+        check(ctx, cf_odom_init_icp_deferred(odom, depthPyr, depthCutoff), "initICP");
     } else {
         check(ctx, cf_odom_share_frame_maps(odom, frameOwner->odom), "share_frame_maps");
     }
diff --git a/co_fusion_amd/lib.py b/co_fusion_amd/lib.py
--- a/co_fusion_amd/lib.py
+++ b/co_fusion_amd/lib.py
@@ -15,7 +15,7 @@
     "cf_rgba_to_intensity", "cf_sobel", "cf_project_cloud", "cf_icp_step", "cf_icp_step_band", "cf_rgb_residual", "cf_rgb_step",
     "cf_so3_step", "cf_gn_solve_step", "cf_so3_prealign_step", "cf_rgb_records_step","cf_odom_create", "cf_odom_destroy", "cf_odom_init_icp_model", "cf_odom_init_rgb_model",
     "cf_odom_init_rgb", "cf_odom_init_models_batch", "cf_odom_init_models_batch_frames", "cf_odom_init_models_batch_select", "cf_model_fill_ratio_device", "cf_odom_init_first_rgb", "cf_odom_init_icp", "cf_odom_init_icp_maps", "cf_odom_get_incremental_transformation",
-    "cf_odom_track_batch_async", "cf_odom_fetch_result", "cf_odom_get_covariance", "cf_odom_bind_frame_maps", "cf_odom_share_frame_maps", "cf_odom_set_culling", "cf_odom_set_band", "cf_set_collective", "cf_model_predict_indices_sharded", "cf_odom_buffer",
+    "cf_odom_init_icp_deferred", "cf_odom_track_batch_async", "cf_odom_fetch_result", "cf_odom_get_covariance", "cf_odom_bind_frame_maps", "cf_odom_share_frame_maps", "cf_odom_set_culling", "cf_odom_set_band", "cf_set_collective", "cf_model_predict_indices_sharded", "cf_odom_buffer",
     "cf_bilateral", "cf_model_create", "cf_model_destroy", "cf_model_initialise", "cf_model_count",
     "cf_model_predict_indices", "cf_model_index_keys", "cf_model_index_resolve", "cf_model_combined_predict", "cf_model_predict_inactive", "cf_model_synthesize_depth", "cf_model_prefetch_fill_ratio", "cf_model_perform_fill_in", "cf_model_requires_fill_in",
     "cf_model_fuse", "cf_model_clean", "cf_models_frame_passes", "cf_models_preindex", "cf_model_download_map", "cf_model_upload_map", "cf_model_buffer",
diff --git a/include/cofusion_hip.h b/include/cofusion_hip.h
--- a/include/cofusion_hip.h
+++ b/include/cofusion_hip.h
@@ -150,6 +150,7 @@
                                      const uint32_t *const *fill_counts, float ratio, const float *const *poses ,
                                      const uint8_t *const *frame_rgba );
 int cf_odom_init_icp(cf_odom *od, const float *const depth_pyr[CF_NUM_PYRS], float depth_cutoff);
+int cf_odom_init_icp_deferred(cf_odom *od, const float *const depth_pyr[CF_NUM_PYRS], float depth_cutoff);
 int cf_odom_get_incremental_transformation(cf_odom *od, float trans[3], float rot[9], const cf_track_opts *opts,
                                            float *icp_err_surface, cf_track_stats *stats);
 int cf_odom_track_batch_async(cf_ctx *ctx, cf_odom *const *ods, int n, const float *const *poses_in ,
```

Result: no change. 954.2 (-0.9%).
